# ashawkey/torch-ngp

Measured on AMD Instinct MI355X. Metric: training samples/s (rays x steps), lego-shaped synthetic, fp16 autocast, full step incl. Adam, higher is better.
Workload: dtype f16

## Files before the change

include/ngp_hip.h:

```cpp
#ifndef NGP_HIP_H
#define NGP_HIP_H

#include <stddef.h>
#include <stdint.h>

#ifdef __cplusplus
extern "C" {
#endif

typedef void* ngp_stream_t;

enum {
    NGP_OK = 0,
    NGP_ERR_INVALID = 1,
    NGP_ERR_LAUNCH = 2,
    NGP_ERR_DEVICE = 3
};

enum { NGP_F32 = 0, NGP_F16 = 1, NGP_F64 = 2 };

#define NGP_MAX_LEVELS 32

const char* ngp_last_error(void);
int ngp_abi_version(void);
// ... 177 lines not shown
#define NGP_FF_LAYERED 4u
#define NGP_FF_SINGLE_WAVE 8u
#define NGP_FF_DEFER_REDUCE 16u
#define NGP_FF_RECOMPUTE 32u
#define NGP_FF_SERIAL_FLUSH 64u
int ngp_ffmlp_forward_ex(const void* inputs, const void* weights, uint32_t B, uint32_t input_dim, uint32_t output_dim,
                         uint32_t hidden_dim, uint32_t num_layers, uint32_t activation, uint32_t output_activation,
                         void* forward_buffer, void* outputs, uint32_t flags, ngp_stream_t stream);
int ngp_ffmlp_inference_ex(const void* inputs, const void* weights, uint32_t B, uint32_t input_dim,
                           uint32_t output_dim, uint32_t hidden_dim, uint32_t num_layers, uint32_t activation,
                           uint32_t output_activation, void* inference_buffer, void* outputs, uint32_t flags,
                           ngp_stream_t stream);
int ngp_ffmlp_backward_ex(const void* grad, const void* inputs, const void* weights, const void* forward_buffer,
                          uint32_t B, uint32_t input_dim, uint32_t output_dim, uint32_t hidden_dim, uint32_t num_layers,
                          uint32_t activation, uint32_t output_activation, int calc_grad_inputs, void* backward_buffer,
                          void* grad_inputs, void* grad_weights, uint32_t flags, ngp_stream_t stream);

size_t ngp_ffmlp_backward_workspace_bytes(uint32_t B, uint32_t input_dim, uint32_t hidden_dim, uint32_t num_layers);
int ngp_ffmlp_backward_ws(const void* grad, const void* inputs, const void* weights, const void* forward_buffer, uint32_t B,
                          uint32_t input_dim, uint32_t output_dim, uint32_t hidden_dim, uint32_t num_layers, uint32_t activation,
                          uint32_t output_activation, int calc_grad_inputs, void* backward_buffer, void* grad_inputs, void* grad_weights,
                          uint32_t flags, void* workspace, size_t workspace_bytes, ngp_stream_t stream);

size_t ngp_ffmlp_backward_backward_workspace_bytes(uint32_t B, uint32_t input_dim, uint32_t hidden_dim, uint32_t num_layers,
                                                   uint32_t activation);
int ngp_ffmlp_backward_backward(const void* grad, const void* inputs, const void* weights, const void* forward_buffer, const void* u,
                                uint32_t B, uint32_t input_dim, uint32_t output_dim, uint32_t hidden_dim, uint32_t num_layers,
                                uint32_t activation, void* grad_grad, void* grad_weights2, void* grad_inputs2, void* workspace,
                                size_t workspace_bytes, ngp_stream_t stream);

int ngp_network_forward(const void* enc, const float* dirs, uint32_t M, uint32_t M_valid, const void* w_sigma, const void* w_color,
                        uint32_t num_layers_sigma, uint32_t num_layers_color, float density_scale, int training,
                        void* forward_buffer_sigma, void* h16, float* sigma, void* color_in, void* forward_buffer_color, float* rgb,
                        uint32_t flags, ngp_stream_t stream);

int ngp_network_forward_rows(const void* enc, const float* dirs, uint32_t M, uint32_t M_valid, const void* w_sigma, const void* w_color,
                             uint32_t num_layers_sigma, uint32_t num_layers_color, float density_scale, int training,
                             void* forward_buffer_sigma, void* h16, float* sigma, void* color_in, void* forward_buffer_color, float* rgb,
                             uint32_t flags, const uint32_t* rows_dev, ngp_stream_t stream);

int ngp_network_backward_color(const void* grad_out16, const void* color_in, const void* w_color, const void* forward_buffer_color, uint32_t M,
                               uint32_t num_layers_color, void* backward_buffer, const float* grad_sigma, const void* h16,
                               float density_scale, void* grad_h16, void* grad_w_color, uint32_t flags, ngp_stream_t stream);
uint32_t ngp_ffmlp_backward_slab_count(uint32_t B, uint32_t input_dim, uint32_t hidden_dim, uint32_t num_layers);
int ngp_ffmlp_reduce_slabs_pair(const void* slabs_a, uint32_t n_slabs_a, uint32_t n_params_a, void* grad_weights_a, const void* slabs_b,
                                uint32_t n_slabs_b, uint32_t n_params_b, void* grad_weights_b, float* found_inf, ngp_stream_t stream);

int ngp_pipeline_mid_forward(const void* h16, const float* dirs, float* sigma, void* color_in, uint32_t M, uint32_t M_valid,
                             float density_scale, ngp_stream_t stream);
int ngp_pipeline_rgb_forward(const void* out16, float* rgb, uint32_t M, ngp_stream_t stream);
int ngp_pipeline_rgb_backward(const float* grad_rgb, const float* rgb, void* grad_out16, uint32_t M, ngp_stream_t stream);
int ngp_pipeline_mid_backward(const float* grad_sigma, const void* h16, const void* grad_color_in, void* grad_h16, uint32_t M,
                              float density_scale, ngp_stream_t stream);

int ngp_pipeline_mse_loss(const float* image, const float* target, uint32_t n, const float* loss_scale, float* loss,
                          float* grad_image, ngp_stream_t stream);

#define NGP_LINEAR_STACK_MAX 8
uint32_t ngp_linear_stack_flat_size(uint32_t depth, uint32_t n_in, uint32_t hidden, uint32_t n_out, int identity);
int ngp_linear_stack_pack(const float* const* weights, uint32_t depth, uint32_t n_in, uint32_t hidden, uint32_t n_out, int identity,
                          void* flat_fp16, ngp_stream_t stream);
int ngp_linear_stack_unpack_grad(const void* grad_flat_fp16, uint32_t depth, uint32_t n_in, uint32_t hidden, uint32_t n_out, int identity,
                                 float* const* grads, ngp_stream_t stream);

int ngp_pad_2d_fp16(const void* src, uint32_t src_rows, uint32_t src_cols, uint32_t src_row_stride, void* dst, uint32_t dst_rows,
                    uint32_t dst_cols, ngp_stream_t stream);

int ngp_rays_from_pixels(const float* poses, uint32_t B, float fx, float fy, float cx, float cy, uint32_t W, const int64_t* inds,
                         uint32_t inds_batch_stride, uint32_t N, float* rays_o, float* rays_d, ngp_stream_t stream);

#define NGP_MARCH_RESET_COUNTER 1u
#define NGP_MARCH_ZERO_TAIL 2u
#define NGP_MARCH_SCAN_LAUNCH 8u
#define NGP_MARCH_NOISE_FROM_SEED 4u
int ngp_march_rays_train_ex(const float* rays_o, const float* rays_d, const uint8_t* grid, float bound, float dt_gamma,
                            uint32_t max_steps, uint32_t N, uint32_t C, uint32_t H, uint32_t M, const float* nears,
                            const float* fars, float* xyzs, float* dirs, float* deltas, int32_t* rays, int32_t* counter,
                            const float* noises, void* workspace, uint32_t flags, ngp_stream_t stream);
int ngp_march_rays_train_aabb(const float* rays_o, const float* rays_d, const uint8_t* grid, float bound, float dt_gamma,
                              uint32_t max_steps, uint32_t N, uint32_t C, uint32_t H, uint32_t M, const float* aabb, float min_near,
                              float* nears, float* fars, float* xyzs, float* dirs, float* deltas, int32_t* rays, int32_t* counter,
                              const float* noises, void* workspace, uint32_t flags, ngp_stream_t stream);

int ngp_march_rays_ex(uint32_t n_alive, uint32_t n_step, const int32_t* rays_alive, const float* rays_t, const float* rays_o,
                      const float* rays_d, float bound, float dt_gamma, uint32_t max_steps, uint32_t C, uint32_t H,
                      const uint8_t* grid, const float* nears, const float* fars, float* xyzs, float* dirs, float* deltas,
                      const float* noises, uint32_t zero_rows, ngp_stream_t stream);

int ngp_march_rays_dev(const int32_t* state, uint32_t alive_bound, uint32_t n_total, uint32_t n_step_cap, const int32_t* rays_alive, const float* rays_t,
                       const float* rays_o, const float* rays_d, float bound, float dt_gamma, uint32_t max_steps, uint32_t C, uint32_t H,
                       const uint8_t* grid, const float* nears, const float* fars, float* xyzs, float* dirs, float* deltas,
                       const float* noises, uint32_t rows, ngp_stream_t stream);
int ngp_march_rays_dev_rows(const int32_t* state, uint32_t alive_bound, uint32_t n_total, uint32_t n_step_cap, const int32_t* rays_alive, const float* rays_t,
                            const float* rays_o, const float* rays_d, float bound, float dt_gamma, uint32_t max_steps, uint32_t C, uint32_t H,
                            const uint8_t* grid, const float* nears, const float* fars, float* xyzs, float* dirs, float* deltas,
                            const float* noises, uint32_t rows, uint32_t* rows_used, ngp_stream_t stream);
int ngp_composite_rays_dev(const int32_t* state, uint32_t alive_bound, uint32_t n_total, uint32_t n_step_cap, float T_thresh, int32_t* rays_alive, float* rays_t,
                           const float* sigmas, const float* rgbs, const float* deltas, float* weights_sum, float* depth, float* image,
                           ngp_stream_t stream);
int ngp_compact_rays_dev(const int32_t* state, uint32_t alive_bound, uint32_t n_total, uint32_t n_step_cap, uint32_t max_steps, const int32_t* rays_alive,
                         int32_t* out_alive, int32_t* out_state, void* workspace, ngp_stream_t stream);

int ngp_composite_rays_features(uint32_t n_alive, uint32_t n_step, float T_thresh, const int32_t* rays_alive, const float* sigmas,
                                const void* feats, const float* deltas, const float* weights_sum, uint32_t C, int feat_dtype,
                                float* out, ngp_stream_t stream);
int ngp_composite_rays_features_dev(const int32_t* state, uint32_t alive_bound, uint32_t n_total, uint32_t n_step_cap, float T_thresh,
                                    const int32_t* rays_alive, const float* sigmas, const void* feats, const float* deltas,
                                    const float* weights_sum, uint32_t C, int feat_dtype, float* out, ngp_stream_t stream);

typedef struct ngp_render_loop {
    int32_t* state;
    int32_t* alive[2];
    float* rays_t; const float* rays_o; const float* rays_d; const float* nears; const float* fars; const uint8_t* grid; const float* noises;
    float* xyzs; float* dirs; float* deltas; void* enc; float* sigmas; float* rgbs;
    const void* embeddings; const int32_t* offsets; const float* level_cost_host; const void* w_sigma; const void* w_color;
    float* weights_sum; float* depth; float* image; void* compact_workspace;
    uint32_t* rows_used;
    uint32_t lanes, rows, n_total, n_step_cap, max_steps, cascade, grid_size;
    uint32_t L, H, gridtype, interp, num_layers_sigma, num_layers_color;
    int32_t align_corners;
    float bound, dt_gamma, T_thresh, S, density_scale;
} ngp_render_loop_t;
int ngp_render_iterations_dev(const ngp_render_loop_t* args, uint32_t n_iter, uint32_t first_cur, ngp_stream_t stream);

size_t ngp_coarse_occupancy_bytes(uint32_t C, uint32_t H);
int ngp_coarse_occupancy(const uint8_t* grid, uint32_t C, uint32_t H, uint8_t* coarse, ngp_stream_t stream);
int ngp_cull_rays(const float* rays_o, const float* rays_d, const float* nears, const float* fars, uint32_t N, float bound, uint32_t C,
                  uint32_t H, const uint8_t* coarse, int32_t* rays_alive, ngp_stream_t stream);

int ngp_composite_rays_train_forward_ex(const float* sigmas, const float* rgbs, const float* deltas, const int32_t* rays,
                                        uint32_t M, uint32_t N, float T_thresh, float* weights_sum, float* depth, float* image,
                                        int bg_mode, float bg_scalar, const float* bg, const float* nears, const float* fars,
                                        float* image_out, float* depth_out, ngp_stream_t stream);
int ngp_composite_rays_train_backward_ex(const float* grad_weights_sum, const float* grad_image, const float* sigmas,
                                         const float* rgbs, const float* deltas, const int32_t* rays,
                                         const float* weights_sum, const float* image, uint32_t M, uint32_t N,
                                         float T_thresh, float* grad_sigmas, float* grad_rgbs, int bg_mode, float bg_scalar,
                                         const float* bg, const uint32_t* rows_used, ngp_stream_t stream);

int ngp_composite_rays_train_geo_forward(const float* sigmas, const float* rgbs, const float* deltas, const int32_t* rays, uint32_t M,
                                         uint32_t N, float T_thresh, float* weights_sum, float* depth, float* image,
                                         float* distortion, ngp_stream_t stream);
int ngp_composite_rays_train_geo_backward(const float* grad_weights_sum, const float* grad_depth, const float* grad_image,
                                          const float* grad_distortion, const float* sigmas, const float* rgbs, const float* deltas,
                                          const int32_t* rays, const float* weights_sum, const float* depth, const float* image,
                                          const float* distortion, uint32_t M, uint32_t N, float T_thresh, float* grad_sigmas,
                                          float* grad_rgbs, ngp_stream_t stream);
int ngp_composite_rays_train_geo_forward_f64(const double* sigmas, const double* rgbs, const double* deltas, const int32_t* rays,
                                             uint32_t M, uint32_t N, float T_thresh, double* weights_sum, double* depth, double* image,
                                             double* distortion, ngp_stream_t stream);
int ngp_composite_rays_train_geo_backward_f64(const double* grad_weights_sum, const double* grad_depth, const double* grad_image,
                                              const double* grad_distortion, const double* sigmas, const double* rgbs,
                                              const double* deltas, const int32_t* rays, const double* weights_sum, const double* depth,
                                              const double* image, const double* distortion, uint32_t M, uint32_t N, float T_thresh,
                                              double* grad_sigmas, double* grad_rgbs, ngp_stream_t stream);

int ngp_composite_rays_train_features_forward(const float* sigmas, const void* feats, const float* deltas, const int32_t* rays, uint32_t M,
                                              uint32_t N, uint32_t C, float T_thresh, int feat_dtype, float* out, ngp_stream_t stream);
int ngp_composite_rays_train_features_backward(const float* grad_out, const float* sigmas, const void* feats, const float* deltas,
                                               const int32_t* rays, const float* out, uint32_t M, uint32_t N, uint32_t C, float T_thresh,
                                               int feat_dtype, float* grad_sigmas, void* grad_feats, ngp_stream_t stream);
int ngp_composite_rays_train_features_forward_f64(const double* sigmas, const double* feats, const double* deltas, const int32_t* rays,
                                                  uint32_t M, uint32_t N, uint32_t C, float T_thresh, double* out, ngp_stream_t stream);
int ngp_composite_rays_train_features_backward_f64(const double* grad_out, const double* sigmas, const double* feats, const double* deltas,
                                                   const int32_t* rays, const double* out, uint32_t M, uint32_t N, uint32_t C,
                                                   float T_thresh, double* grad_sigmas, double* grad_feats, ngp_stream_t stream);
// ... 91 lines not shown
```

torch-ngp_amd/_ngp_capi.py:

```python
import ctypes
import os

import torch

_HERE = os.path.dirname(os.path.abspath(__file__))
LIB_PATH = os.environ.get('NGP_HIP_LIBRARY') or os.path.join(_HERE, 'libngp_hip.so')

NGP_F32, NGP_F16, NGP_F64 = 0, 1, 2
NGP_FF_INPUT_PLANAR, NGP_FF_DX_PLANAR, NGP_FF_LAYERED, NGP_FF_SINGLE_WAVE, NGP_FF_DEFER_REDUCE, NGP_FF_RECOMPUTE = 1, 2, 4, 8, 16, 32
NGP_FF_SERIAL_FLUSH = 64
NGP_MARCH_RESET_COUNTER, NGP_MARCH_ZERO_TAIL, NGP_MARCH_NOISE_FROM_SEED, NGP_MARCH_SCAN_LAUNCH = 1, 2, 4, 8
NGP_OPT_PHASE_CHECK, NGP_OPT_PHASE_UPDATE, NGP_OPT_PHASE_COMMIT, NGP_OPT_PHASE_FLIP = 1, 2, 4, 8
ABI_VERSION = 11

if not os.path.exists(LIB_PATH):
    raise ImportError(
        f"{LIB_PATH} is missing: build the HIP extension first (python __graft_entry__.py, or "
        f"make -C {os.path.join(_HERE, 'csrc')}).  There is no CPU fallback for these operators.")

lib = ctypes.CDLL(LIB_PATH)

_vp, _u32, _f32, _i32, _sz = ctypes.c_void_p, ctypes.c_uint32, ctypes.c_float, ctypes.c_int, ctypes.c_size_t

_SIGNATURES = {
    'ngp_grid_encode_forward': [_vp, _vp, _vp, _vp, _u32, _u32, _u32, _u32, _f32, _u32, _vp, _u32, _i32, _u32, _i32, _vp],
    'ngp_grid_encode_backward': [_vp, _vp, _vp, _vp, _vp, _u32, _u32, _u32, _u32, _f32, _u32, _vp, _vp, _u32, _i32, _u32, _i32, _vp],
    'ngp_grad_total_variation': [_vp, _vp, _vp, _vp, _f32, _u32, _u32, _u32, _u32, _f32, _u32, _u32, _i32, _i32, _vp],
    'ngp_grid_corner_indices': [_vp, _vp, _vp, _u32, _u32, _u32, _f32, _u32, _u32, _i32, _vp],
    'ngp_grid_level_table': [_u32, _f32, _u32, _vp, _vp],
    'ngp_grid_encode_backward_backward': [_vp, _vp, _vp, _vp, _vp, _vp, _vp, _vp, _u32, _u32, _u32, _u32, _f32, _u32, _u32, _i32, _u32, _i32, _vp,
                                          _sz, _vp],
    'ngp_grid_encode_backward_ordered': [_vp, _vp, _vp, _vp, _vp, _u32, _u32, _u32, _u32, _f32, _u32, _vp, _vp, _u32, _i32, _u32, _i32, _f32, _vp,
                                         _sz, _vp],
    'ngp_grid_encode_backward_backward_ordered': [_vp, _vp, _vp, _vp, _vp, _vp, _vp, _vp, _u32, _u32, _u32, _u32, _f32, _u32, _u32, _i32, _u32, _i32,
                                                  _vp, _sz, _vp],
    'ngp_grid_backward_is_reproducible': [_vp, _u32, _u32, _u32, _u32, _f32, _u32, _u32, _i32, _i32],
    'ngp_sh_encode_forward': [_vp, _vp, _u32, _u32, _u32, _vp, _i32, _vp],
    'ngp_sh_encode_backward': [_vp, _vp, _u32, _u32, _u32, _vp, _vp, _i32, _vp],
    'ngp_freq_encode_forward': [_vp, _u32, _u32, _u32, _u32, _vp, _vp],
    'ngp_freq_encode_backward': [_vp, _vp, _u32, _u32, _u32, _u32, _vp, _vp],
    'ngp_freq_encode_forward_f64': [_vp, _u32, _u32, _u32, _u32, _vp, _vp],
    'ngp_freq_encode_backward_f64': [_vp, _vp, _u32, _u32, _u32, _u32, _vp, _vp],
    'ngp_freq_encode_backward_backward': [_vp, _vp, _vp, _u32, _u32, _u32, _u32, _vp, _vp, _i32, _vp],
    'ngp_sh_encode_backward_backward': [_vp, _vp, _vp, _vp, _u32, _u32, _u32, _vp, _vp, _i32, _vp],
    'ngp_near_far_from_aabb': [_vp, _vp, _vp, _u32, _f32, _vp, _vp, _vp],
    'ngp_sph_from_ray': [_vp, _vp, _f32, _u32, _vp, _vp],
    'ngp_morton3D': [_vp, _u32, _vp, _vp],
    'ngp_morton3D_invert': [_vp, _u32, _vp, _vp],
    'ngp_packbits': [_vp, _u32, _f32, _vp, _vp],
    'ngp_packbits_ex': [_vp, _u32, _f32, _vp, _vp, _vp],
    'ngp_march_rays_train': [_vp, _vp, _vp, _f32, _f32, _u32, _u32, _u32, _u32, _u32, _vp, _vp, _vp, _vp, _vp, _vp, _vp, _vp, _vp, _vp],
    'ngp_composite_rays_train_forward': [_vp, _vp, _vp, _vp, _u32, _u32, _f32, _vp, _vp, _vp, _vp],
    'ngp_composite_rays_train_backward': [_vp, _vp, _vp, _vp, _vp, _vp, _vp, _vp, _u32, _u32, _f32, _vp, _vp, _vp],
    'ngp_march_rays': [_u32, _u32, _vp, _vp, _vp, _vp, _f32, _f32, _u32, _u32, _u32, _vp, _vp, _vp, _vp, _vp, _vp, _vp, _vp],
    'ngp_march_rays_ex': [_u32, _u32, _vp, _vp, _vp, _vp, _f32, _f32, _u32, _u32, _u32, _vp, _vp, _vp, _vp, _vp, _vp, _vp, _u32, _vp],
    'ngp_composite_rays': [_u32, _u32, _f32, _vp, _vp, _vp, _vp, _vp, _vp, _vp, _vp, _vp],
    'ngp_near_far_from_aabb_f64': [_vp, _vp, _vp, _u32, _f32, _vp, _vp, _vp],
    'ngp_sph_from_ray_f64': [_vp, _vp, _f32, _u32, _vp, _vp],
    'ngp_packbits_f64': [_vp, _u32, _f32, _vp, _vp],
    'ngp_composite_rays_train_forward_f64': [_vp, _vp, _vp, _vp, _u32, _u32, _f32, _vp, _vp, _vp, _vp],
    'ngp_composite_rays_train_backward_f64': [_vp, _vp, _vp, _vp, _vp, _vp, _vp, _vp, _u32, _u32, _f32, _vp, _vp, _vp],
    'ngp_composite_rays_f64': [_u32, _u32, _f32, _vp, _vp, _vp, _vp, _vp, _vp, _vp, _vp, _vp],
    'ngp_compact_rays': [_vp, _u32, _vp, _vp, _vp, _vp],
    'ngp_coarse_occupancy': [_vp, _u32, _u32, _vp, _vp],
    'ngp_cull_rays': [_vp, _vp, _vp, _vp, _u32, _f32, _u32, _u32, _vp, _vp, _vp],
    'ngp_march_rays_dev': [_vp, _u32, _u32, _u32, _vp, _vp, _vp, _vp, _f32, _f32, _u32, _u32, _u32, _vp, _vp, _vp, _vp, _vp, _vp, _vp, _u32, _vp],
    'ngp_composite_rays_dev': [_vp, _u32, _u32, _u32, _f32, _vp, _vp, _vp, _vp, _vp, _vp, _vp, _vp, _vp],
    'ngp_compact_rays_dev': [_vp, _u32, _u32, _u32, _u32, _vp, _vp, _vp, _vp, _vp],
    'ngp_render_iterations_dev': [_vp, _u32, _u32, _vp],
    'ngp_ffmlp_forward': [_vp, _vp, _u32, _u32, _u32, _u32, _u32, _u32, _u32, _vp, _vp, _vp],
    'ngp_ffmlp_inference': [_vp, _vp, _u32, _u32, _u32, _u32, _u32, _u32, _u32, _vp, _vp, _vp],
    'ngp_ffmlp_backward': [_vp, _vp, _vp, _vp, _u32, _u32, _u32, _u32, _u32, _u32, _u32, _i32, _vp, _vp, _vp, _vp],
    'ngp_grid_encode_forward_ex': [_vp, _vp, _vp, _vp, _u32, _u32, _u32, _u32, _f32, _u32, _vp, _u32, _i32, _u32, _i32, _f32, _vp],
    'ngp_grid_encode_forward_sched': [_vp, _vp, _vp, _vp, _u32, _u32, _u32, _u32, _f32, _u32, _vp, _u32, _i32, _u32, _i32, _f32, _vp, _vp],
    'ngp_grid_encode_forward_sel': [_vp, _vp, _vp, _vp, _vp, _vp, _vp, _u32, _u32, _u32, _u32, _f32, _u32, _u32, _i32, _u32, _i32, _f32, _vp, _vp],
    'ngp_grid_encode_backward_ex': [_vp, _vp, _vp, _vp, _vp, _u32, _u32, _u32, _u32, _f32, _u32, _vp, _vp, _u32, _i32, _u32, _i32, _f32, _vp],
    'ngp_grid_encode_backward_ws': [_vp, _vp, _vp, _vp, _vp, _u32, _u32, _u32, _u32, _f32, _u32, _vp, _vp, _u32, _i32, _u32, _i32, _f32, _vp, _vp,
                                    _sz, _vp],
    'ngp_grid_encode_backward_checked': [_vp, _vp, _vp, _vp, _vp, _u32, _u32, _u32, _u32, _f32, _u32, _vp, _vp, _u32, _i32, _u32, _i32, _f32, _vp,
                                         _vp, _sz, _vp, _vp],
    'ngp_grid_encode_backward_checked_slabs': [_vp, _vp, _vp, _vp, _vp, _u32, _u32, _u32, _u32, _f32, _u32, _vp, _vp, _u32, _i32, _u32, _i32, _f32,
                                               _vp, _vp, _sz, _vp, _vp, _vp],
    'ngp_density_grid_update': [_vp, _vp, _u32, _f32, _f32, _vp, _u32, _vp, _f32, _vp, _vp, _vp, _vp],
    'ngp_ffmlp_forward_ex': [_vp, _vp, _u32, _u32, _u32, _u32, _u32, _u32, _u32, _vp, _vp, _u32, _vp],
    'ngp_ffmlp_inference_ex': [_vp, _vp, _u32, _u32, _u32, _u32, _u32, _u32, _u32, _vp, _vp, _u32, _vp],
    'ngp_ffmlp_backward_ex': [_vp, _vp, _vp, _vp, _u32, _u32, _u32, _u32, _u32, _u32, _u32, _i32, _vp, _vp, _vp, _u32, _vp],
    'ngp_ffmlp_backward_ws': [_vp, _vp, _vp, _vp, _u32, _u32, _u32, _u32, _u32, _u32, _u32, _i32, _vp, _vp, _vp, _u32, _vp, _sz, _vp],
    'ngp_ffmlp_backward_backward': [_vp, _vp, _vp, _vp, _vp, _u32, _u32, _u32, _u32, _u32, _u32, _vp, _vp, _vp, _vp, _sz, _vp],
    'ngp_network_forward': [_vp, _vp, _u32, _u32, _vp, _vp, _u32, _u32, _f32, _i32, _vp, _vp, _vp, _vp, _vp, _vp, _u32, _vp],
    'ngp_network_forward_rows': [_vp, _vp, _u32, _u32, _vp, _vp, _u32, _u32, _f32, _i32, _vp, _vp, _vp, _vp, _vp, _vp, _u32, _vp, _vp],
    'ngp_march_rays_dev_rows': [_vp, _u32, _u32, _u32, _vp, _vp, _vp, _vp, _f32, _f32, _u32, _u32, _u32, _vp, _vp, _vp, _vp, _vp, _vp, _vp, _u32, _vp, _vp],
    'ngp_pipeline_mid_forward': [_vp, _vp, _vp, _vp, _u32, _u32, _f32, _vp],
    'ngp_pipeline_rgb_forward': [_vp, _vp, _u32, _vp],
    'ngp_pipeline_rgb_backward': [_vp, _vp, _vp, _u32, _vp],
    'ngp_pipeline_mid_backward': [_vp, _vp, _vp, _vp, _u32, _f32, _vp],
    'ngp_pipeline_mse_loss': [_vp, _vp, _u32, _vp, _vp, _vp, _vp],
    'ngp_rays_from_pixels': [_vp, _u32, _f32, _f32, _f32, _f32, _u32, _vp, _u32, _u32, _vp, _vp, _vp],
    'ngp_march_rays_train_ex': [_vp, _vp, _vp, _f32, _f32, _u32, _u32, _u32, _u32, _u32, _vp, _vp, _vp, _vp, _vp, _vp, _vp, _vp, _vp, _u32, _vp],
    'ngp_march_rays_train_aabb': [_vp, _vp, _vp, _f32, _f32, _u32, _u32, _u32, _u32, _u32, _vp, _f32, _vp, _vp, _vp, _vp, _vp, _vp, _vp, _vp, _vp, _u32,
                                  _vp],
    'ngp_composite_rays_train_forward_ex': [_vp, _vp, _vp, _vp, _u32, _u32, _f32, _vp, _vp, _vp, _i32, _f32, _vp, _vp, _vp, _vp, _vp, _vp],
    'ngp_composite_rays_train_backward_ex': [_vp, _vp, _vp, _vp, _vp, _vp, _vp, _vp, _u32, _u32, _f32, _vp, _vp, _i32, _f32, _vp, _vp, _vp],
    'ngp_composite_rays_train_geo_forward': [_vp, _vp, _vp, _vp, _u32, _u32, _f32, _vp, _vp, _vp, _vp, _vp],
    'ngp_composite_rays_train_geo_backward': [_vp, _vp, _vp, _vp, _vp, _vp, _vp, _vp, _vp, _vp, _vp, _vp, _u32, _u32, _f32, _vp, _vp, _vp],
    'ngp_composite_rays_train_geo_forward_f64': [_vp, _vp, _vp, _vp, _u32, _u32, _f32, _vp, _vp, _vp, _vp, _vp],
    'ngp_composite_rays_train_geo_backward_f64': [_vp, _vp, _vp, _vp, _vp, _vp, _vp, _vp, _vp, _vp, _vp, _vp, _u32, _u32, _f32, _vp, _vp, _vp],
    'ngp_composite_rays_train_features_forward': [_vp, _vp, _vp, _vp, _u32, _u32, _u32, _f32, _i32, _vp, _vp],
    'ngp_composite_rays_train_features_backward': [_vp, _vp, _vp, _vp, _vp, _vp, _u32, _u32, _u32, _f32, _i32, _vp, _vp, _vp],
    'ngp_composite_rays_train_features_forward_f64': [_vp, _vp, _vp, _vp, _u32, _u32, _u32, _f32, _vp, _vp],
    'ngp_composite_rays_train_features_backward_f64': [_vp, _vp, _vp, _vp, _vp, _vp, _u32, _u32, _u32, _f32, _vp, _vp, _vp],
    'ngp_composite_rays_features': [_u32, _u32, _f32, _vp, _vp, _vp, _vp, _vp, _u32, _i32, _vp, _vp],
    'ngp_composite_rays_features_dev': [_vp, _u32, _u32, _u32, _f32, _vp, _vp, _vp, _vp, _vp, _u32, _i32, _vp, _vp],
    'ngp_composite_train_loss_backward': [_vp, _vp, _vp, _vp, _u32, _u32, _f32, _i32, _f32, _vp, _vp, _vp, _vp, _vp, _vp, _vp, _vp, _vp, _vp, _vp,
                                          _vp, _vp, _sz, _vp],
    'ngp_composite_train_geo_loss_backward': [_vp, _vp, _vp, _vp, _u32, _u32, _f32, _i32, _f32, _vp, _vp, _vp, _vp, _f32, _f32, _vp, _vp, _vp, _vp,
                                              _vp, _vp, _vp, _vp, _vp, _vp, _vp, _vp, _vp, _sz, _vp],
    'ngp_network_backward_color': [_vp, _vp, _vp, _vp, _u32, _u32, _vp, _vp, _vp, _f32, _vp, _vp, _u32, _vp],
    'ngp_ffmlp_reduce_slabs_pair': [_vp, _u32, _u32, _vp, _vp, _u32, _u32, _vp, _vp, _vp],
    'ngp_optim_adam_step': [_i32, _vp, _vp, _vp, _vp, _vp, _vp, _vp, _vp, _f32, _f32, _f32, _f32, _f32, _f32, _f32, _vp, _vp],
    'ngp_optim_adam_step_ex': [_i32, _vp, _vp, _vp, _vp, _vp, _vp, _vp, _vp, _f32, _f32, _f32, _f32, _f32, _f32, _f32, _vp, _vp, _f32, _u32, _vp],
    'ngp_optim_adam_small_commit': [_i32, _vp, _vp, _vp, _vp, _vp, _vp, _vp, _vp, _f32, _f32, _f32, _f32, _f32, _f32, _f32, _vp, _i32, _vp, _vp,
                                    ctypes.c_uint64, _vp],
    'ngp_optim_ema_update': [_i32, _vp, _vp, _vp, _f32, _vp],
    'ngp_optim_poison_shards': [_vp, _u32, ctypes.c_uint64, _vp, _vp],
    'ngp_optim_shard_verdict': [_vp, _vp, _vp, _u32, ctypes.c_uint64, _vp],
    'ngp_linear_stack_pack': [_vp, _u32, _u32, _u32, _u32, _i32, _vp, _vp],
    'ngp_linear_stack_unpack_grad': [_vp, _u32, _u32, _u32, _u32, _i32, _vp, _vp],
    'ngp_pad_2d_fp16': [_vp, _u32, _u32, _u32, _vp, _u32, _u32, _vp],
    'ngp_allocate_splitk': [_sz],
    'ngp_free_splitk': [],
    'ngp_cmdlist_create': [_vp],
    'ngp_cmdlist_begin': [_vp],
    'ngp_cmdlist_mark': [_vp, _u32, _i32],
    'ngp_cmdlist_end': [_vp],
    'ngp_cmdlist_count': [_vp, _vp],
    'ngp_cmdlist_entry_name': [_vp, _u32, _vp, _u32],
    'ngp_cmdlist_replay': [_vp, _vp],
    'ngp_cmdlist_wait_mark': [_vp, _u32, _vp],
    'ngp_cmdlist_destroy': [_vp],
    'ngp_ray_sample_ts': [_vp, _vp, _vp, _vp, _u32, _u32, _f32, _vp, _vp],
    'ngp_ray_sample_ts_f64': [_vp, _vp, _vp, _vp, _u32, _u32, _f32, _vp, _vp],
    'ngp_ray_points_forward': [_vp, _vp, _vp, _vp, _u32, _u32, _f32, _vp, _vp, _vp],
    'ngp_ray_points_forward_f64': [_vp, _vp, _vp, _vp, _u32, _u32, _f32, _vp, _vp, _vp],
    'ngp_ray_points_backward': [_vp, _vp, _vp, _vp, _vp, _vp, _vp, _u32, _u32, _f32, _vp, _vp, _vp],
    'ngp_ray_points_backward_f64': [_vp, _vp, _vp, _vp, _vp, _vp, _u32, _u32, _f32, _vp, _vp, _vp],
    'ngp_grid_input_gradient': [_vp, _vp, _vp, _vp, _u32, _u32, _u32, _u32, _f32, _u32, _u32, _i32, _u32, _i32, _f32, _vp, _vp],
    'ngp_rays_from_pixels_backward': [_vp, _vp, _u32, _f32, _f32, _f32, _f32, _u32, _vp, _u32, _u32, _vp, _vp],
    'ngp_error_map_draw': [_vp, _u32, _u32, _u32, _u32, _u32, _u32, _vp, _vp, _vp, _vp, _vp, _vp],
    'ngp_error_map_update': [_vp, _vp, _vp, _vp, _u32, _u32, _f32, _f32, _vp],
}
for _name, _args in _SIGNATURES.items():
    _fn = getattr(lib, _name)
    _fn.argtypes = _args
    _fn.restype = ctypes.c_int
lib.ngp_last_error.restype = ctypes.c_char_p
lib.ngp_target_arch.restype = ctypes.c_char_p
lib.ngp_abi_version.restype = ctypes.c_int
lib.ngp_ffmlp_backward_slab_count.argtypes = [_u32, _u32, _u32, _u32]
lib.ngp_ffmlp_backward_slab_count.restype = _u32
lib.ngp_march_rays_train_workspace_bytes.argtypes = [_u32]
lib.ngp_march_rays_train_workspace_bytes.restype = _sz
lib.ngp_compact_rays_workspace_bytes.argtypes = [_u32]
lib.ngp_ffmlp_backward_workspace_bytes.argtypes = [_u32, _u32, _u32, _u32]
lib.ngp_ffmlp_backward_workspace_bytes.restype = _sz
lib.ngp_ffmlp_backward_backward_workspace_bytes.argtypes = [_u32, _u32, _u32, _u32, _u32]
lib.ngp_ffmlp_backward_backward_workspace_bytes.restype = _sz
lib.ngp_grid_backward_workspace_bytes.argtypes = [_vp, _u32, _u32, _u32, _u32, _f32, _u32, _u32, _i32, _i32]
lib.ngp_grid_backward_workspace_bytes.restype = _sz
lib.ngp_grid_backward_backward_workspace_bytes.argtypes = [_vp, _u32, _u32, _u32, _u32, _i32]
lib.ngp_grid_backward_backward_workspace_bytes.restype = _sz
lib.ngp_compact_rays_workspace_bytes.restype = _sz
lib.ngp_grid_ordered_workspace_bytes.argtypes = [_u32, _u32, _u32, _i32]
lib.ngp_grid_ordered_workspace_bytes.restype = _sz
lib.ngp_grid_table_adam_prefix.argtypes = [_vp, _u32, _u32, _u32, _u32, _f32, _u32, _u32, _i32, _i32]
lib.ngp_grid_table_adam_prefix.restype = _u32
lib.ngp_coarse_occupancy_bytes.argtypes = [_u32, _u32]
lib.ngp_coarse_occupancy_bytes.restype = _sz
lib.ngp_grid_forward_work_lists.argtypes = [_u32, _u32, _vp, _vp, _vp, _vp]
lib.ngp_grid_forward_work_lists.restype = _u32
lib.ngp_density_grid_update_workspace_bytes.argtypes = [_u32]
lib.ngp_linear_stack_flat_size.argtypes = [_u32, _u32, _u32, _u32, _i32]
lib.ngp_linear_stack_flat_size.restype = _u32
lib.ngp_density_grid_update_workspace_bytes.restype = _sz
# ... 138 lines not shown
```

torch-ngp_amd/csrc/common.h:

```cpp
#pragma once
#include <hip/hip_runtime.h>
#include <stdint.h>
#include <cstdio>
#include <cstdarg>

#include "../../include/ngp_hip.h"
#include "cmdlist_core.h"

namespace ngp {

using half_t = _Float16;
typedef _Float16 half2_t __attribute__((ext_vector_type(2)));
typedef _Float16 half4_t __attribute__((ext_vector_type(4)));
typedef _Float16 half8_t __attribute__((ext_vector_type(8)));
typedef float float2_t __attribute__((ext_vector_type(2)));
typedef float float4_t __attribute__((ext_vector_type(4)));
typedef float float16_t __attribute__((ext_vector_type(16)));

constexpr int WAVE = 64;

void set_error(const char* fmt, ...);
void set_error_message(const char* message);

inline int check_launch(const char* what) {
    hipError_t e = hipGetLastError();
    if (e != hipSuccess) {
        set_error("%s: kernel launch failed: %s", what, hipGetErrorString(e));
        return NGP_ERR_LAUNCH;
    }
    return NGP_OK;
}

#define NGP_REQUIRE(cond, code, ...)        \
    do {                                    \
        if (!(cond)) {                      \
            ::ngp::set_error(__VA_ARGS__);  \
            return (code);                  \
        }                                   \
    } while (0)

inline uint32_t cdiv(uint32_t a, uint32_t b) { return (a + b - 1) / b; }
inline uint64_t cdiv64(uint64_t a, uint64_t b) { return (a + b - 1) / b; }

inline hipStream_t as_stream(ngp_stream_t s) { return reinterpret_cast<hipStream_t>(s); }

template <typename T> struct launch_param { using type = T; };
template <typename... KA>
inline hipError_t launch(const char* name, void (*kernel)(KA...), dim3 grid, dim3 block, size_t lds, hipStream_t st, const typename launch_param<KA>::type&... a) {
    void* argv[] = {const_cast<void*>(static_cast<const void*>(&a))..., nullptr};
    const hipError_t e = hipLaunchKernel(reinterpret_cast<const void*>(kernel), grid, block, argv, lds, st);
    if (cmdlist::List* l = cmdlist::recording()) {
        static const size_t sizes[] = {sizeof(KA)..., 0}, aligns[] = {alignof(KA)..., 0};
        l->record_launch(reinterpret_cast<const void*>(kernel), name, cmdlist::Dim{grid.x, grid.y, grid.z}, cmdlist::Dim{block.x, block.y, block.z},
                         (uint32_t)lds, (uint32_t)sizeof...(KA), argv, sizes, aligns);
    }
    return e;
}
#define NGP_LAUNCH_STATUS(kernel, grid, block, lds, st, ...) ::ngp::launch(#kernel, kernel, grid, block, lds, st, __VA_ARGS__)
#define NGP_LAUNCH(...) ((void)NGP_LAUNCH_STATUS(__VA_ARGS__))
inline hipError_t memset_async(void* dst, int value, size_t bytes, hipStream_t st) {
    const hipError_t e = hipMemsetAsync(dst, value, bytes, st);
    if (cmdlist::List* l = cmdlist::recording()) e == hipSuccess ? l->record_memset(dst, value, bytes) : l->poison();
    return e;
}
inline hipError_t memcpy_async(void* dst, const void* src, size_t bytes, hipMemcpyKind kind, hipStream_t st) {
    const hipError_t e = hipMemcpyAsync(dst, src, bytes, kind, st);
    if (cmdlist::List* l = cmdlist::recording()) e == hipSuccess ? l->record_memcpy(dst, src, bytes, (int)kind) : l->poison();
    return e;
}

#ifdef NGP_DEBUG_BOUNDS
#define NGP_BOUNDS(cond) do { if (!(cond)) __builtin_trap(); } while (0)
#else
#define NGP_BOUNDS(cond) do { } while (0)
#endif

__device__ __forceinline__ _Float16 to_half_rne(float v) {
    asm volatile("" : "+v"(v));
    return (_Float16)v;
}

__device__ __forceinline__ float clampf(float x, float lo, float hi) { return fminf(hi, fmaxf(lo, x)); }

__device__ __forceinline__ uint32_t wave_inclusive_scan(uint32_t v) {
    const int lane = threadIdx.x & 63;
#pragma unroll
    for (int o = 1; o < 64; o <<= 1) {
        uint32_t n = __shfl_up(v, o, 64);
        if (lane >= o) v += n;
    }
    return v;
}

__device__ __forceinline__ float wave_sum(float v) {
#pragma unroll
    for (int o = 32; o > 0; o >>= 1) v += __shfl_xor(v, o, 64);
    return v;
}

template <int CTRL, int ROW_MASK>
__device__ __forceinline__ float dpp_or(float identity, float src) {
    return __builtin_bit_cast(float, __builtin_amdgcn_update_dpp(__builtin_bit_cast(int, identity), __builtin_bit_cast(int, src), CTRL, ROW_MASK,
                                                                 0xF, false));
}
__device__ __forceinline__ float wave_incl_sum(float v, int) {
    v += dpp_or<0x111, 0xF>(0.0f, v);
    v += dpp_or<0x112, 0xF>(0.0f, v);
    v += dpp_or<0x114, 0xF>(0.0f, v);
    v += dpp_or<0x118, 0xF>(0.0f, v);
    v += dpp_or<0x142, 0xA>(0.0f, v);
    v += dpp_or<0x143, 0xC>(0.0f, v);
    return v;
}
__device__ __forceinline__ float lane63(float v) { return __builtin_bit_cast(float, __builtin_amdgcn_readlane(__builtin_bit_cast(int, v), 63)); }
__device__ __forceinline__ float wave_total(float v) { return lane63(wave_incl_sum(v, 0)); }

__device__ __forceinline__ void loss_sum_block(const float* err, uint32_t N, float* loss, float* part) {
    const uint32_t t = threadIdx.x;
    float acc = 0.0f;
    if (t < 256u) {
        for (uint32_t i = t; i < N; i += 256u) acc += __hip_atomic_load(&err[i], __ATOMIC_RELAXED, __HIP_MEMORY_SCOPE_AGENT);
        acc = wave_total(acc);
        if ((t & 63u) == 0u) part[t >> 6] = acc;
    }
    __syncthreads();
    if (t == 0u) {
        float v = 0.0f;
#pragma unroll
        for (int w = 0; w < 4; w++) v += part[w];
        loss[0] = v / (float)(3u * N);
    }
}

enum OptState { OPT_SCALE, OPT_GROWTH_TRACKER, OPT_FOUND_INF, OPT_STEP_COUNT, OPT_LR_MULT, OPT_TABLE_PARITY, OPT_TICKET, OPT_SCALE_DEAD, OPT_STATE_WORDS };
static_assert(OPT_STATE_WORDS == 8, "include/ngp_hip.h: state = device float[8]");
struct AdamConsts {
    float inv_scale, bc1, bc2_sqrt, lr_mult;
    bool skip;
};
__device__ __forceinline__ AdamConsts adam_consts(const float* state, float beta1, float beta2, float grad_mult) {
    AdamConsts a;
    const bool scale_dead = !__builtin_isfinite(1.0f / state[OPT_SCALE]);
    a.skip = state[OPT_FOUND_INF] != 0.0f || scale_dead;
    a.inv_scale = scale_dead ? 0.0f : grad_mult / state[OPT_SCALE];
    const float t = state[OPT_STEP_COUNT] + 1.0f;
    a.bc1 = 1.0f - powf(beta1, t);
    a.bc2_sqrt = sqrtf(1.0f - powf(beta2, t));
    a.lr_mult = state[OPT_LR_MULT];
    return a;
}
__device__ __forceinline__ void adam_element(float g, float& pm, float& pv, float& pp, float beta1, float beta2, float eps, float step_size,
                                             float bc2_sqrt) {
    pm = beta1 * pm + (1.0f - beta1) * g;
    pv = beta2 * pv + (1.0f - beta2) * g * g;
    pp -= step_size * pm / (sqrtf(pv) / bc2_sqrt + eps);
}
struct TableAdam {
    float* p[2];
// ... 73 lines not shown
```

torch-ngp_amd/csrc/ffmlp.hip:

```cpp
#include "common.h"
#include "sh_poly.inc"

namespace ngp {

constexpr int FF_WAVES = 4;
constexpr int FF_THREADS = FF_WAVES * 64;
constexpr int FF_TILE = 32;

enum Act : uint32_t { ACT_RELU = 0, ACT_EXP = 1, ACT_SINE = 2, ACT_SIGMOID = 3, ACT_SQUAREPLUS = 4, ACT_SOFTPLUS = 5, ACT_NONE = 6 };
constexpr float K_ACT = 10.0f;

__device__ __forceinline__ float act_forward(uint32_t a, float x) {
    switch (a) {
        case ACT_RELU: return x > 0.0f ? x : 0.0f;
        case ACT_EXP: return __expf(x);
        case ACT_SINE: return __sinf(x);
        case ACT_SIGMOID: return 1.0f / (1.0f + __expf(-x));
        case ACT_SQUAREPLUS: { const float s = x * K_ACT; return 0.5f * (s + sqrtf(s * s + 4.0f)) / K_ACT; }
        case ACT_SOFTPLUS: return __logf(__expf(x * K_ACT) + 1.0f) / K_ACT;
        default: return x;
    }
}
__device__ __forceinline__ float act_backward_factor(uint32_t a, float y) {
    switch (a) {
// ... 251 lines not shown
            const half8_t* wl = img_hid + (size_t)l * NIB * NKB * 64;
#pragma unroll
            for (int ib = 0; ib < NIB; ib++) {
                acc[ib] = zero16();
#pragma unroll
                for (int kb = 0; kb < NKB; kb++) acc[ib] = mfma(wl[(ib * NKB + kb) * 64], hid[kb], acc[ib]);
            }
        }
        float16_t o = zero16();
#pragma unroll
        for (int kb = 0; kb < NKB; kb++) o = mfma(img_out[kb * 64], hid[kb], o);
        half4_t lo, hi;
#pragma unroll
        for (int c = 0; c < 4; c++) {
            lo[c] = (half_t)(PLAIN ? o[c] : act_forward(out_act, o[c]));
            hi[c] = (half_t)(PLAIN ? o[4 + c] : act_forward(out_act, o[4 + c]));
        }
        half_t* orow = outputs + ((size_t)tile * FF_TILE + n) * 16 + 4 * h;
        *reinterpret_cast<half4_t*>(orow) = lo;
        *reinterpret_cast<half4_t*>(orow + 8) = hi;
    }
}

template <int WIDTH, bool TRAIN, bool PLAIN>
__global__ __launch_bounds__(FF_THREADS) __attribute__((amdgpu_waves_per_eu(4, 4))) void k_ffmlp_forward(
    const half_t* __restrict__ inputs, const half_t* __restrict__ weights, half_t* __restrict__ forward_buffer, half_t* __restrict__ outputs,
    uint32_t n_tiles, uint32_t in_dim, uint32_t num_layers, uint32_t act, uint32_t out_act, bool in_planar) {
    ffmlp_forward_body<WIDTH, TRAIN, PLAIN>(inputs, weights, forward_buffer, outputs, n_tiles, in_dim, num_layers, act, out_act, in_planar);
}
template <int WIDTH, bool TRAIN, bool PLAIN>
__global__ __launch_bounds__(FF_THREADS) __attribute__((amdgpu_waves_per_eu(2, 2))) void k_ffmlp_forward_wide(
    const half_t* __restrict__ inputs, const half_t* __restrict__ weights, half_t* __restrict__ forward_buffer, half_t* __restrict__ outputs,
    uint32_t n_tiles, uint32_t in_dim, uint32_t num_layers, uint32_t act, uint32_t out_act, bool in_planar) {
    ffmlp_forward_body<WIDTH, TRAIN, PLAIN>(inputs, weights, forward_buffer, outputs, n_tiles, in_dim, num_layers, act, out_act, in_planar);
}


template <bool TRAIN, int NT>
__device__ __forceinline__ void relu_network_tail(float16_t (&acc)[NT][2], float16_t (&o)[NT], const half8_t* __restrict__ hid_img,
                                                  const half8_t* __restrict__ out_img, uint32_t nl, half_t* __restrict__ fb, size_t layer_stride,
                                                  const uint32_t (&tile)[NT], const bool (&live)[NT], int lane) {
    constexpr int WIDTH = 64, NIB = 2, NKB = 4;
    half8_t hid[NT][NKB];
    for (uint32_t l = 0;; l++) {
#pragma unroll
        for (int t = 0; t < NT; t++) {
            pack_hidden_relu<WIDTH>(acc[t], hid[t]);
            if (TRAIN && fb && live[t]) {
                half8_t* dst = reinterpret_cast<half8_t*>(fb) + l * layer_stride + (size_t)tile[t] * NKB * 64 + lane;
#pragma unroll
                for (int kb = 0; kb < NKB; kb++) stream_store(dst + kb * 64, hid[t][kb]);
            }
        }
        if (l + 1 == nl) break;
        const half8_t* wl = hid_img + (size_t)l * NIB * NKB * 64;
#pragma unroll
        for (int ib = 0; ib < NIB; ib++) {
#pragma unroll
            for (int t = 0; t < NT; t++) acc[t][ib] = zero16();
#pragma unroll
            for (int kb = 0; kb < NKB; kb++) {
                const half8_t a = wl[(ib * NKB + kb) * 64];
#pragma unroll
                for (int t = 0; t < NT; t++) acc[t][ib] = mfma(a, hid[t][kb], acc[t][ib]);
            }
        }
    }
#pragma unroll
    for (int t = 0; t < NT; t++) o[t] = zero16();
#pragma unroll
    for (int kb = 0; kb < NKB; kb++) {
        const half8_t a = out_img[kb * 64];
#pragma unroll
        for (int t = 0; t < NT; t++) o[t] = mfma(a, hid[t][kb], o[t]);
    }
}

template <bool TRAIN, int WAVES , int NT >
__global__ __launch_bounds__(WAVES * 64) __attribute__((amdgpu_waves_per_eu(NT == 1 ? 4 : 2, NT == 1 ? 4 : 3))) void k_network_forward(
    const half_t* __restrict__ enc, bool enc_planar, const float* __restrict__ dirs, uint32_t M_valid, const half_t* __restrict__ w_sigma,
    const half_t* __restrict__ w_color, half_t* __restrict__ fb_s, half_t* __restrict__ h16, float* __restrict__ sigma,
    half_t* __restrict__ color_in, half_t* __restrict__ fb_c, float* __restrict__ rgb, uint32_t n_tiles_cap, uint32_t nl_s, uint32_t nl_c,
    float density_scale, const uint32_t* __restrict__ rows_dev) {
    constexpr int WIDTH = 64, NIB = 2, NKB = 4;
    constexpr uint32_t in_kb = 2;
    const uint32_t n_tiles = rows_dev ? min(n_tiles_cap, (rows_dev[0] + (uint32_t)FF_TILE - 1u) / (uint32_t)FF_TILE) : n_tiles_cap;
    extern __shared__ __attribute__((aligned(16))) unsigned char smem[];
    half8_t* img_s = reinterpret_cast<half8_t*>(smem);
    const uint32_t frags_s = NIB * in_kb + (nl_s - 1) * NIB * NKB + NKB;
    half8_t* img_c = img_s + (size_t)frags_s * 64;
    const size_t rows = (size_t)n_tiles_cap * FF_TILE;
    const int lane = threadIdx.x & 63, wid = threadIdx.x >> 6;
    const int n = lane & 31, h = lane >> 5;
    const uint32_t n_groups = (n_tiles + NT - 1) / NT;
    half8_t x_next[NT][in_kb];
    float dir_next[NT][3];
#pragma unroll
    for (int t = 0; t < NT; t++) dir_next[t][0] = dir_next[t][1] = dir_next[t][2] = 0.0f;
    auto request = [&](uint32_t group) {
        if (group < n_groups) {
#pragma unroll
            for (int t = 0; t < NT; t++) {
                const uint32_t tl = group * NT + t < n_tiles ? group * NT + t : n_tiles - 1;
                const size_t srow = (size_t)tl * FF_TILE + n;
#pragma unroll
                for (uint32_t kb = 0; kb < in_kb; kb++) x_next[t][kb] = load_features8(enc, enc_planar, rows, srow, 32, 16 * kb + 8 * h);
                dir_next[t][0] = dir_next[t][1] = dir_next[t][2] = 0.0f;
                if (srow < M_valid) { dir_next[t][0] = dirs[srow * 3]; dir_next[t][1] = dirs[srow * 3 + 1]; dir_next[t][2] = dirs[srow * 3 + 2]; }
            }
        }
    };
    request(blockIdx.x * WAVES + wid);
    build_forward_image<WIDTH>(img_s, w_sigma, 32, nl_s);
    build_forward_image<WIDTH>(img_c, w_color, 32, nl_c);
    __syncthreads();

    const size_t layer_stride = (size_t)n_tiles_cap * NKB * 64;
    const half8_t* s_l0 = img_s + lane;
    const half8_t* s_hid = s_l0 + (size_t)NIB * in_kb * 64;
    const half8_t* s_out = s_hid + (size_t)(nl_s - 1) * NIB * NKB * 64;
    const half8_t* c_l0 = img_c + lane;
    const half8_t* c_hid = c_l0 + (size_t)NIB * in_kb * 64;
    const half8_t* c_out = c_hid + (size_t)(nl_c - 1) * NIB * NKB * 64;

    for (uint32_t group = blockIdx.x * WAVES + wid; group < n_groups; group += gridDim.x * WAVES) {
        uint32_t tile[NT];
        bool live[NT];
        size_t srow[NT];
        half8_t x_cur[NT][in_kb];
        float dir_x[NT], dir_y[NT], dir_z[NT];
#pragma unroll
        for (int t = 0; t < NT; t++) {
            live[t] = NT == 1 || group * NT + t < n_tiles;
            tile[t] = live[t] ? group * NT + t : n_tiles - 1;
            srow[t] = (size_t)tile[t] * FF_TILE + n;
#pragma unroll
            for (uint32_t kb = 0; kb < in_kb; kb++) x_cur[t][kb] = x_next[t][kb];
            dir_x[t] = dir_next[t][0]; dir_y[t] = dir_next[t][1]; dir_z[t] = dir_next[t][2];
        }
        request(group + gridDim.x * WAVES);
        float16_t acc[NT][NIB], o[NT];
#pragma unroll
        for (int t = 0; t < NT; t++)
#pragma unroll
            for (int ib = 0; ib < NIB; ib++) acc[t][ib] = zero16();
#pragma unroll
        for (uint32_t kb = 0; kb < in_kb; kb++)
#pragma unroll
            for (int ib = 0; ib < NIB; ib++) {
                const half8_t a = s_l0[(ib * in_kb + kb) * 64];
#pragma unroll
                for (int t = 0; t < NT; t++) acc[t][ib] = mfma(a, x_cur[t][kb], acc[t][ib]);
            }
        relu_network_tail<TRAIN, NT>(acc, o, s_hid, s_out, nl_s, fb_s, layer_stride, tile, live, lane);
        half8_t cin[NT][2];
#pragma unroll
        for (int t = 0; t < NT; t++) {
            half4_t lo, hi;
#pragma unroll
            for (int c = 0; c < 4; c++) { lo[c] = (half_t)o[t][c]; hi[c] = (half_t)o[t][4 + c]; }
            if (TRAIN && live[t]) {
                half_t* hrow = h16 + srow[t] * 16 + 4 * h;
                *reinterpret_cast<half4_t*>(hrow) = lo;
                *reinterpret_cast<half4_t*>(hrow + 8) = hi;
            }
            if (h == 0 && live[t]) sigma[srow[t]] = density_scale * expf((float)lo[0]);
// ... 529 lines not shown
                pack_transposed(t, xT);
#pragma unroll
                for (int g = 0; g < 2; g++)
#pragma unroll
                    for (int ib = 0; ib < NIB; ib++) gw_in[ib][jb] = mfma(zT[ib][g], xT[g], gw_in[ib][jb]);
            }
        }
        if (with_dx) store_dx<WIDTH, IN_JB>(img_in, dz, grad_inputs, tile, n, h, in_dim, rows, dx_planar);
        if (pf_depth == 1 && tile + tile_step < n_tiles) {
            asm volatile("s_waitcnt lgkmcnt(0)" ::: "memory");
            prefetch_tile<WIDTH>(pf_base, tile + tile_step, grad, fb, inputs, num_layers, layer_stride, rows, in_dim, in_planar, lane, n, h);
        }
    }

    float* red = reinterpret_cast<float*>(smem);
    const SlabLayout lay{WIDTH, in_dim, num_layers};
    const uint32_t n_params = lay.n_params();
    auto each = [&](const auto& sink) { slab_put_all<WIDTH, IN_JB, NHM>(sink, lay, gw_in, gw_hid, gw_out); };
    if (slab_staged_single<WIDTH, IN_JB, NHM> && !serial_flush) {
        static_assert(!slab_staged_single<WIDTH, IN_JB, NHM> || slab_fits_whole<WIDTH, IN_JB, NHM>, "the single-wave staged sum is one pass");
        slab_sum_pass<FF_THREADS>(red, lds_bytes, SlabPart{0, n_params}, wid, slabs + (size_t)blockIdx.x * n_params, grad_weights_direct, n, h, each);
        return;
    }
    slab_serial_begin<FF_THREADS>(red, n_params);
    const SlabSerial serial{red, n, h};
    for (int turn = 0; turn < FF_WAVES; turn++) {
        if (wid == turn) each(serial);
        __syncthreads();
    }
    slab_serial_store<FF_THREADS>(red, n_params, slabs, grad_weights_direct);
}

constexpr int FP_PAIRS = 4;
constexpr int FP_THREADS = 2 * FP_PAIRS * 64;

struct MidEpilogue {
    const float* grad_sigma;
    const half_t* h16;
    half_t* grad_h16;
    float density_scale;
};

template <int WIDTH, int NHM, typename Sink>
__device__ __forceinline__ void recompute_hidden(const half8_t* __restrict__ fimg_lane, uint32_t in_kb, const unsigned char* xb, bool in_planar,
                                                 int lane, Sink&& sink) {
    constexpr int NIB = Shape<WIDTH>::NIB, NKB = Shape<WIDTH>::NKB;
    float16_t acc[NIB];
#pragma unroll
    for (int ib = 0; ib < NIB; ib++) acc[ib] = zero16();
    for (uint32_t kb = 0; kb < in_kb; kb++) {
        const half8_t x = tile_x(xb, kb, in_planar, lane);
#pragma unroll
        for (int ib = 0; ib < NIB; ib++) acc[ib] = mfma(fimg_lane[(ib * in_kb + kb) * 64], x, acc[ib]);
    }
    const half8_t* fhid = fimg_lane + (size_t)NIB * in_kb * 64;
    half8_t hid[NKB];
#pragma unroll
    for (int l = 0; l <= NHM; l++) {
        pack_hidden_relu<WIDTH>(acc, hid);
        sink(l, hid);
        if (l == NHM) break;
        const half8_t* wl = fhid + (size_t)l * NIB * NKB * 64;
#pragma unroll
        for (int ib = 0; ib < NIB; ib++) {
            acc[ib] = zero16();
#pragma unroll
            for (int kb = 0; kb < NKB; kb++) acc[ib] = mfma(wl[(ib * NKB + kb) * 64], hid[kb], acc[ib]);
        }
    }
}

template <int N>
__device__ __forceinline__ void wait_vmcnt() {
    asm volatile("s_waitcnt vmcnt(%0)" ::"n"(N) : "memory");
}

template <int WIDTH, int IN_JB, int NHM , bool RELU, bool RECOMP = false>
__global__ __launch_bounds__(FP_THREADS) __attribute__((amdgpu_waves_per_eu(2, 2)))
void k_ffmlp_backward_paired(const half_t* __restrict__ grad, const half_t* __restrict__ inputs, const half_t* __restrict__ weights,
                             const half_t* __restrict__ forward_buffer, uint32_t n_tiles, uint32_t in_dim, uint32_t num_layers, uint32_t act,
                             bool with_dx, half_t* __restrict__ grad_inputs, float* __restrict__ slabs,
                             half_t* __restrict__ grad_weights_direct, bool in_planar, bool dx_planar, uint32_t pf_depth, MidEpilogue mid,
                             uint32_t lds_bytes, bool serial_flush) {
    static_assert(NHM == 1 || NHM == 2, "the paired backward covers 2- and 3-layer networks");
    constexpr int NIB = Shape<WIDTH>::NIB, NKB = Shape<WIDTH>::NKB;
    extern __shared__ __attribute__((aligned(16))) unsigned char smem[];
    half8_t* img = reinterpret_cast<half8_t*>(smem);
    const uint32_t nfrag = bwd_frag_count<WIDTH>(in_dim, num_layers, with_dx);
    const uint32_t in_kb = in_dim / 16;
    const uint32_t ffrag = RECOMP ? NIB * in_kb + (num_layers - 1) * NIB * NKB : 0u;
    const int lane = threadIdx.x & 63, wid = threadIdx.x >> 6;
    const int n = lane & 31, h = lane >> 5;
    const int pair = wid & (FP_PAIRS - 1), role = wid / FP_PAIRS;
    const size_t layer_stride = (size_t)n_tiles * NKB * 64;
    const half8_t* fb = reinterpret_cast<const half8_t*>(forward_buffer);
    const size_t rows = (size_t)n_tiles * FF_TILE;
    const uint32_t act_layers = RECOMP ? 0u : num_layers;
    const uint32_t tile_frags = 1 + act_layers * NKB + in_kb;
    unsigned char* pf_base = smem + (size_t)(nfrag + ffrag) * 1024 + (size_t)pair * pf_depth * tile_frags * 1024;
    half8_t* scratch = reinterpret_cast<half8_t*>(smem + (size_t)(nfrag + ffrag) * 1024 + (size_t)FP_PAIRS * pf_depth * tile_frags * 1024 +
                                                  (size_t)pair * NHM * NKB * 1024) + lane;
    const uint32_t base_step = gridDim.x * FP_PAIRS;
    uint32_t cur = 0;
    const uint32_t tile_loads = tile_dma_count<WIDTH>(act_layers, in_dim, in_planar);
    auto prefetch = [&](uint32_t buffer, uint32_t tile) {
        const uint32_t issued = prefetch_tile<WIDTH>(pf_base + (size_t)buffer * tile_frags * 1024, tile, grad, fb, inputs, act_layers, layer_stride,
                                                     rows, in_dim, in_planar, lane, n, h);
        NGP_BOUNDS(issued == tile_loads);
        (void)issued;
    };
    if (role == 0) {
        for (uint32_t d = 0; d + 1 < (pf_depth > 1 ? pf_depth : 2u); d++)
            if (blockIdx.x * FP_PAIRS + d * base_step + pair < n_tiles) prefetch(d, blockIdx.x * FP_PAIRS + d * base_step + pair);
    }
    build_backward_image<WIDTH>(img, weights, in_dim, num_layers, with_dx);
    if (RECOMP) build_forward_image<WIDTH>(img + (size_t)nfrag * 64, weights, in_dim, num_layers, 0, ffrag);
    const Selectors sel = make_selectors(n, h);
    __syncthreads();

    const half8_t* img_out = img + lane;
    const half8_t* img_hid = img_out + (size_t)NIB * 64;
    const half8_t* img_in = img_hid + (size_t)(num_layers - 1) * NIB * NKB * 64;
    const half8_t* fimg = img + (size_t)nfrag * 64 + lane;
    static_assert(tile_dma_count<64>(0, 32, false) == 3u && tile_dma_count<64>(0, 32, true) == 9u && tile_dma_count<64>(2, 32, false) == 11u &&
                  tile_dma_count<64>(2, 32, true) == 17u, "the enumerated vmcnt immediates below are the DMA counts of the three-deep shapes");
    const bool deep = pf_depth == 3 && (tile_loads == 3u || tile_loads == 9u || tile_loads == 11u || tile_loads == 17u);
    auto next_tile_buffer = [&](uint32_t base) -> const unsigned char* {
        if (role == 0) {
            if (deep && base + base_step + pair < n_tiles) {
                switch (tile_loads) {
                    case 3u: wait_vmcnt<3>(); break;
                    case 9u: wait_vmcnt<9>(); break;
                    case 11u: wait_vmcnt<11>(); break;
                    default: wait_vmcnt<17>(); break;
                }
            } else {
                wait_vmcnt<0>();
            }
        }
        __syncthreads();
        const unsigned char* tb = pf_base + (size_t)cur * tile_frags * 1024;
        if (pf_depth > 1) {
            const uint32_t ahead = pf_depth - 1;
            const uint32_t fill = cur == 0 ? pf_depth - 1 : cur - 1;
            cur = cur + 1 == pf_depth ? 0u : cur + 1;
            if (role == 0 && base + ahead * base_step + pair < n_tiles) prefetch(fill, base + ahead * base_step + pair);
        }
        return tb;
    };
    auto end_of_round = [&](uint32_t base) {
        if (pf_depth == 1) {
            __syncthreads();
            if (role == 0 && base + base_step + pair < n_tiles) prefetch(0, base + base_step + pair);
        }
    };
    float* red = reinterpret_cast<float*>(smem);
    const SlabLayout lay{WIDTH, in_dim, num_layers};
    const uint32_t n_params = lay.n_params();
    const uint32_t base_out = lay.out();
    const uint32_t base_top = lay.hidden(num_layers - 1);
    const uint32_t base_low = lay.hidden(1);
    const SlabSerial serial{red, n, h};
    constexpr bool whole = slab_fits_whole<WIDTH, IN_JB, NHM>;
    const SlabPart part_a = whole ? SlabPart{0u, n_params} : SlabPart{base_low, n_params - base_low}, part_b = SlabPart{0u, base_low};
    auto pass = [&](SlabPart p, auto&& stage_fn) {
        slab_sum_pass<FP_THREADS>(red, lds_bytes, p, pair, slabs + (size_t)blockIdx.x * n_params, grad_weights_direct, n, h, stage_fn);
// ... 982 lines not shown
```

torch-ngp_amd/csrc/gridencoder.hip:

```cpp
#include "common.h"
#include "grid_index.h"
#include "fp64.h"
#include <math.h>
#include <string.h>
#include <algorithm>
#include <vector>

namespace ngp {

template <typename T, int C>
struct Vec;
template <int C>
struct Vec<float, C> {
    float v[C];
    __device__ __forceinline__ void load(const float* p) {
#pragma unroll
        for (int c = 0; c < C; c++) v[c] = p[c];
    }
};
template <>
struct Vec<float, 2> {
    float v[2];
    __device__ __forceinline__ void load(const float* p) {
        float2_t t = *reinterpret_cast<const float2_t*>(p);
// ... 878 lines not shown
#pragma unroll
    for (int s = 0; s < NS; s++) {
        slot[s] = 0u;
        if (binned && bin_issues(live_mask, bin_run_mask(bl.addr[s], pairs))) slot[s] = lds_add_rtn_u32(bin_counter_addr<FAST>(bl.addr[s], it, prow_base));
    }
    const half2_t gh = __builtin_bit_cast(half2_t, gbits);
    const float g0 = (float)gh.x, g1 = (float)gh.y;
#pragma unroll
    for (int s = 0; s < NS; s++) {
        const uint32_t addr = bl.addr[s];
        float w = bl.wp[0][s & 1];
#pragma unroll
        for (int d = 1; d < D; d++) w *= bl.wp[d][(s >> d) & 1];
        float v0 = w * g0, v1 = w * g1;
        const LaneMask m = bin_run_mask(addr, pairs);
        uint32_t key = FAST ? (addr & (uint32_t)(BIN_SLICE - 1)) : (it.interleaved ? (addr >> BIN_DENSE_BITS) : (addr & (uint32_t)(BIN_SLICE - 1)));
        if (m.any()) {
            seg_scan_rows(v0, v1, m);
            if (__builtin_amdgcn_ballot_w64(fmaxf(__builtin_fabsf(v0), __builtin_fabsf(v1)) >= 32768.0f) != 0ull) {
                if (__builtin_fabsf(v0) >= 32768.0f) { v0 *= 0.015625f; key |= BIN_KEY_SCALED0; }
                if (__builtin_fabsf(v1) >= 32768.0f) { v1 *= 0.015625f; key |= BIN_KEY_SCALED1; }
            }
        }
        const uint32_t packed = pack_half2(v0, v1);
        if (bin_issues(live_mask, m)) {
            NGP_BOUNDS(!binned || slot[s] < (uint32_t)(BIN_PPB * NS) + (uint32_t)BIN_MAX_BINS);
            if (binned)
                *(__attribute__((address_space(3))) unsigned long long*)(uintptr_t)(staging_base + slot[s] * 8u) = ((unsigned long long)packed << 32) | key;
            else atomic_add_packed(it.gtable + (size_t)addr * 2, packed);
        }
    }
}

template <int BPL, int WAVES>
__device__ __forceinline__ uint32_t bin_offsets(const uint32_t* __restrict__ hist, uint32_t* __restrict__ prow, int lane, int wid, const BinItem& it,
                                                uint32_t n_chunks, uint32_t* __restrict__ descriptors, uint32_t staging_base) {
    constexpr int CAP = 64 * BPL;
    uint32_t tot[BPL], mine[BPL];
#pragma unroll
    for (int k = 0; k < BPL; k++) tot[k] = mine[k] = 0u;
#pragma unroll BPL <= 2 ? WAVES : 1
    for (int w = 0; w < WAVES; w++) {
#pragma unroll
        for (int k = 0; k < BPL; k++) tot[k] += hist[w * CAP + lane * BPL + k];
    }
#pragma unroll 1
    for (int w = 0; w < wid; w++) {
#pragma unroll
        for (int k = 0; k < BPL; k++) mine[k] += hist[w * CAP + lane * BPL + k];
    }
    uint32_t begin = 0u;
    {
        uint32_t even[BPL], erun = 0u;
#pragma unroll
        for (int k = 0; k < BPL; k++) { even[k] = (tot[k] + 1u) & ~1u; erun += even[k]; }
        const uint32_t incl = wave_incl_sum_u32(erun);
        begin = incl - erun;
        const uint32_t total_units = wave_last_lane(incl) >> 1;
#pragma unroll
        for (int k = 0; k < BPL; k++) {
            prow[lane * BPL + k] = begin + mine[k];
            const uint32_t bin = (uint32_t)(lane * BPL + k);
            NGP_BOUNDS(begin + even[k] <= (uint32_t)(BIN_PPB * 8) + (uint32_t)CAP && it.chunk_x < n_chunks);
            if (wid == 0 && bin < it.n_bins) {
                descriptors[it.desc_base + (size_t)bin * n_chunks + it.chunk_x] = (begin >> 1) | (tot[k] << 16);
                if (tot[k] & 1u)
                    *(volatile __attribute__((address_space(3))) unsigned long long*)(uintptr_t)(staging_base + (begin + tot[k]) * 8u) = 0ull;
            }
            begin += even[k];
        }
        return total_units;
    }
}

#ifndef NGP_BIN_WAVES_PER_EU
#define NGP_BIN_WAVES_PER_EU 6
#endif
template <int D, int AMERGE ,
          int BPL >
__global__ __launch_bounds__(BIN_THREADS) __attribute__((amdgpu_waves_per_eu(BPL == 2 ? NGP_BIN_WAVES_PER_EU : 4, BPL == 2 ? NGP_BIN_WAVES_PER_EU : 4)))
void k_grid_backward_bin(const half_t* __restrict__ grad, const float* __restrict__ inputs, const int32_t* __restrict__ offsets,
                         half_t* __restrict__ grad_grid, uint32_t B, GridLevels lv, uint32_t gridtype, bool align_corners, uint32_t interp,
                         InputMap im, BinPlan plan, uint32_t* __restrict__ descriptors, uint2* __restrict__ records, AtomicPart ap) {
    uint32_t bin_block = blockIdx.x, n_bin_blocks = gridDim.x;
    if (ap.n_blocks) {
        const uint64_t total = gridDim.x;
        const uint32_t a0 = (uint32_t)(((uint64_t)blockIdx.x * ap.n_blocks) / total);
        const uint32_t a1 = (uint32_t)((((uint64_t)blockIdx.x + 1u) * ap.n_blocks) / total);
        if (a1 > a0) {
            backward_atomic_block<half_t, D, 2, AMERGE, BIN_THREADS>(grad, inputs, offsets, grad_grid, B, ap.levels.level[a0 / ap.blocks_per_level], lv,
                                                                gridtype, align_corners, interp, ap.points_per_block, im,
                                                                a0 % ap.blocks_per_level);
            return;
        }
        bin_block = blockIdx.x - a0;
        n_bin_blocks = gridDim.x - ap.n_blocks;
    }
    constexpr int C = 2;
    constexpr int NS = 1 << D;
    constexpr int MAX_REC = BIN_PPB * NS;
    constexpr int WAVES = BIN_THREADS / 64;
    extern __shared__ __attribute__((aligned(16))) unsigned char bin_smem[];
    unsigned char* staging = bin_smem;
    const uint32_t staging_base = (uint32_t)(uintptr_t)(__attribute__((address_space(3))) void*)staging;
    uint32_t* hist = reinterpret_cast<uint32_t*>(bin_smem + sizeof(uint2) * (MAX_REC + 64 * BPL));
    constexpr uint32_t cap = 64 * BPL;
    static_assert((MAX_REC / 2 + 32 * BPL) * BIN_UNIT_BYTES <= MAX_REC * sizeof(uint2), "pair units (plus half a unit of padding per bin) fit the chunk");
    uint32_t* pos = hist + WAVES * cap;
    const int tid = threadIdx.x, lane = tid & 63, wid = (int)__builtin_amdgcn_readfirstlane(tid >> 6);
    uint32_t* __restrict__ hrow = hist + wid * cap;
    uint32_t* __restrict__ prow = pos + wid * cap;
    const uint32_t hrow_base = (uint32_t)(uintptr_t)(__attribute__((address_space(3))) void*)hrow;
    const uint32_t prow_base = (uint32_t)(uintptr_t)(__attribute__((address_space(3))) void*)prow;
    const uint32_t n_levels = plan.n_levels;
    const uint32_t n_items = plan.n_chunks * n_levels;
    uint32_t item = (uint32_t)(((uint64_t)bin_block * n_items) / n_bin_blocks);
    const uint32_t item_end = (uint32_t)((((uint64_t)bin_block + 1u) * n_items) / n_bin_blocks);
    BinItem it;
    it.chunk_x = item / n_levels;
    it.li = item - it.chunk_x * n_levels;

    for (uint32_t i = lane; i < cap; i += 64) hrow[i] = 0u;
    unsigned long long levels_differ;
    {
        bool differ = false;
        if ((uint32_t)lane < n_levels) {
            const uint32_t level = plan.level(lane);
            differ = (uint32_t)offsets[level + 1] - (uint32_t)offsets[level] != plan.size(lane);
        }
        levels_differ = __builtin_amdgcn_ballot_w64(differ);
    }
    float x[D];
#pragma unroll
    for (int d = 0; d < D; d++) x[d] = 0.0f;
    uint32_t g_cur = 0u, chunk_loaded = 0xffffffffu;
    auto fetch_g = [&](uint32_t chunk_x, uint32_t li) -> uint32_t {
        const uint32_t b = chunk_x * BIN_PPB + (uint32_t)tid;
        return b < B ? *reinterpret_cast<const uint32_t*>(grad + ((size_t)plan.level(li) * B + b) * C) : 0u;
    };
    if (item < item_end) g_cur = fetch_g(it.chunk_x, it.li);
    __syncthreads();
    for (; item < item_end; item++) {
        const uint32_t b = it.chunk_x * BIN_PPB + (uint32_t)tid;
        const bool in_range = b < B;
        if (it.chunk_x != chunk_loaded) {
            chunk_loaded = it.chunk_x;
            if (in_range) {
#pragma unroll
                for (int d = 0; d < D; d++) x[d] = inputs[(size_t)b * D + d];
            }
        }
        uint32_t li_next = it.li + 1u, chunk_next = it.chunk_x;
        if (li_next == n_levels) { li_next = 0u; chunk_next++; }
        const uint32_t g_next = item + 1u < item_end ? fetch_g(chunk_next, li_next) : 0u;
        const uint32_t* __restrict__ lc = plan.lc[it.li];
        const uint32_t level = lc[LC_LEVEL], flags = lc[LC_FLAGS];
        it.n_bins = lc[LC_N_BINS];
        it.scale = __builtin_bit_cast(float, lc[LC_SCALE]);
        it.desc_base = lc[LC_DESC_BASE];
        it.interleaved = (flags & LC_INTERLEAVED) != 0u;
        LevelIndexer<D> indexer;
        indexer.size = lc[LC_SIZE];
        indexer.mask = lc[LC_MASK];
        indexer.hashed = (flags & LC_HASHED) != 0u;
        indexer.need_mod = (flags & LC_NEED_MOD) != 0u;
#pragma unroll
// ... 1007 lines not shown
```

torch-ngp_amd/csrc/raymarching.hip:

```cpp
#include "common.h"
#include <math.h>
#include <float.h>

namespace ngp {

constexpr int RM_THREADS = 256;

__device__ __forceinline__ void near_far_from_aabb(float ox, float oy, float oz, float dx, float dy, float dz, const float* __restrict__ aabb,
                                                   float min_near, float& near_out, float& far_out) {
    const float rdx = 1.0f / dx, rdy = 1.0f / dy, rdz = 1.0f / dz;
    float near = (aabb[0] - ox) * rdx, far = (aabb[3] - ox) * rdx, t;
    near_out = far_out = FLT_MAX;
    if (near > far) { t = near; near = far; far = t; }
    float ny = (aabb[1] - oy) * rdy, fy = (aabb[4] - oy) * rdy;
    if (ny > fy) { t = ny; ny = fy; fy = t; }
    if (near > fy || ny > far) return;
    if (ny > near) near = ny;
    if (fy < far) far = fy;
    float nz = (aabb[2] - oz) * rdz, fz = (aabb[5] - oz) * rdz;
    if (nz > fz) { t = nz; nz = fz; fz = t; }
    if (near > fz || nz > far) return;
    if (nz > near) near = nz;
    if (fz < far) far = fz;
    if (near < min_near) near = min_near;
// ... 254 lines not shown
    const float stop = fminf(tt, far);
    constexpr int U = 8;
    for (;;) {
        float s[U];
        float c = t;
#pragma unroll
        for (int i = 0; i < U; i++) {
            c += CONST_DT ? dt_const : step_dt(p, c);
            s[i] = c;
        }
        float pick = s[U - 1];
#pragma unroll
        for (int i = U - 2; i >= 0; i--) pick = (s[i] < stop) ? pick : s[i];
        if (!(pick > t)) return stop;
        t = pick;
        if (!(t < stop)) return t;
    }
}

__device__ __forceinline__ uint32_t block_sum(uint32_t v, uint32_t* lds4) {
    const int lane = threadIdx.x & 63, wid = threadIdx.x >> 6;
    uint32_t s = v;
#pragma unroll
    for (int o = 32; o > 0; o >>= 1) s += __shfl_xor(s, o, 64);
    __syncthreads();
    if (lane == 0) lds4[wid] = s;
    __syncthreads();
    uint32_t tot = 0;
#pragma unroll
    for (int w = 0; w < RM_THREADS / 64; w++) tot += lds4[w];
    return tot;
}

constexpr int MW_WAVES = 4;
constexpr uint32_t CT_GROUPS = 32, CT_GROUP_STRIDE = 32;
constexpr uint32_t MARCH_MASK_WINDOWS = 20;

__host__ __device__ inline size_t march_ws_ticket_word(uint32_t N) {
    const size_t words = (size_t)(2 + ((N + 1u) & ~1u)) + 2 * (size_t)N * MARCH_MASK_WINDOWS;
    return (words + CT_GROUP_STRIDE - 1) / CT_GROUP_STRIDE * CT_GROUP_STRIDE;
}

__device__ __forceinline__ float readlane_f(float v, uint32_t l) {
    return __builtin_bit_cast(float, __builtin_amdgcn_readlane(__builtin_bit_cast(int, v), (int)l));
}

template <bool CONST_DT>
__device__ __forceinline__ void window_terms(const MarchParams& p, float t_base, float dt_const, uint32_t lane, float& mine,
                                             float& t_next_base, float& inc_out, bool& closed_out) {
    if (CONST_DT) {
        const float t1 = t_base + dt_const;
        const float inc = t1 - t_base;
        const float err = dt_const - inc;
        const float t_end = __builtin_fmaf(64.0f, inc, t_base);
        const uint32_t e0 = __builtin_bit_cast(uint32_t, t_base) >> 23, e1 = __builtin_bit_cast(uint32_t, t_end) >> 23;
        const float half_ulp = __builtin_bit_cast(float, (e0 > 24u ? e0 - 24u : 0u) << 23);
        const bool closed = inc > 0.0f && e0 == e1 && e0 > 24u && e0 < 255u && fabsf(err) != half_ulp;
        if (__builtin_amdgcn_readfirstlane((int)closed)) {
            mine = __builtin_fmaf((float)lane, inc, t_base);
            t_next_base = t_end;
            inc_out = inc;
            closed_out = true;
            return;
        }
    }
    inc_out = 0.0f;
    closed_out = false;
    float t = t_base;
    mine = t_base;
#pragma unroll
    for (uint32_t j = 1; j < 64; j++) {
        t += CONST_DT ? dt_const : step_dt(p, t);
        mine = (lane == j) ? t : mine;
    }
    t_next_base = t + (CONST_DT ? dt_const : step_dt(p, t));
}

__device__ __forceinline__ float seeded_noise(uint32_t n, uint32_t seed) {
    uint32_t x = (n * 0x9E3779B9u) ^ (seed * 0x85EBCA6Bu + 0x27D4EB2Fu);
    x ^= x >> 16; x *= 0x7FEB352Du; x ^= x >> 15; x *= 0x846CA68Bu; x ^= x >> 16;
    return (float)(x >> 8) * 0x1p-24f;
}

template <bool WRITE, bool CONST_DT>
__global__ __launch_bounds__(MW_WAVES * 64) void k_march_train_wave(const float* __restrict__ rays_o, const float* __restrict__ rays_d,
                                                                    const uint8_t* __restrict__ grid, float bound, float dt_gamma,
                                                                    uint32_t max_steps, uint32_t N, uint32_t C, uint32_t H, uint32_t M,
                                                                    float* __restrict__ nears, float* __restrict__ fars,
                                                                    float* __restrict__ xyzs, float* __restrict__ dirs,
                                                                    float* __restrict__ deltas, int32_t* __restrict__ rays,
                                                                    const float* __restrict__ noises, uint32_t* __restrict__ n_windows,
                                                                    uint64_t* __restrict__ masks, bool noise_from_seed,
                                                                    const float* __restrict__ aabb, float min_near,
                                                                    uint32_t* __restrict__ fit_end, uint32_t ray_blocks,
                                                                    int32_t* __restrict__ self_scan_counter, bool zero_tail) {
    const uint32_t lane = threadIdx.x & 63;
    __shared__ uint32_t part[MW_WAVES], part2[MW_WAVES];
    if (WRITE && blockIdx.x >= ray_blocks) {
        uint32_t first_row;
        if (self_scan_counter) {
            constexpr uint32_t T = MW_WAVES * 64;
            const uint32_t per = (N + T - 1) / T, lo = min(N, threadIdx.x * per), hi = min(N, lo + per);
            uint32_t seg = 0;
            for (uint32_t i = lo; i < hi; i++) seg += (uint32_t)rays[i * 3 + 2];
            const uint32_t incl = wave_inclusive_scan(seg);
            if (lane == 63) part[threadIdx.x >> 6] = incl;
            __syncthreads();
            uint32_t before = 0, total = 0;
#pragma unroll
            for (int w = 0; w < MW_WAVES; w++) { before += (uint32_t)w < (threadIdx.x >> 6) ? part[w] : 0u; total += part[w]; }
            uint32_t off = before + incl - seg, unfit = 0xFFFFFFFFu;
            for (uint32_t i = lo; i < hi; i++) {
                const uint32_t c = (uint32_t)rays[i * 3 + 2];
                if (c != 0u && off + c > M && unfit == 0xFFFFFFFFu) unfit = off;
                off += c;
            }
#pragma unroll
            for (int o = 32; o > 0; o >>= 1) unfit = min(unfit, (uint32_t)__shfl_xor((int)unfit, o, 64));
            if (lane == 0) part2[threadIdx.x >> 6] = unfit;
            __syncthreads();
#pragma unroll
            for (int w = 0; w < MW_WAVES; w++) unfit = min(unfit, part2[w]);
            const uint32_t end = unfit != 0xFFFFFFFFu ? unfit : total;
            first_row = end < M ? end : M;
            if (blockIdx.x == ray_blocks && threadIdx.x == 0) {
                self_scan_counter[0] = (int32_t)total;
                self_scan_counter[1] = (int32_t)N;
                fit_end[0] = first_row;
                fit_end[1] = 0u;
            }
            if (blockIdx.x == ray_blocks && threadIdx.x < CT_GROUPS) fit_end[march_ws_ticket_word(N) + threadIdx.x * CT_GROUP_STRIDE] = 0u;
        } else {
            first_row = fit_end[0];
        }
        if (zero_tail) {
            const uint32_t stride = (gridDim.x - ray_blocks) * MW_WAVES * 64;
            for (uint32_t row = first_row + (blockIdx.x - ray_blocks) * MW_WAVES * 64 + threadIdx.x; row < M; row += stride) {
                xyzs[(size_t)row * 3] = 0.0f; xyzs[(size_t)row * 3 + 1] = 0.0f; xyzs[(size_t)row * 3 + 2] = 0.0f;
                dirs[(size_t)row * 3] = 0.0f; dirs[(size_t)row * 3 + 1] = 0.0f; dirs[(size_t)row * 3 + 2] = 0.0f;
                *reinterpret_cast<float2_t*>(deltas + (size_t)row * 2) = float2_t{0.0f, 0.0f};
            }
        }
        return;
    }
    const uint32_t wid = (uint32_t)__builtin_amdgcn_readfirstlane((int)(threadIdx.x >> 6));
    const uint32_t n = blockIdx.x * MW_WAVES + wid;
    uint32_t scanned_offset = 0;
    if (WRITE && self_scan_counter) {
        uint32_t sum = 0;
        const uint32_t first = blockIdx.x * MW_WAVES;
        for (uint32_t i = threadIdx.x; i < first; i += MW_WAVES * 64) sum += (uint32_t)rays[i * 3 + 2];
#pragma unroll
        for (int o = 32; o > 0; o >>= 1) sum += (uint32_t)__shfl_xor((int)sum, o, 64);
        if (lane == 0) part[wid] = sum;
        __syncthreads();
#pragma unroll
        for (int w = 0; w < MW_WAVES; w++) scanned_offset += part[w];
        for (uint32_t w = 0; w < wid; w++) scanned_offset += first + w < N ? (uint32_t)rays[(first + w) * 3 + 2] : 0u;
        if (n < N && lane == 0) rays[n * 3 + 1] = (int32_t)scanned_offset;
    }
    if (n >= N) return;
    const MarchParams p = make_params(bound, dt_gamma, max_steps, C, H, grid);
    const Ray r = load_ray(rays_o, rays_d, n);
    float far, near;
    if (!WRITE && aabb) {
        near_far_from_aabb(r.ox, r.oy, r.oz, r.dx, r.dy, r.dz, aabb, min_near, near, far);
        if (lane == 0) { nears[n] = near; fars[n] = far; }
    } else {
        far = fars[n];
        near = nears[n];
    }
    const float dt_const = step_dt(p, 0.0f);

    uint32_t limit = max_steps, offset = 0;
    if (WRITE) {
        offset = self_scan_counter ? scanned_offset : (uint32_t)rays[n * 3 + 1];
        limit = (uint32_t)rays[n * 3 + 2];
        if (limit == 0 || offset + limit > M) return;
    }
    uint32_t num_steps = 0;
    const float noise = noise_from_seed ? seeded_noise(n, reinterpret_cast<const uint32_t*>(noises)[0]) : noises[n];
    float t_base = __builtin_fmaf(step_dt(p, near), noise, near);
    float last_t = t_base;
    uint32_t window = 0;

    if (WRITE) {
        const uint32_t nw = n_windows[n];
        if (nw <= MARCH_MASK_WINDOWS) {
            const uint64_t* my_masks = masks + (size_t)n * MARCH_MASK_WINDOWS;
            for (; window < nw; window++) {
                float mine, t_next, inc_unused;
                bool closed_unused;
                window_terms<CONST_DT>(p, t_base, dt_const, lane, mine, t_next, inc_unused, closed_unused);
                t_base = t_next;
                const uint64_t emit = my_masks[window];
                if (emit == 0ull) continue;
                const float x = clampf(__builtin_fmaf(mine, r.dx, r.ox), -p.bound, p.bound);
                const float y = clampf(__builtin_fmaf(mine, r.dy, r.oy), -p.bound, p.bound);
                const float z = clampf(__builtin_fmaf(mine, r.dz, r.oz), -p.bound, p.bound);
                const float dt = step_dt(p, mine);
                const bool e = (emit >> lane) & 1ull;
                const uint64_t below = emit & ((1ull << lane) - 1ull);
                const uint32_t rank = (uint32_t)__builtin_popcountll(below);
                const float t_after = mine + dt;
                const int src = below ? 63 - __builtin_clzll(below) : 0;
                const float prev_after = __shfl(t_after, src, 64);
                const float lt = below ? prev_after : last_t;
                if (e) {
                    const size_t o = (size_t)offset + rank;
                    float* xo = xyzs + o * 3;
                    float* dd = dirs + o * 3;
                    xo[0] = x; xo[1] = y; xo[2] = z;
                    dd[0] = r.dx; dd[1] = r.dy; dd[2] = r.dz;
                    *reinterpret_cast<float2_t*>(deltas + o * 2) = float2_t{dt, t_after - lt};
                }
                last_t = readlane_f(t_after, 63u - (uint32_t)__builtin_clzll(emit));
                offset += (uint32_t)__builtin_popcountll(emit);
            }
            return;
        }
    }
    float carry = -INFINITY;
    bool done = !(t_base < far);

    float mine_n = 0.0f, t_after_n = t_base, base_n = t_base, inc_n = 0.0f;
    bool closed_n = false;
    ProbeGeom g_n = {};
    uint32_t byte_n = 0u;
    bool valid_n = false;
    auto issue_window = [&](float base) {
        base_n = base;
        window_terms<CONST_DT>(p, base, dt_const, lane, mine_n, t_after_n, inc_n, closed_n);
        valid_n = mine_n < far;
        g_n = probe_geom(p, r, valid_n ? mine_n : near);
        byte_n = p.grid[g_n.index >> 3];
    };
    if (!done) issue_window(t_base);

    while (!done) {
        const float mine = mine_n;
        const float t_next_base = t_after_n;
        const float win_base = base_n, win_inc = inc_n;
        const bool win_closed = closed_n;
        const bool valid = valid_n;
        const ProbeGeom g = g_n;
        const uint32_t byte = byte_n;
        if (__builtin_amdgcn_readfirstlane((int)(t_next_base < far))) issue_window(t_next_base);
        else valid_n = false;
        bool occ = false;
        float tt = -INFINITY;
        const float x = g.x, y = g.y, z = g.z, dt = g.dt;
        if (valid) occ = probe_resolve(p, r, mine, g, byte, tt);
        const uint64_t validmask = __ballot(valid);
        const uint64_t occmask = __ballot(valid && occ);
        const uint64_t entrymask = __ballot(!(mine < carry));
        uint32_t cur = entrymask ? (uint32_t)__builtin_ctzll(entrymask) : 64u;
        bool ray_done = false;
        uint64_t emit = 0;

        if (cur < 64u) {
            const float target = (valid && !occ) ? tt : -INFINITY;
            uint32_t land = lane + 1u;
            if (CONST_DT && win_closed) {
                const float est = fminf(fmaxf(ceilf((target - win_base) / win_inc) - 1.0f, 0.0f), 64.0f);
                const uint32_t q0 = (uint32_t)est;
                land = q0 > land ? q0 : land;
#pragma unroll
                for (int k = 0; k < 2; k++) {
                    const float tq = __builtin_fmaf((float)land, win_inc, win_base);
                    land = (land < 64u && tq < target) ? land + 1u : land;
                }
                land = land < 64u ? land : 64u;
            } else {
#pragma unroll
                for (uint32_t s = 32; s >= 1; s >>= 1) {
                    const uint32_t q = land + s - 1u;
                    const float tq = __shfl(mine, (int)(q & 63u), 64);
                    const bool adv = (q < 64u) && (tq < target);
                    land = adv ? land + s : land;
                }
            }
            carry = -INFINITY;
            while (cur < 64u) {
                if (!((validmask >> cur) & 1ull) || num_steps >= limit) { ray_done = true; break; }
                if ((occmask >> cur) & 1ull) {
                    const uint64_t rest = ~(occmask >> cur);
                    uint32_t run = rest ? (uint32_t)__builtin_ctzll(rest) : 64u;
                    const uint32_t room = limit - num_steps;
                    run = run < room ? run : room;
                    emit |= (run >= 64u ? ~0ull : ((1ull << run) - 1ull)) << cur;
                    num_steps += run;
                    cur += run;
                } else {
                    const uint32_t nx = (uint32_t)__builtin_amdgcn_readlane((int)land, (int)cur);
                    if (nx >= 64u) carry = readlane_f(target, cur);
                    cur = nx;
                }
            }
        }

        if (WRITE && emit != 0ull) {
            const bool e = (emit >> lane) & 1ull;
            const uint64_t below = emit & ((1ull << lane) - 1ull);
            const uint32_t rank = (uint32_t)__builtin_popcountll(below);
            const float t_after = mine + dt;
            const int src = below ? 63 - __builtin_clzll(below) : 0;
            const float prev_after = __shfl(t_after, src, 64);
            const float lt = below ? prev_after : last_t;
            if (e) {
                const size_t o = (size_t)offset + rank;
                NGP_BOUNDS(o < (size_t)M);
                float* xo = xyzs + o * 3;
                float* dd = dirs + o * 3;
                xo[0] = x; xo[1] = y; xo[2] = z;
                dd[0] = r.dx; dd[1] = r.dy; dd[2] = r.dz;
                *reinterpret_cast<float2_t*>(deltas + o * 2) = float2_t{dt, t_after - lt};
            }
            last_t = readlane_f(t_after, 63u - (uint32_t)__builtin_clzll(emit));
            offset += (uint32_t)__builtin_popcountll(emit);
        }
        if (!WRITE && lane == 0 && window < MARCH_MASK_WINDOWS) masks[(size_t)n * MARCH_MASK_WINDOWS + window] = emit;
        window++;
        done = ray_done || (validmask != ~0ull);
        t_base = t_next_base;
    }
    if (!WRITE && lane == 0) {
        rays[n * 3] = (int32_t)n;
        rays[n * 3 + 2] = (int32_t)num_steps;
        n_windows[n] = window;
    }
}

constexpr int SCAN_THREADS = 1024;
__global__ __launch_bounds__(SCAN_THREADS) void k_march_train_scan(int32_t* __restrict__ rays, int32_t* __restrict__ counter, uint32_t N,
                                                                   uint32_t M, int reset, uint32_t* __restrict__ ws) {
    __shared__ uint32_t wsum[SCAN_THREADS / 64];
    __shared__ uint32_t first_unfit;
    const int lane = threadIdx.x & 63, wid = threadIdx.x >> 6;
    uint32_t running = reset ? 0u : (uint32_t)counter[0];
    const int32_t rays_before = reset ? 0 : counter[1];
    if (threadIdx.x == 0) first_unfit = 0xFFFFFFFFu;
    __syncthreads();
    for (uint32_t tile = 0; tile < N; tile += SCAN_THREADS) {
        const uint32_t n = tile + threadIdx.x;
        const uint32_t c = n < N ? (uint32_t)rays[n * 3 + 2] : 0u;
        const uint32_t incl = wave_inclusive_scan(c);
        if (lane == 63) wsum[wid] = incl;
        __syncthreads();
        uint32_t wbase = 0, total = 0;
#pragma unroll
        for (int w = 0; w < SCAN_THREADS / 64; w++) {
            const uint32_t v = wsum[w];
            wbase += w < wid ? v : 0u;
            total += v;
        }
        const uint32_t offset = running + wbase + incl - c;
        if (n < N) {
            rays[n * 3 + 1] = (int32_t)offset;
            if (c != 0u && offset + c > M) atomicMin(&first_unfit, offset);
        }
        running += total;
        __syncthreads();
    }
    if (threadIdx.x == 0) {
        counter[0] = (int32_t)running;
        counter[1] = rays_before + (int32_t)N;
        const uint32_t fit_end = first_unfit != 0xFFFFFFFFu ? first_unfit : running;
        ws[0] = fit_end < M ? fit_end : M;
        ws[1] = 0u;
    }
    if (threadIdx.x < CT_GROUPS) ws[march_ws_ticket_word(N) + threadIdx.x * CT_GROUP_STRIDE] = 0u;
}

__device__ __host__ __forceinline__ uint32_t loop_n_step(uint32_t n_total, uint32_t n_alive, uint32_t cap) {
    if (cap == 0u) cap = 8u;
    if (n_alive == 0) return 1u;
    const uint32_t q = n_total / n_alive;
    return q > cap ? cap : (q < 1u ? 1u : q);
}

__global__ __launch_bounds__(RM_THREADS) void k_march_rays(uint32_t n_alive, uint32_t n_step, const int32_t* __restrict__ rays_alive,
                                                           const float* __restrict__ rays_t, const float* __restrict__ rays_o,
                                                           const float* __restrict__ rays_d, float bound, float dt_gamma,
                                                           uint32_t max_steps, uint32_t C, uint32_t H, const uint8_t* __restrict__ grid,
                                                           const float* __restrict__ fars, float* __restrict__ xyzs,
                                                           float* __restrict__ dirs, float* __restrict__ deltas,
                                                           const float* __restrict__ noises, uint32_t zero_rows,
                                                           const int32_t* __restrict__ dev_state, uint32_t n_total, uint32_t n_step_cap,
                                                           uint32_t* __restrict__ rows_used) {
    const uint32_t n = blockIdx.x * RM_THREADS + threadIdx.x;
    if (dev_state) {
        n_alive = (uint32_t)dev_state[0];
        n_step = loop_n_step(n_total, n_alive, n_step_cap);
    }
    if (rows_used) {
        const uint32_t used = n_alive * n_step;
        const uint32_t padded = min(zero_rows, used + 128u - used % 128u);
        if (n == 0u) rows_used[0] = padded;
        zero_rows = padded;
    }
    if (zero_rows > 0) {
        for (uint32_t row = n_alive * n_step + n; row < zero_rows; row += gridDim.x * RM_THREADS) {
            xyzs[(size_t)row * 3] = 0.0f; xyzs[(size_t)row * 3 + 1] = 0.0f; xyzs[(size_t)row * 3 + 2] = 0.0f;
            dirs[(size_t)row * 3] = 0.0f; dirs[(size_t)row * 3 + 1] = 0.0f; dirs[(size_t)row * 3 + 2] = 0.0f;
            deltas[(size_t)row * 2] = 0.0f; deltas[(size_t)row * 2 + 1] = 0.0f;
        }
    }
    if (n >= n_alive) return;
    const uint32_t index = (uint32_t)rays_alive[n];
    const MarchParams p = make_params(bound, dt_gamma, max_steps, C, H, grid);
    const Ray r = load_ray(rays_o, rays_d, index);
    const float far = fars[index];
    float t = rays_t[index];
// ... 268 lines not shown
    const float gi0 = grad_image[index * 3], gi1 = grad_image[index * 3 + 1], gi2 = grad_image[index * 3 + 2];
    float gw = grad_ws ? grad_ws[index] : 0.0f;
    if (fin.mode != 0) {
        const float b0 = fin.mode == 2 ? fin.bg[index * 3] : fin.bg_scalar, b1 = fin.mode == 2 ? fin.bg[index * 3 + 1] : fin.bg_scalar,
                    b2 = fin.mode == 2 ? fin.bg[index * 3 + 2] : fin.bg_scalar;
        gw -= gi0 * b0 + gi1 * b1 + gi2 * b2;
    }
    const RayTotals f{image[index * 3], image[index * 3 + 1], image[index * 3 + 2], weights_sum[index], 0.0f, 0.0f};
    composite_backward_sweep<false>(sigmas, rgbs, deltas, offset, num, T_thresh, lane, f, RayGrads{gi0, gi1, gi2, gw, 0.0f, 0.0f}, sink);
}

__global__ __launch_bounds__(CT_WAVES * 64) void k_composite_train_geo_fwd(const float* __restrict__ sigmas, const float* __restrict__ rgbs,
                                                                           const float* __restrict__ deltas, const int32_t* __restrict__ rays,
                                                                           uint32_t M, uint32_t N, float T_thresh,
                                                                           float* __restrict__ weights_sum, float* __restrict__ depth,
                                                                           float* __restrict__ image, float* __restrict__ distortion) {
    const int lane = threadIdx.x & 63;
    const uint32_t n = blockIdx.x * CT_WAVES + (threadIdx.x >> 6);
    if (n >= N) return;
    const uint32_t index = (uint32_t)rays[n * 3], offset = (uint32_t)rays[n * 3 + 1], num = (uint32_t)rays[n * 3 + 2];
    RayTotals f{};
    if (num != 0 && offset + num <= M) f = composite_forward_sweep<true>(sigmas, rgbs, deltas, offset, num, T_thresh, lane);
    if (lane == 0) {
        weights_sum[index] = f.ws;
        depth[index] = f.d;
        image[index * 3] = f.r; image[index * 3 + 1] = f.g; image[index * 3 + 2] = f.b;
        distortion[index] = f.dist;
    }
}

__global__ __launch_bounds__(CT_WAVES * 64) void k_composite_train_geo_bwd(const float* __restrict__ grad_ws, const float* __restrict__ grad_depth,
                                                                           const float* __restrict__ grad_image, const float* __restrict__ grad_dist,
                                                                           const float* __restrict__ sigmas, const float* __restrict__ rgbs,
                                                                           const float* __restrict__ deltas, const int32_t* __restrict__ rays,
                                                                           const float* __restrict__ weights_sum, const float* __restrict__ depth,
                                                                           const float* __restrict__ image, const float* __restrict__ distortion,
                                                                           uint32_t M, uint32_t N, float T_thresh, float* __restrict__ grad_sigmas,
                                                                           float* __restrict__ grad_rgbs) {
    const int lane = threadIdx.x & 63;
    const uint32_t n = blockIdx.x * CT_WAVES + (threadIdx.x >> 6);
    if (n >= N) return;
    const uint32_t index = (uint32_t)rays[n * 3], offset = (uint32_t)rays[n * 3 + 1], num = (uint32_t)rays[n * 3 + 2];
    if (num == 0 || offset + num > M) return;
    const float gi0 = grad_image ? grad_image[index * 3] : 0.0f, gi1 = grad_image ? grad_image[index * 3 + 1] : 0.0f,
                gi2 = grad_image ? grad_image[index * 3 + 2] : 0.0f;
    const float gw = grad_ws ? grad_ws[index] : 0.0f, gd = grad_depth ? grad_depth[index] : 0.0f, gl = grad_dist ? grad_dist[index] : 0.0f;
    const RayTotals f{image[index * 3], image[index * 3 + 1], image[index * 3 + 2], weights_sum[index], depth[index], distortion[index]};
    composite_backward_sweep<true>(sigmas, rgbs, deltas, offset, num, T_thresh, lane, f, RayGrads{gi0, gi1, gi2, gw, gd, gl},
                                   RgbSink{grad_sigmas, grad_rgbs, false});
}

__device__ __forceinline__ void composite_loss_tail(const float* __restrict__ ray_err, uint32_t N, uint32_t* __restrict__ ticket,
                                                    float* __restrict__ loss, uint32_t ray_blocks, uint32_t* __restrict__ group_tickets) {
    if (loss == nullptr) return;
    __shared__ float part[CT_WAVES];
    __shared__ bool last;
    asm volatile("s_waitcnt vmcnt(0)" ::: "memory");
    __builtin_amdgcn_fence(__ATOMIC_RELEASE, "workgroup");
    __syncthreads();
    if (threadIdx.x == 0) {
        const uint32_t groups = ray_blocks < CT_GROUPS ? ray_blocks : CT_GROUPS;
        const uint32_t group = blockIdx.x % groups, members = (ray_blocks - group + groups - 1u) / groups;
        uint32_t* gt = group_tickets + group * CT_GROUP_STRIDE;
        bool l = false;
        if (__hip_atomic_fetch_add(gt, 1u, __ATOMIC_RELAXED, __HIP_MEMORY_SCOPE_AGENT) == members - 1u) {
            __hip_atomic_store(gt, 0u, __ATOMIC_RELAXED, __HIP_MEMORY_SCOPE_AGENT);
            l = __hip_atomic_fetch_add(ticket, 1u, __ATOMIC_RELAXED, __HIP_MEMORY_SCOPE_AGENT) == groups - 1u;
        }
        last = l;
    }
    __syncthreads();
    if (!last) return;
    static_assert(CT_WAVES == 4, "loss_sum_block adds four wave sums");
    loss_sum_block(ray_err, N, loss, part);
    if (threadIdx.x == 0) __hip_atomic_store(ticket, 0u, __ATOMIC_RELAXED, __HIP_MEMORY_SCOPE_AGENT);
}

__global__ __launch_bounds__(CT_WAVES * 64) void k_composite_train_loss_bwd(
    const float* __restrict__ sigmas, const float* __restrict__ rgbs, const float* __restrict__ deltas, const int32_t* __restrict__ rays,
    uint32_t M, uint32_t N, float T_thresh, float* __restrict__ weights_sum, Finish fin, const float* __restrict__ target,
    const float* __restrict__ loss_scale, float* __restrict__ ray_err, uint32_t* __restrict__ ticket, float* __restrict__ loss,
    float* __restrict__ grad_sigmas, half_t* __restrict__ grad_out16, const uint32_t* __restrict__ rows_used, uint32_t ray_blocks,
    uint32_t* __restrict__ group_tickets) {
    const int lane = threadIdx.x & 63;
    const SigmoidHalfSink sink{grad_sigmas, grad_out16};
    if (blockIdx.x >= ray_blocks) return zero_unowned_rows(sink, rows_used, M, ray_blocks);
    const uint32_t n = blockIdx.x * CT_WAVES + (threadIdx.x >> 6);
    if (n < N) {
        const uint32_t index = (uint32_t)rays[n * 3], offset = (uint32_t)rays[n * 3 + 1], num = (uint32_t)rays[n * 3 + 2];
        const bool has_rows = num != 0 && offset + num <= M;
        RayTotals f{};
        if (has_rows) f = composite_forward_sweep<false>(sigmas, rgbs, deltas, offset, num, T_thresh, lane);
        const float b0 = fin.mode == 2 ? fin.bg[index * 3] : fin.bg_scalar, b1 = fin.mode == 2 ? fin.bg[index * 3 + 1] : fin.bg_scalar,
                    b2 = fin.mode == 2 ? fin.bg[index * 3 + 2] : fin.bg_scalar;
        const float t1 = 1.0f - f.ws;
        const float i0 = f.r + t1 * b0, i1 = f.g + t1 * b1, i2 = f.b + t1 * b2;
        const float scale = loss_scale ? loss_scale[0] : 1.0f;
        const float norm = 2.0f / (float)(3u * N);
        const float e0 = i0 - target[index * 3], e1 = i1 - target[index * 3 + 1], e2 = i2 - target[index * 3 + 2];
        const float gi0 = (norm * e0) * scale, gi1 = (norm * e1) * scale, gi2 = (norm * e2) * scale;
        if (lane == 0) {
            weights_sum[index] = f.ws;
            fin.image_out[index * 3] = i0; fin.image_out[index * 3 + 1] = i1; fin.image_out[index * 3 + 2] = i2;
            const float nr = fin.nears[index], fr = fin.fars[index];
            fin.depth_out[index] = fmaxf(f.d - nr, 0.0f) / (fr - nr);
            __hip_atomic_store(&ray_err[n], __builtin_fmaf(e2, e2, __builtin_fmaf(e1, e1, e0 * e0)), __ATOMIC_RELAXED, __HIP_MEMORY_SCOPE_AGENT);
        }
        if (has_rows) {
            const float gw = 0.0f - (gi0 * b0 + gi1 * b1 + gi2 * b2);
            composite_backward_sweep<false>(sigmas, rgbs, deltas, offset, num, T_thresh, lane, f, RayGrads{gi0, gi1, gi2, gw, 0.0f, 0.0f}, sink);
        }
    }
    composite_loss_tail(ray_err, N, ticket, loss, ray_blocks, group_tickets);
}

__global__ __launch_bounds__(CT_WAVES * 64) void k_composite_train_geo_loss_bwd(
    const float* __restrict__ sigmas, const float* __restrict__ rgbs, const float* __restrict__ deltas, const int32_t* __restrict__ rays,
    uint32_t M, uint32_t N, float T_thresh, float* __restrict__ weights_sum, Finish fin, const float* __restrict__ target,
    float lambda_distortion, float lambda_depth, const float* __restrict__ target_depth, const float* __restrict__ depth_weight,
    const float* __restrict__ loss_scale, float* __restrict__ depth_raw, float* __restrict__ distortion, float* __restrict__ ray_err,
    uint32_t* __restrict__ ticket, float* __restrict__ loss, float* __restrict__ grad_sigmas, half_t* __restrict__ grad_out16,
    const uint32_t* __restrict__ rows_used, uint32_t ray_blocks, uint32_t* __restrict__ group_tickets) {
    const int lane = threadIdx.x & 63;
    const SigmoidHalfSink sink{grad_sigmas, grad_out16};
    if (blockIdx.x >= ray_blocks) return zero_unowned_rows(sink, rows_used, M, ray_blocks);
    const uint32_t n = blockIdx.x * CT_WAVES + (threadIdx.x >> 6);
    if (n < N) {
        const uint32_t index = (uint32_t)rays[n * 3], offset = (uint32_t)rays[n * 3 + 1], num = (uint32_t)rays[n * 3 + 2];
        const bool has_rows = num != 0 && offset + num <= M;
        RayTotals f{};
        if (has_rows) f = composite_forward_sweep<true>(sigmas, rgbs, deltas, offset, num, T_thresh, lane);
        const float b0 = fin.mode == 2 ? fin.bg[index * 3] : fin.bg_scalar, b1 = fin.mode == 2 ? fin.bg[index * 3 + 1] : fin.bg_scalar,
                    b2 = fin.mode == 2 ? fin.bg[index * 3 + 2] : fin.bg_scalar;
        const float t1 = 1.0f - f.ws;
        const float i0 = f.r + t1 * b0, i1 = f.g + t1 * b1, i2 = f.b + t1 * b2;
        const float scale = loss_scale ? loss_scale[0] : 1.0f;
        const float norm = 2.0f / (float)(3u * N);
        const float e0 = i0 - target[index * 3], e1 = i1 - target[index * 3 + 1], e2 = i2 - target[index * 3 + 2];
        const float gi0 = (norm * e0) * scale, gi1 = (norm * e1) * scale, gi2 = (norm * e2) * scale;
        const float nr = fin.nears[index], fr = fin.fars[index];
        const float span = fmaxf(fr - nr, FLT_MIN);
        const float dn = f.dist / span;
        const float gl = ((lambda_distortion / (float)N) / span) * scale;
        const float m = depth_weight ? depth_weight[index] : 1.0f;
        const float dz = f.d - (target_depth ? target_depth[index] : 0.0f);
        const float gd = (((2.0f * lambda_depth) / (float)N) * m * dz) * scale;
        if (lane == 0) {
            weights_sum[index] = f.ws;
            fin.image_out[index * 3] = i0; fin.image_out[index * 3 + 1] = i1; fin.image_out[index * 3 + 2] = i2;
            fin.depth_out[index] = fmaxf(f.d - nr, 0.0f) / (fr - nr);
            depth_raw[index] = f.d;
            distortion[index] = dn;
            __hip_atomic_store(&ray_err[n], __builtin_fmaf(e2, e2, __builtin_fmaf(e1, e1, e0 * e0)) +
                                                3.0f * (lambda_distortion * dn + lambda_depth * (m * (dz * dz))),
                               __ATOMIC_RELAXED, __HIP_MEMORY_SCOPE_AGENT);
        }
        if (has_rows) {
            const float gw = 0.0f - (gi0 * b0 + gi1 * b1 + gi2 * b2);
            composite_backward_sweep<true>(sigmas, rgbs, deltas, offset, num, T_thresh, lane, f, RayGrads{gi0, gi1, gi2, gw, gd, gl}, sink);
        }
    }
    composite_loss_tail(ray_err, N, ticket, loss, ray_blocks, group_tickets);
}

__global__ __launch_bounds__(RM_THREADS) void k_composite_rays(uint32_t n_alive, uint32_t n_step, float T_thresh, int32_t* __restrict__ rays_alive,
                                                               float* __restrict__ rays_t, const float* __restrict__ sigmas,
// ... 424 lines not shown
#define RM_LAUNCH_1D(kernel, count, st, ...) NGP_LAUNCH(kernel, dim3(cdiv((count), RM_THREADS)), dim3(RM_THREADS), 0, st, __VA_ARGS__)

extern "C" int ngp_near_far_from_aabb(const float* rays_o, const float* rays_d, const float* aabb, uint32_t N, float min_near,
                                      float* nears, float* fars, ngp_stream_t stream) {
    if (N == 0) return NGP_OK;
    NGP_REQUIRE(rays_o && rays_d && aabb && nears && fars, NGP_ERR_INVALID, "near_far_from_aabb: NULL tensor");
    RM_LAUNCH_1D(k_near_far_from_aabb, N, as_stream(stream), rays_o, rays_d, aabb, N, min_near, nears, fars);
    return check_launch("near_far_from_aabb");
}

extern "C" int ngp_sph_from_ray(const float* rays_o, const float* rays_d, float radius, uint32_t N, float* coords,
                                ngp_stream_t stream) {
    if (N == 0) return NGP_OK;
    NGP_REQUIRE(rays_o && rays_d && coords, NGP_ERR_INVALID, "sph_from_ray: NULL tensor");
    RM_LAUNCH_1D(k_sph_from_ray, N, as_stream(stream), rays_o, rays_d, radius, N, coords);
    return check_launch("sph_from_ray");
}

extern "C" int ngp_morton3D(const int32_t* coords, uint32_t N, int32_t* indices, ngp_stream_t stream) {
    if (N == 0) return NGP_OK;
    NGP_REQUIRE(coords && indices, NGP_ERR_INVALID, "morton3D: NULL tensor");
    RM_LAUNCH_1D(k_morton3D, N, as_stream(stream), coords, N, indices);
    return check_launch("morton3D");
}

extern "C" int ngp_morton3D_invert(const int32_t* indices, uint32_t N, int32_t* coords, ngp_stream_t stream) {
    if (N == 0) return NGP_OK;
    NGP_REQUIRE(coords && indices, NGP_ERR_INVALID, "morton3D_invert: NULL tensor");
    RM_LAUNCH_1D(k_morton3D_invert, N, as_stream(stream), indices, N, coords);
    return check_launch("morton3D_invert");
}

extern "C" int ngp_packbits_ex(const float* grid, uint32_t N, float density_thresh, const float* thresh_cap, uint8_t* bitfield,
                               ngp_stream_t stream) {
    if (N == 0) return NGP_OK;
    NGP_REQUIRE(grid && bitfield, NGP_ERR_INVALID, "packbits: NULL tensor");
    NGP_REQUIRE((reinterpret_cast<uintptr_t>(grid) & 15) == 0, NGP_ERR_INVALID, "packbits: grid must be 16-byte aligned");
    RM_LAUNCH_1D(k_packbits, N, as_stream(stream), grid, N, density_thresh, thresh_cap, bitfield);
    return check_launch("packbits");
}

extern "C" int ngp_packbits(const float* grid, uint32_t N, float density_thresh, uint8_t* bitfield, ngp_stream_t stream) {
    return ngp_packbits_ex(grid, N, density_thresh, nullptr, bitfield, stream);
}

extern "C" size_t ngp_density_grid_update_workspace_bytes(uint32_t n_cells) {
    return sizeof(double) * (size_t)cdiv(n_cells, DM_THREADS * DM_PER_THREAD) + 64;
}

extern "C" int ngp_density_grid_update(const float* sigmas, const int64_t* cells, uint32_t n, float density_scale, float decay, float* density_grid,
                                       uint32_t n_cells, float* scratch, float density_thresh, float* mean_out, uint8_t* bitfield, void* workspace,
                                       ngp_stream_t stream) {
    NGP_REQUIRE(density_grid && scratch && mean_out && bitfield && workspace, NGP_ERR_INVALID, "density_grid_update: NULL tensor");
    NGP_REQUIRE(n_cells >= 8 && n_cells % 8 == 0, NGP_ERR_INVALID, "density_grid_update: the grid must hold a multiple of 8 cells (got %u)", n_cells);
    NGP_REQUIRE(((reinterpret_cast<uintptr_t>(density_grid) | reinterpret_cast<uintptr_t>(scratch)) & 15) == 0, NGP_ERR_INVALID,
                "density_grid_update: grid and scratch must be 16-byte aligned");
    hipStream_t st = as_stream(stream);
    if (n) {
        NGP_REQUIRE(sigmas && cells, NGP_ERR_INVALID, "density_grid_update: NULL tensor");
        RM_LAUNCH_1D(k_density_scatter, n, st, sigmas, cells, n, density_scale, scratch, n_cells);
    }
    const uint32_t blocks = cdiv(n_cells, DM_THREADS * DM_PER_THREAD);
    double* partials = reinterpret_cast<double*>(workspace);
    uint32_t* ticket = reinterpret_cast<uint32_t*>(partials + blocks);
    NGP_LAUNCH(k_density_apply_mean, dim3(blocks), dim3(DM_THREADS), 0, st, density_grid, scratch, n_cells, decay, partials, ticket, mean_out);
    RM_LAUNCH_1D(k_packbits, n_cells / 8, st, (const float*)density_grid, n_cells / 8, density_thresh, (const float*)mean_out, bitfield);
    return check_launch("density_grid_update");
}

extern "C" size_t ngp_march_rays_train_workspace_bytes(uint32_t N) {
    return sizeof(uint32_t) * (march_ws_ticket_word(N) + (size_t)CT_GROUPS * CT_GROUP_STRIDE);
}

static int check_march_args(const char* fn, uint32_t C, uint32_t H, uint32_t max_steps) {
    NGP_REQUIRE(C >= 1 && C <= 8, NGP_ERR_INVALID, "%s: cascade count C must be in [1, 8] (got %u)", fn, C);
    NGP_REQUIRE(H >= 2 && H <= 1024, NGP_ERR_INVALID, "%s: grid size H must be in [2, 1024] (got %u)", fn, H);
    NGP_REQUIRE(max_steps >= 1, NGP_ERR_INVALID, "%s: max_steps must be positive", fn);
    return NGP_OK;
}

static int march_rays_train_impl(const float* rays_o, const float* rays_d, const uint8_t* grid_in, float bound, float dt_gamma,
                                 uint32_t max_steps, uint32_t N, uint32_t C, uint32_t H, uint32_t M, const float* aabb, float min_near,
                                 float* nears, float* fars, float* xyzs, float* dirs, float* deltas, int32_t* rays, int32_t* counter,
                                 const float* noises, void* workspace, uint32_t flags, ngp_stream_t stream) {
    int rc = check_march_args("march_rays_train", C, H, max_steps);
    if (rc) return rc;
    if (N == 0) return NGP_OK;
    NGP_REQUIRE(rays_o && rays_d && grid_in && nears && fars && xyzs && dirs && deltas && rays && counter && noises && workspace,
                NGP_ERR_INVALID, "march_rays_train: NULL tensor");
    hipStream_t st = as_stream(stream);
    uint32_t* ws = reinterpret_cast<uint32_t*>(workspace);
    const uint32_t ray_blocks = cdiv(N, MW_WAVES);
    const bool zero_tail = (flags & NGP_MARCH_ZERO_TAIL) && M > 0;
    const bool self_scan = (flags & NGP_MARCH_RESET_COUNTER) && !(flags & NGP_MARCH_SCAN_LAUNCH) && N <= 8192u;
    const uint32_t extra = zero_tail ? 16u : (self_scan ? 1u : 0u);
    const dim3 block(MW_WAVES * 64);
    const bool const_dt = dt_gamma == 0.0f;
#define MARCH_WAVE(WRITE, CDT)                                                                                                              \
    NGP_LAUNCH((k_march_train_wave<WRITE, CDT>), dim3(ray_blocks + ((WRITE) ? extra : 0u)), block, 0, st, rays_o, rays_d, grid_bits,   \
                       bound, dt_gamma, max_steps, N, C, H, M, nears, fars, xyzs, dirs, deltas, rays, noises, ws_windows, ws_masks,              \
                       (flags & NGP_MARCH_NOISE_FROM_SEED) != 0, aabb, min_near, ws, ray_blocks, self_scan ? counter : (int32_t*)nullptr,       \
                       zero_tail)
    const uint8_t* grid_bits = grid_in;
    uint32_t* ws_windows = ws + 2;
    uint64_t* ws_masks = reinterpret_cast<uint64_t*>(ws + 2 + ((N + 1u) & ~1u));
    if (const_dt) MARCH_WAVE(false, true); else MARCH_WAVE(false, false);
    rc = check_launch("march_rays_train(count)");
    if (rc) return rc;
    if (!self_scan) {
        NGP_LAUNCH(k_march_train_scan, dim3(1), dim3(SCAN_THREADS), 0, st, rays, counter, N, M, (int)((flags & NGP_MARCH_RESET_COUNTER) != 0), ws);
        rc = check_launch("march_rays_train(scan)");
        if (rc) return rc;
    }
    if (const_dt) MARCH_WAVE(true, true); else MARCH_WAVE(true, false);
#undef MARCH_WAVE
    return check_launch("march_rays_train(write)");
}

extern "C" int ngp_march_rays_train_ex(const float* rays_o, const float* rays_d, const uint8_t* grid_in, float bound, float dt_gamma,
                                       uint32_t max_steps, uint32_t N, uint32_t C, uint32_t H, uint32_t M, const float* nears,
                                       const float* fars, float* xyzs, float* dirs, float* deltas, int32_t* rays, int32_t* counter,
                                       const float* noises, void* workspace, uint32_t flags, ngp_stream_t stream) {
    return march_rays_train_impl(rays_o, rays_d, grid_in, bound, dt_gamma, max_steps, N, C, H, M, nullptr, 0.0f, const_cast<float*>(nears),
                                 const_cast<float*>(fars), xyzs, dirs, deltas, rays, counter, noises, workspace, flags, stream);
}

extern "C" int ngp_march_rays_train_aabb(const float* rays_o, const float* rays_d, const uint8_t* grid_in, float bound, float dt_gamma,
                                         uint32_t max_steps, uint32_t N, uint32_t C, uint32_t H, uint32_t M, const float* aabb, float min_near,
                                         float* nears, float* fars, float* xyzs, float* dirs, float* deltas, int32_t* rays, int32_t* counter,
                                         const float* noises, void* workspace, uint32_t flags, ngp_stream_t stream) {
    NGP_REQUIRE(aabb || N == 0, NGP_ERR_INVALID, "march_rays_train_aabb: NULL box");
    return march_rays_train_impl(rays_o, rays_d, grid_in, bound, dt_gamma, max_steps, N, C, H, M, aabb, min_near, nears, fars, xyzs, dirs, deltas,
                                 rays, counter, noises, workspace, flags, stream);
}

extern "C" int ngp_march_rays_train(const float* rays_o, const float* rays_d, const uint8_t* grid_in, float bound, float dt_gamma,
                                    uint32_t max_steps, uint32_t N, uint32_t C, uint32_t H, uint32_t M, const float* nears,
                                    const float* fars, float* xyzs, float* dirs, float* deltas, int32_t* rays, int32_t* counter,
                                    const float* noises, void* workspace, ngp_stream_t stream) {
    return ngp_march_rays_train_ex(rays_o, rays_d, grid_in, bound, dt_gamma, max_steps, N, C, H, M, nears, fars, xyzs, dirs, deltas, rays,
                                   counter, noises, workspace, 0u, stream);
}

static int make_finish(const char* fn, int bg_mode, float bg_scalar, const float* bg, const float* nears, const float* fars, float* image_out,
                       float* depth_out, bool forward, Finish* fin) {
    NGP_REQUIRE(bg_mode >= 0 && bg_mode <= 2, NGP_ERR_INVALID, "%s: bg_mode must be 0, 1 or 2", fn);
    NGP_REQUIRE(bg_mode != 2 || bg, NGP_ERR_INVALID, "%s: bg_mode 2 needs a per-ray background tensor", fn);
    NGP_REQUIRE(bg_mode == 0 || !forward || (nears && fars && image_out && depth_out), NGP_ERR_INVALID, "%s: NULL finishing tensor", fn);
    *fin = Finish{bg_mode, bg_scalar, bg, nears, fars, image_out, depth_out};
    return NGP_OK;
}

extern "C" int ngp_composite_rays_train_forward_ex(const float* sigmas, const float* rgbs, const float* deltas, const int32_t* rays,
                                                   uint32_t M, uint32_t N, float T_thresh, float* weights_sum, float* depth, float* image,
                                                   int bg_mode, float bg_scalar, const float* bg, const float* nears, const float* fars,
                                                   float* image_out, float* depth_out, ngp_stream_t stream) {
    if (N == 0) return NGP_OK;
    NGP_REQUIRE(sigmas && rgbs && deltas && rays && weights_sum && depth && image, NGP_ERR_INVALID,
                "composite_rays_train_forward: NULL tensor");
    Finish fin;
    int rc = make_finish("composite_rays_train_forward", bg_mode, bg_scalar, bg, nears, fars, image_out, depth_out, true, &fin);
    if (rc) return rc;
    NGP_LAUNCH(k_composite_train_fwd, dim3(cdiv(N, CT_WAVES)), dim3(CT_WAVES * 64), 0, as_stream(stream), sigmas, rgbs, deltas,
                       rays, M, N, T_thresh, weights_sum, depth, image, fin);
    return check_launch("composite_rays_train_forward");
}

extern "C" int ngp_composite_rays_train_forward(const float* sigmas, const float* rgbs, const float* deltas, const int32_t* rays,
                                                uint32_t M, uint32_t N, float T_thresh, float* weights_sum, float* depth,
                                                float* image, ngp_stream_t stream) {
    return ngp_composite_rays_train_forward_ex(sigmas, rgbs, deltas, rays, M, N, T_thresh, weights_sum, depth, image, 0, 0.0f, nullptr,
                                               nullptr, nullptr, nullptr, nullptr, stream);
}

extern "C" int ngp_composite_rays_train_backward_ex(const float* grad_weights_sum, const float* grad_image, const float* sigmas,
                                                    const float* rgbs, const float* deltas, const int32_t* rays,
                                                    const float* weights_sum, const float* image, uint32_t M, uint32_t N,
                                                    float T_thresh, float* grad_sigmas, float* grad_rgbs, int bg_mode, float bg_scalar,
                                                    const float* bg, const uint32_t* rows_used, ngp_stream_t stream) {
    if (N == 0) return NGP_OK;
    NGP_REQUIRE(grad_image && sigmas && rgbs && deltas && rays && weights_sum && image && grad_sigmas && grad_rgbs, NGP_ERR_INVALID,
                "composite_rays_train_backward: NULL tensor");
    NGP_REQUIRE(grad_weights_sum || bg_mode != 0, NGP_ERR_INVALID, "composite_rays_train_backward: NULL tensor");
    Finish fin;
    int rc = make_finish("composite_rays_train_backward", bg_mode, bg_scalar, bg, nullptr, nullptr, nullptr, nullptr, false, &fin);
    if (rc) return rc;
    const uint32_t ray_blocks = cdiv(N, CT_WAVES);
    const uint32_t tail_blocks = rows_used ? 32u : 0u;
    NGP_LAUNCH(k_composite_train_bwd, dim3(ray_blocks + tail_blocks), dim3(CT_WAVES * 64), 0, as_stream(stream), grad_weights_sum,
                       grad_image, sigmas, rgbs, deltas, rays, weights_sum, image, M, N, T_thresh, grad_sigmas, grad_rgbs, fin, rows_used,
                       ray_blocks);
    return check_launch("composite_rays_train_backward");
}

extern "C" int ngp_composite_rays_train_geo_forward(const float* sigmas, const float* rgbs, const float* deltas, const int32_t* rays, uint32_t M,
                                                    uint32_t N, float T_thresh, float* weights_sum, float* depth, float* image,
                                                    float* distortion, ngp_stream_t stream) {
    if (N == 0) return NGP_OK;
    NGP_REQUIRE(sigmas && rgbs && deltas && rays && weights_sum && depth && image && distortion, NGP_ERR_INVALID,
                "composite_rays_train_geo_forward: NULL tensor");
    NGP_LAUNCH(k_composite_train_geo_fwd, dim3(cdiv(N, CT_WAVES)), dim3(CT_WAVES * 64), 0, as_stream(stream), sigmas, rgbs, deltas,
                       rays, M, N, T_thresh, weights_sum, depth, image, distortion);
    return check_launch("composite_rays_train_geo_forward");
}

extern "C" int ngp_composite_rays_train_geo_backward(const float* grad_weights_sum, const float* grad_depth, const float* grad_image,
                                                     const float* grad_distortion, const float* sigmas, const float* rgbs,
                                                     const float* deltas, const int32_t* rays, const float* weights_sum, const float* depth,
                                                     const float* image, const float* distortion, uint32_t M, uint32_t N, float T_thresh,
                                                     float* grad_sigmas, float* grad_rgbs, ngp_stream_t stream) {
    if (N == 0) return NGP_OK;
    NGP_REQUIRE(sigmas && rgbs && deltas && rays && weights_sum && depth && image && distortion && grad_sigmas && grad_rgbs, NGP_ERR_INVALID,
                "composite_rays_train_geo_backward: NULL tensor");
    NGP_LAUNCH(k_composite_train_geo_bwd, dim3(cdiv(N, CT_WAVES)), dim3(CT_WAVES * 64), 0, as_stream(stream), grad_weights_sum,
                       grad_depth, grad_image, grad_distortion, sigmas, rgbs, deltas, rays, weights_sum, depth, image, distortion, M, N,
                       T_thresh, grad_sigmas, grad_rgbs);
// ... 287 lines not shown
```

torch-ngp_amd/fused.py:

```python
import ctypes
import os
from collections import namedtuple

import numpy as np
import torch
from torch.autograd import Function

import _ngp_capi as capi
from optim import announce_overwrite, clean_deposits, resync_stale_shadows

_PLANAR_IN = capi.NGP_FF_INPUT_PLANAR
_PLANAR_DX = capi.NGP_FF_DX_PLANAR

NetCfg = namedtuple('NetCfg', 'bound L S H gridtype align interp nl_sigma nl_color training')
RenderCfg = namedtuple('RenderCfg', 'cascade grid_size min_near capacity perturb dt_gamma max_steps T_thresh density_scale bg_scalar')
Marched = namedtuple('Marched', 'xyzs dirs deltas rays nears fars ws')
Saved = namedtuple('Saved', 'xyzs offsets enc ws16 wc16 fb_s fb_c h16 color_in rgb sigma deltas rays weights_sum image_raw bg march_ws')
Bufs = namedtuple('Bufs', 'emb16 ws16 wc16 g_emb g_ws g_wc')


class GeoLoss(namedtuple('GeoLoss', 'lambda_distortion lambda_depth target_depth depth_weight', defaults=(0.0, 0.0, None, None))):
    __slots__ = ()

    def __new__(cls, lambda_distortion=0.0, lambda_depth=0.0, target_depth=None, depth_weight=None):
# ... 82 lines not shown
        scratch_s = scratch_c[:nl_sigma]
        capi.check(capi.lib.ngp_ffmlp_backward_ex(g_h16.data_ptr(), enc.data_ptr(), ws16.data_ptr(), fb_s.data_ptr(), M, 32, 16, 64, nl_sigma,
                                                   0, 6, 1, scratch_s.data_ptr(), g_enc.data_ptr(), g_ws.data_ptr(), _PLANAR_IN | _PLANAR_DX, st))
        _grid_backward(g_enc, x, offsets, g_emb, M, cfg.L, cfg.S, cfg.H, cfg.gridtype, cfg.align, cfg.interp, cfg.bound, st)
        if deposited:
            return None, None, None, None, None, None, None, None, None
        return None, None, g_emb, g_ws, g_wc, None, None, None, None


USE_FUSED_NETWORK = True


def _network_forward(enc, dirs, d_valid, ws16, wc16, nl_sigma, nl_color, density_scale, training, fb_s, h16, sigma, color_in, fb_c, out16, rgb, M, st):
    if USE_FUSED_NETWORK:
        capi.check(capi.lib.ngp_network_forward(enc.data_ptr(), dirs.data_ptr(), M, d_valid, ws16.data_ptr(), wc16.data_ptr(), nl_sigma, nl_color,
                                                 float(density_scale), 1 if training else 0, capi.ptr(fb_s), capi.ptr(h16) if training else None,
                                                 sigma.data_ptr(), capi.ptr(color_in) if training else None, capi.ptr(fb_c), rgb.data_ptr(), _PLANAR_IN, st))
        return
    if training:
        capi.check(capi.lib.ngp_ffmlp_forward_ex(enc.data_ptr(), ws16.data_ptr(), M, 32, 16, 64, nl_sigma, 0, 6, fb_s.data_ptr(), h16.data_ptr(),
                                                  _PLANAR_IN, st))
    else:
        capi.check(capi.lib.ngp_ffmlp_inference_ex(enc.data_ptr(), ws16.data_ptr(), M, 32, 16, 64, nl_sigma, 0, 6, None, h16.data_ptr(), _PLANAR_IN, st))
    capi.check(capi.lib.ngp_pipeline_mid_forward(h16.data_ptr(), dirs.data_ptr(), sigma.data_ptr(), color_in.data_ptr(), M, d_valid, float(density_scale), st))
    if training:
        capi.check(capi.lib.ngp_ffmlp_forward_ex(color_in.data_ptr(), wc16.data_ptr(), M, 32, 16, 64, nl_color, 0, 6, fb_c.data_ptr(), out16.data_ptr(), 0, st))
    else:
        capi.check(capi.lib.ngp_ffmlp_inference_ex(color_in.data_ptr(), wc16.data_ptr(), M, 32, 16, 64, nl_color, 0, 6, None, out16.data_ptr(), 0, st))
    capi.check(capi.lib.ngp_pipeline_rgb_forward(out16.data_ptr(), rgb.data_ptr(), M, st))


def _grid_backward(g_enc, x, offsets, g_emb, M, L, S, H, gridtype, align, interp, bound, st, found_inf=None, slabs=None, overwrite=False,
                   table_adam=None):
    arr, ws, nbytes = capi.grid_backward_workspace(offsets, M, 3, 2, L, S, H, gridtype, align, capi.NGP_F16)
    if overwrite:
        slabs = slabs if slabs is not None else capi.SlabSets()
        slabs.overwrite_table = 1
    if table_adam is not None:
        if not overwrite:
            raise RuntimeError('fused: table_adam needs overwrite_table')
        slabs.table_adam = ctypes.cast(ctypes.pointer(table_adam), ctypes.c_void_p)
    if found_inf is not None and arr is None:
        raise RuntimeError('fused: the in-kernel non-finite sweep needs the host copy of the encoder offsets (call iteration_checks_gradients '
                           'outside stream capture first)')
    capi.check(capi.lib.ngp_grid_encode_backward_checked_slabs(g_enc.data_ptr(), x.data_ptr(), None, offsets.data_ptr(), capi.ptr(g_emb), M, 3, 2, L, S,
                                                                 H, None, None, gridtype, align, interp, capi.NGP_F16, float(bound),
                                                                 None if arr is None else ctypes.cast(arr, ctypes.c_void_p), capi.ptr(ws), nbytes,
                                                                 capi.ptr(found_inf), None if slabs is None else ctypes.cast(ctypes.pointer(slabs), ctypes.c_void_p),
                                                                 st))


def _half_weights(params, cast=True):
    sh = [getattr(p, '_ngp_fp16_pin', None) for p in params]
    if any(t is None for t in sh):
        resync_stale_shadows(params)
        sh = [t if t is not None else getattr(p, '_ngp_fp16', None) for t, p in zip(sh, params)]
    if cast:
        sh = [t if t is not None else p.detach().to(torch.half) for t, p in zip(sh, params)]
    return sh


def _operands(params, deposit, overwrite_table=False):
    sh = [getattr(p, '_ngp_fp16', None) for p in params]
    gr = [getattr(p, '_ngp_grad16', None) for p in params]
    if not deposit or any(t is None for t in sh + gr):
        return Bufs(*_half_weights(params), None, None, None)
    resync_stale_shadows(params)
    clean_deposits(params[1:] if overwrite_table else params)
    return Bufs(*sh, *gr)


def _grad_targets(bufs, n_emb, dev):
    if bufs.g_emb is not None:
        return bufs.g_emb, bufs.g_ws.view(-1), bufs.g_wc.view(-1), True
    return torch.zeros(n_emb, 2, device=dev, dtype=torch.half), torch.empty_like(bufs.ws16), torch.empty_like(bufs.wc16), False


def fused_ngp(x, d, encoder, sigma_net, color_net, bound, training, density_scale=1.0):
    cfg = network_cfg(encoder, sigma_net, color_net, bound, training)
    params = (encoder.embeddings, sigma_net.weights, color_net.weights)
    return _fused_ngp.apply(x, d, *params, encoder.offsets, cfg, _operands(params, deposit=training), density_scale)


def _render_train_march(rays_o, rays_d, bitfield, aabb, counter, cfg, rcfg, noise_seed=None, into=None):
    N = rays_o.shape[0]
    M = rcfg.capacity
    dev = rays_o.device
    st = capi.stream()
    f32 = dict(device=dev, dtype=torch.float32)
    if into is not None:
        (xyzs, dirs, deltas, rays, nears, fars, ws) = into
    else:
        nears = torch.empty(N, **f32)
        fars = torch.empty(N, **f32)
        xyzs = torch.empty(M, 3, **f32)
        dirs = torch.empty(M, 3, **f32)
        deltas = torch.empty(M, 2, **f32)
        rays = torch.empty(N, 3, device=dev, dtype=torch.int32)
        ws = torch.empty(capi.lib.ngp_march_rays_train_workspace_bytes(N), dtype=torch.uint8, device=dev)
    march_flags = capi.NGP_MARCH_RESET_COUNTER | capi.NGP_MARCH_ZERO_TAIL | (0 if USE_FUSED_SCAN else capi.NGP_MARCH_SCAN_LAUNCH)
    if rcfg.perturb and noise_seed is not None:
        noises, march_flags = noise_seed, march_flags | capi.NGP_MARCH_NOISE_FROM_SEED
    else:
        noises = torch.rand(N, **f32) if rcfg.perturb else torch.zeros(N, **f32)
    capi.check(capi.lib.ngp_march_rays_train_aabb(rays_o.data_ptr(), rays_d.data_ptr(), bitfield.data_ptr(), float(cfg.bound), float(rcfg.dt_gamma),
                                                   rcfg.max_steps, N, rcfg.cascade, rcfg.grid_size, M, aabb.data_ptr(), float(rcfg.min_near),
                                                   nears.data_ptr(), fars.data_ptr(), xyzs.data_ptr(), dirs.data_ptr(), deltas.data_ptr(),
                                                   rays.data_ptr(), counter.data_ptr(), noises.data_ptr(), ws.data_ptr(), march_flags, st))
    return Marched(xyzs, dirs, deltas, rays, nears, fars, ws)


def _render_train_network(marched, bufs, bg, offsets, cfg, rcfg, composite=True):
    xyzs, rays = marched.xyzs, marched.rays
    nl_sigma, nl_color = cfg.nl_sigma, cfg.nl_color
    N, M = rays.shape[0], rcfg.capacity
    dev = xyzs.device
    st = capi.stream()
    f32 = dict(device=dev, dtype=torch.float32)
    half = dict(device=dev, dtype=torch.half)
    enc = torch.empty(cfg.L, M, 2, **half)
    costs = capi.ray_level_costs(cfg.L, cfg.S, cfg.H, 3.0 ** 0.5 / (rcfg.max_steps * max(float(cfg.bound), 1e-6))) if USE_BALANCED_FORWARD else None
    _grid_forward(xyzs, bufs.emb16, offsets, enc, M, cfg.L, cfg.S, cfg.H, cfg.gridtype, cfg.align, cfg.interp, cfg.bound, costs, st)
    h16 = torch.empty(M, 16, **half)
    color_in = torch.empty(M, 32, **half)
    out16 = torch.empty(M, 16, **half)
    sigma = torch.empty(M, **f32)
    rgb = torch.empty(M, 3, **f32)
    if _recompute(nl_sigma, nl_color):
        fb_s = fb_c = None
    else:
        fb_s = torch.empty(nl_sigma, M, 64, **half)
        fb_c = torch.empty(nl_color, M, 64, **half)
    _network_forward(enc, marched.dirs, M, bufs.ws16, bufs.wc16, nl_sigma, nl_color, float(rcfg.density_scale), True, fb_s, h16, sigma, color_in, fb_c,
                     out16, rgb, M, st)
    saved = Saved(xyzs, offsets, enc, bufs.ws16, bufs.wc16, fb_s, fb_c, h16, color_in, rgb, sigma, marched.deltas, rays, weights_sum=None,
                  image_raw=None, bg=bg, march_ws=marched.ws)
    if not composite:
        return saved
    weights_sum = torch.empty(N, **f32)
    depth_raw = torch.empty(N, **f32)
    image_raw = torch.empty(N, 3, **f32)
    image = torch.empty(N, 3, **f32)
    depth = torch.empty(N, **f32)
    bg_mode = 2 if bg is not None else 1
    capi.check(capi.lib.ngp_composite_rays_train_forward_ex(sigma.data_ptr(), rgb.data_ptr(), marched.deltas.data_ptr(), rays.data_ptr(), M, N,
                                                             float(rcfg.T_thresh), weights_sum.data_ptr(), depth_raw.data_ptr(), image_raw.data_ptr(),
                                                             bg_mode, float(rcfg.bg_scalar), capi.ptr(bg), marched.nears.data_ptr(),
                                                             marched.fars.data_ptr(), image.data_ptr(), depth.data_ptr(), st))
    return image, depth, weights_sum, saved._replace(weights_sum=weights_sum, image_raw=image_raw)


def _render_train_backward(saved, cfg, rcfg, grad_image, grad_ws, g_emb, g_ws, g_wc, found_inf=None, overwrite=False, input_grads=False):
    s = saved
    M, N = s.xyzs.shape[0], s.rays.shape[0]
    dev = s.xyzs.device
    st = capi.stream()
    g_sigma = torch.empty(M, device=dev)
    g_rgb = torch.empty(M, 3, device=dev)
    bg_mode = 2 if s.bg is not None else 1
    capi.check(capi.lib.ngp_composite_rays_train_backward_ex(capi.ptr(grad_ws), grad_image.data_ptr(), s.sigma.data_ptr(), s.rgb.data_ptr(),
                                                              s.deltas.data_ptr(), s.rays.data_ptr(), s.weights_sum.data_ptr(),
                                                              s.image_raw.data_ptr(), M, N, float(rcfg.T_thresh), g_sigma.data_ptr(),
                                                              g_rgb.data_ptr(), bg_mode, float(rcfg.bg_scalar), capi.ptr(s.bg),
                                                              s.march_ws.data_ptr(), st))
    g_out16 = torch.empty(M, 16, device=dev, dtype=torch.half)
    capi.check(capi.lib.ngp_pipeline_rgb_backward(g_rgb.data_ptr(), s.rgb.data_ptr(), g_out16.data_ptr(), M, st))
    return _network_backward(saved, cfg, rcfg, g_sigma, g_out16, g_emb, g_ws, g_wc, found_inf, None, overwrite, input_grads=input_grads)


def _network_backward(saved, cfg, rcfg, g_sigma, g_out16, g_emb, g_ws, g_wc, found_inf=None, loss_job=None, overwrite=False, table_adam=None,
                      input_grads=False):
    if input_grads and saved.fb_c is None:
        raise RuntimeError('fused: gradients with respect to the rays need the stored activations of the MLPs; this render was run with '
                           'NGP_FUSED_RECOMPUTE=1 (NGP_FF_RECOMPUTE: no forward buffers) -- switch it off to refine poses')
    s = saved
    nl_sigma, nl_color, density_scale = cfg.nl_sigma, cfg.nl_color, rcfg.density_scale
    grid = (cfg.L, cfg.S, cfg.H, cfg.gridtype, cfg.align, cfg.interp, cfg.bound)
    M = s.xyzs.shape[0]
    st = capi.stream()
    half = dict(device=s.xyzs.device, dtype=torch.half)
    g_enc = torch.empty(cfg.L, M, 2, **half)
    g_color_in = None
    if USE_FUSED_MID and nl_color in (2, 3) and nl_sigma in (2, 3) and not input_grads:
# ... 158 lines not shown
    return bool(USE_RECOMPUTE and USE_FUSED_NETWORK and USE_FUSED_MID and nl_color in (2, 3) and nl_sigma in (2, 3))


def iteration_checks_gradients(model):
    nl = (int(model.sigma_net.num_layers), int(model.color_net.num_layers))
    return bool(USE_FUSED_CHECK and USE_FUSED_MID and all(n in (2, 3) for n in nl) and capi.host_offsets(model.encoder.offsets) is not None)


def _train_iteration_rest(marched, bufs, bg_t, offsets, target, loss_scale, cfg, rcfg, found_inf=None, overwrite=False, table_adam=None,
                          geo_loss=None):
    if table_adam is not None and not (USE_FUSED_COMPOSITE and found_inf is not None and overwrite):
        raise RuntimeError('fused: table_adam needs the fused compositor, the in-kernel non-finite sweep (found_inf) and overwrite_table')
    if geo_loss is not None and not USE_FUSED_COMPOSITE:
        raise RuntimeError('fused: geo_loss needs the fused compositor (USE_FUSED_COMPOSITE)')
    g_emb, g_ws, g_wc = bufs.g_emb, bufs.g_ws.view(-1), bufs.g_wc.view(-1)
    if not USE_FUSED_COMPOSITE:
        image, depth, weights_sum, saved = _render_train_network(marched, bufs, bg_t, offsets, cfg, rcfg)
        loss = torch.empty(1, device=image.device, dtype=torch.float32)
        grad_image = torch.empty_like(image)
        capi.check(capi.lib.ngp_pipeline_mse_loss(image.data_ptr(), target.data_ptr(), image.numel(), capi.ptr(loss_scale), loss.data_ptr(),
                                                   grad_image.data_ptr(), capi.stream()))
        _render_train_backward(saved, cfg, rcfg, grad_image, None, g_emb, g_ws, g_wc, found_inf, overwrite)
        return loss, image, depth, weights_sum
    s = _render_train_network(marched, bufs, bg_t, offsets, cfg, rcfg, composite=False)
    N, M, dev = s.rays.shape[0], s.xyzs.shape[0], s.xyzs.device
    f32 = dict(device=dev, dtype=torch.float32)
    weights_sum, image, depth = torch.empty(N, **f32), torch.empty(N, 3, **f32), torch.empty(N, **f32)
    loss, ray_err = torch.empty(1, **f32), torch.empty(N, **f32)
    g_sigma = torch.empty(M, **f32)
    g_out16 = torch.empty(M, 16, device=dev, dtype=torch.half)
    defer = _carries_reductions(cfg.nl_sigma, cfg.nl_color)
    if geo_loss is not None:
        for name in ('target_depth', 'depth_weight'):
            t = getattr(geo_loss, name)
            if t is not None and (t.shape[0] != N or t.device != dev):
                raise RuntimeError(f'fused: geo_loss.{name} must be [{N}] float32 on {dev}')
        depth_raw, distortion = torch.empty(N, **f32), torch.empty(N, **f32)
        capi.check(capi.lib.ngp_composite_train_geo_loss_backward(s.sigma.data_ptr(), s.rgb.data_ptr(), s.deltas.data_ptr(), s.rays.data_ptr(), M, N,
                                                                   float(rcfg.T_thresh), 2 if s.bg is not None else 1, float(rcfg.bg_scalar),
                                                                   capi.ptr(s.bg), marched.nears.data_ptr(), marched.fars.data_ptr(),
                                                                   target.data_ptr(), geo_loss.lambda_distortion, geo_loss.lambda_depth,
                                                                   capi.ptr(geo_loss.target_depth), capi.ptr(geo_loss.depth_weight),
                                                                   capi.ptr(loss_scale), weights_sum.data_ptr(), image.data_ptr(), depth.data_ptr(),
                                                                   depth_raw.data_ptr(), distortion.data_ptr(),
                                                                   None if defer else loss.data_ptr(), ray_err.data_ptr(), g_sigma.data_ptr(),
                                                                   g_out16.data_ptr(), s.march_ws.data_ptr(),
                                                                   s.march_ws.numel() * s.march_ws.element_size(), capi.stream()))
        _network_backward(s, cfg, rcfg, g_sigma, g_out16, g_emb, g_ws, g_wc, found_inf, loss_job=(ray_err, loss) if defer else None,
                          overwrite=overwrite, table_adam=table_adam)
        return loss, image, depth, weights_sum, depth_raw, distortion
    capi.check(capi.lib.ngp_composite_train_loss_backward(s.sigma.data_ptr(), s.rgb.data_ptr(), s.deltas.data_ptr(), s.rays.data_ptr(), M, N,
                                                           float(rcfg.T_thresh), 2 if s.bg is not None else 1, float(rcfg.bg_scalar), capi.ptr(s.bg),
                                                           marched.nears.data_ptr(), marched.fars.data_ptr(), target.data_ptr(),
                                                           capi.ptr(loss_scale), weights_sum.data_ptr(), image.data_ptr(), depth.data_ptr(),
                                                           None if defer else loss.data_ptr(), ray_err.data_ptr(), g_sigma.data_ptr(),
                                                           g_out16.data_ptr(), s.march_ws.data_ptr(),
                                                           s.march_ws.numel() * s.march_ws.element_size(), capi.stream()))
    _network_backward(s, cfg, rcfg, g_sigma, g_out16, g_emb, g_ws, g_wc, found_inf, loss_job=(ray_err, loss) if defer else None,
                      overwrite=overwrite, table_adam=table_adam)
    return loss, image, depth, weights_sum


@torch.no_grad()
def fused_train_iteration_split(model, rays_o, rays_d, target, box, counter, capacity, loss_scale, bg_color=1, perturb=False, dt_gamma=0,
                                max_steps=1024, T_thresh=1e-4, noise_seed=None, found_inf=None, overwrite_table=False, table_adam=None,
                                geo_loss=None):
    cfg = network_cfg(model.encoder, model.sigma_net, model.color_net, model.bound, True)
    bg_t, rcfg = _render_cfg(model, capacity, bg_color, perturb, dt_gamma, max_steps, T_thresh)
    bufs = _operands((model.encoder.embeddings, model.sigma_net.weights, model.color_net.weights), True, overwrite_table)
    if bufs.g_emb is None:
        raise RuntimeError('fused_train_iteration: the parameters are not managed by optim.NGPAdam(deposit=True)')
    rays_o = rays_o.contiguous().view(-1, 3)
    rays_d = rays_d.contiguous().view(-1, 3)
    target = target.contiguous().view(-1, 3)
    if target.shape[0] != rays_o.shape[0] or target.dtype != torch.float32:
        raise RuntimeError('fused_train_iteration: target must be [N,3] float32')
    if geo_loss is not None and not isinstance(geo_loss, GeoLoss):
        raise TypeError('fused_train_iteration: geo_loss must be a fused.GeoLoss')
    box_ = {}

    def march():
        box_['m'] = _render_train_march(rays_o, rays_d, model.density_bitfield, box, counter, cfg, rcfg, noise_seed, into=box_.get('m'))

    def rest():
        ta = _table_adam_of(table_adam, model)
        out = _train_iteration_rest(box_['m'], bufs, bg_t, model.encoder.offsets, target, loss_scale, cfg, rcfg, found_inf, overwrite_table, ta,
                                    geo_loss)
        if overwrite_table:
            announce_overwrite(model.encoder.embeddings, None if ta is None else _table_adam_prefix(model, cfg, capacity))
        return out
    return march, rest


density_point_spacing = None


@torch.no_grad()
def fused_density(x, encoder, sigma_net, bound):
    M = x.shape[0]
    dev = x.device
    st = capi.stream()
    emb16, w16 = _half_weights((encoder.embeddings, sigma_net.weights))
    L = int(encoder.num_levels)
    enc = torch.empty(L, M, 2, device=dev, dtype=torch.half)
    S, H = float(np.log2(encoder.per_level_scale)), int(encoder.base_resolution)
    costs = None if density_point_spacing is None else capi.ray_level_costs(L, S, H, float(density_point_spacing))
    _grid_forward(x.contiguous(), emb16, encoder.offsets, enc, M, L, S, H, int(encoder.gridtype_id), int(bool(encoder.align_corners)),
                  int(encoder.interp_id), bound, costs, st)
    h16 = torch.empty(M, 16, device=dev, dtype=torch.half)
    capi.check(capi.lib.ngp_ffmlp_inference_ex(enc.data_ptr(), w16.data_ptr(), M, 32, 16, 64, int(sigma_net.num_layers), 0, 6, None, h16.data_ptr(),
                                                _PLANAR_IN, st))
    return torch.exp(h16[:, 0].float()), h16[:, 1:]


def inference_weights(model, x):
    enc, sn, cn = getattr(model, 'encoder', None), getattr(model, 'sigma_net', None), getattr(model, 'color_net', None)
    if enc is None or sn is None or cn is None or torch.is_grad_enabled():
        return None
    probe = torch.empty(128, 3, device=x.device, dtype=torch.float32)
    if not getattr(model, '_fused_ok', lambda *_: False)(probe, probe):
        return None
    emb16, ws16, wc16 = _half_weights((enc.embeddings, sn.weights, cn.weights), cast=False)
    if emb16 is None or ws16 is None or wc16 is None or getattr(emb16, '_ngp_sel', None) is not None:
        return None
    return emb16, ws16, wc16, network_cfg(enc, sn, cn, model.bound, False)


class pinned_half_weights:

    def __init__(self, model):
        enc, sn, cn = getattr(model, 'encoder', None), getattr(model, 'sigma_net', None), getattr(model, 'color_net', None)
        self.params = [getattr(enc, 'embeddings', None), getattr(sn, 'weights', None), getattr(cn, 'weights', None)]

    def __enter__(self):
        if all(p is not None and p.is_cuda for p in self.params) and not torch.is_grad_enabled():
            for p in self.params:
                fn = getattr(p, '_ngp_materialize', None)
                if fn is not None:
                    fn()
                buf = getattr(p, '_ngp_fp16_pinbuf', None)
                if buf is None or buf.shape != p.shape or buf.device != p.device:
                    buf = torch.empty_like(p, dtype=torch.half)
                    p._ngp_fp16_pinbuf = buf
                buf.copy_(p.detach())
                p._ngp_fp16_pin = buf
        return self

    def __exit__(self, *exc):
        for p in self.params:
            if p is not None and hasattr(p, '_ngp_fp16_pin'):
                del p._ngp_fp16_pin
        return False
```

torch-ngp_amd/graph.py:

```python
import contextlib
import os

import torch


def _capture_into(g, **kw):
    import torch.distributed as dist
    if dist.is_available() and dist.is_initialized():
        kw.setdefault('capture_error_mode', 'thread_local')
    return torch.cuda.graph(g, **kw)


MARCH_MARKS = {'boundary': None, 'net': ('k_network_forward', 1), 'composite': ('k_composite_train', 1), 'sigma': ('k_grid_backward_bin', 0),
               'sort': ('k_grid_backward_accumulate', 0)}
MARCH_MARK_ID = 1


_PARKED = []


def _drain_parked():
    if _PARKED and torch.cuda.is_available() and not torch.cuda.is_current_stream_capturing():
        torch.cuda.synchronize()
        del _PARKED[:]


def mse_loss(out, target):
    return torch.nn.functional.mse_loss(out['image'][0], target)


class GraphedTrainStep:
    def __init__(self, model, optimizer, scaler, n_rays, render_kwargs, loss_fn=mse_loss, averager=None, capacity_quantum=8192,
                 update_interval=16, after_update=None, autocast_dtype=torch.float16, direct=True, capacity_slack=2, lookahead=False,
                 fused_table_adam=False, capacity_ladder=(0.8, 1.25, 1.5625, 1.953125, 2.44140625), geo_loss=None):
        self.model, self.optimizer, self.scaler = model, optimizer, scaler
        self.loss_fn, self.averager = loss_fn, averager
        if averager is not None and averager is not optimizer and getattr(optimizer, 'flat_grad16', None) is not None:
            raise RuntimeError('GraphedTrainStep: with optim.NGPAdam(deposit=True) pass the optimizer itself as `averager`')
        self.render_kwargs = dict(render_kwargs)
        self.quantum = int(capacity_quantum)
        self.slack = int(capacity_slack)
        self.update_interval = int(update_interval)
        self.after_update = after_update
        self.autocast_dtype = autocast_dtype
        dev = next(model.parameters()).device
        self.dev = dev
        self.rays_o = torch.zeros(1, n_rays, 3, device=dev)
        self.rays_d = torch.zeros(1, n_rays, 3, device=dev)
        self.target = torch.zeros(n_rays, 3, device=dev)
        self.counter = torch.zeros(16, 2, dtype=torch.int32, device=dev)
        self.global_step = 0
        self.captured_capacity = None
        self._captured = {}
        self.capacity_ladder = tuple(float(f) for f in (capacity_ladder or ()))
        self.n_switches = 0
        self.graphs = None
        self.lists = None
        self.use_lists = os.environ.get('NGP_STEP_CMDLIST', '1') != '0'
        self.march_at = os.environ.get('NGP_STEP_MARCH_AT', 'boundary')
        if self.march_at not in MARCH_MARKS:
            raise ValueError(f'NGP_STEP_MARCH_AT={self.march_at!r}: one of {sorted(MARCH_MARKS)}')
        self.n_list_replays = 0
        self.loss = None
        self.image = None
        self.n_captures = 0
        self.capture_error = None
        self._checked_ok = False
        self.producers_check = False
        self.used_direct = False
        self.graph_updates = True
        self.update_graphs = {}
        self.n_update_captures = 0
        self.update_capture_error = None
        self.capacity = None
        self.direct = bool(direct) and loss_fn is mse_loss and scaler is None and getattr(optimizer, 'flat_grad16', None) is not None
        self.geo_loss = geo_loss
        if geo_loss is not None:
            from fused import GeoLoss
            if not isinstance(geo_loss, GeoLoss):
                raise TypeError('GraphedTrainStep: geo_loss must be a fused.GeoLoss')
            if geo_loss.lambda_depth > 0:
                raise ValueError('GraphedTrainStep: lambda_depth > 0 is not supported under the graphs (depth targets are per-batch tensors); '
                                 'use fused.fused_train_iteration(geo_loss=) eagerly')
            if not self.direct or self.render_kwargs.get('geo', False) or self.render_kwargs.get('staged', False):
                raise ValueError('GraphedTrainStep: geo_loss needs the autograd-free iteration (direct=True, the default loss_fn, scaler=None, '
                                 "optim.NGPAdam) and render_kwargs without 'geo' / 'staged'")
        self.lookahead = bool(lookahead) and self.direct and (averager is None or (averager is optimizer and getattr(optimizer, 'shard', False)))
        self.la = None
        self.la_image = None
        self.la_cur = 0
        self.la_ready = [None, None]
        self.la_hits = 0
        self.occupancy_epoch = 0
        self.la_presampled = None
        self.la_presample_hits = 0
        self.graph_collectives = os.environ.get('NGP_GRAPH_COLLECTIVES', '0') == '1'
        self.la_apply = None
        self.fused_table_adam = bool(fused_table_adam) and self.direct and averager is None and hasattr(optimizer, 'enable_table_fusion')
        self.table_fused = False
        if self.lookahead:
            self.la_rays_o = [torch.zeros(n_rays, 3, device=dev) for _ in range(2)]
            self.la_rays_d = [torch.zeros(n_rays, 3, device=dev) for _ in range(2)]
            self.la_target = [torch.zeros(n_rays, 3, device=dev) for _ in range(2)]
            self.la_seed = torch.zeros(2, dtype=torch.int32, device=dev)
            self.la_side = torch.cuda.Stream(device=dev)
            self.la_event = [torch.cuda.Event(), torch.cuda.Event()]
            self.la_sample_event = torch.cuda.Event()
            self.la_slot_event = None

    def close(self):
        side = getattr(self, 'la_side', None)
        try:
            if torch.cuda.is_available() and torch.cuda.is_current_stream_capturing():
                _PARKED.append((self.graphs, self.la, self.update_graphs, side, getattr(self, 'optimizer', None), getattr(self, '_captured', None),
                                getattr(self, 'la_apply', None), getattr(self, '_sample_pool', None), getattr(self, '_rest_pool', None)))
                return
            if side is not None:
                side.synchronize()
            comm = getattr(getattr(self, 'optimizer', None), '_comm_stream', None)
            if comm is not None:
                comm.synchronize()
            if torch.cuda.is_available() and (self.graphs is not None or self.update_graphs):
                torch.cuda.current_stream().synchronize()
            for snap in [self.__dict__] + list(getattr(self, '_captured', {}).values()):
                for cl in snap.get('lists') or ():
                    cl.destroy()
                snap['lists'] = None
            _drain_parked()
        except Exception:
            pass

    def __del__(self):
        self.close()

    def _capacity(self):
        mc = int(self.model.mean_count)
        if mc <= 0:
            return None
        return ((mc + 128 + self.quantum - 1) // self.quantum) * self.quantum

    _SNAP = ('graphs', 'lists', 'la', 'loss', 'image', 'la_image', 'la_apply', '_rest_pool', 'sharded', 'used_direct', 'table_fused', 'producers_check', '_checked_ok')

    def _snapshot(self):
        return {k: getattr(self, k, None) for k in self._SNAP}
# ... 24 lines not shown
        if cap is not None and self.capture_error is None and not self._fits(cap):
            self._geo_loss_needs_direct()
            self.captured_capacity = cap
            try:
                self._capture()
            except Exception as e:
                self.capture_error = repr(e)
                self.graphs = None
                self._captures_discarded()
                torch.cuda.synchronize()
        if cap is not None and self.graphs is not None and self.capture_error is None and self.capacity_ladder:
            base = self.captured_capacity
            for f in self.capacity_ladder:
                rung = ((int(base * f) + self.quantum - 1) // self.quantum) * self.quantum
                if rung in self._captured or rung < 16384:
                    continue
                kept = {k: getattr(self.optimizer, k) for k in ('_poison_captured', '_poisoned') if hasattr(self.optimizer, k)}
                try:
                    self.captured_capacity = rung
                    self._capture()
                except Exception as e:
                    self.ladder_error = repr(e)
                    for k, v in kept.items():
                        setattr(self.optimizer, k, v)
                    torch.cuda.synchronize()
                    break
            self._activate(base)
        m = self.model
        if self.graphs is not None and self.graph_updates and getattr(m, 'refresh_occupancy', None) is not None and getattr(m, 'cuda_ray', False):
            if update_modes is None:
                update_modes = (True, False) if m.iter_density < 16 else (False,)
            for full in update_modes:
                self._capture_update(bool(full))
        return self.captures - before

    def sync_params(self):
        fn = getattr(self.optimizer, 'materialize', None)
        if fn is not None:
            fn()

    def _overwrites_table(self):
        import fused
        sharded = self.averager is self.optimizer and getattr(self.optimizer, 'shard', False)
        return bool(fused.USE_OVERWRITE_TABLE and (self.averager is None or sharded))

    def _mark_deposits(self):
        emb = getattr(getattr(self.model, 'encoder', None), 'embeddings', None)
        if emb is not None and self.used_direct and self._overwrites_table():
            from optim import replayed_kept_deposits
            replayed_kept_deposits([emb] if self.averager is None else [emb] + list(getattr(self.optimizer, 'flat_params', [])))

    def _after_replay(self):
        self._mark_deposits()
        if self.table_fused:
            from optim import replayed_fused_table_step
            replayed_fused_table_step(self.optimizer)

    def _captures_discarded(self):
        self.lists = None
        fn = getattr(self.optimizer, 'captures_discarded', None)
        if fn is not None:
            fn()

    def _table_fusion_fits(self, emb):
        import ctypes
        import _ngp_capi as capi
        from fused import network_cfg
        from optim import table_fusion_fits
        m = self.model
        arr = capi.host_offsets(m.encoder.offsets)
        if arr is None:
            return False
        cfg = network_cfg(m.encoder, m.sigma_net, m.color_net, m.bound, True)
        prefix = int(capi.lib.ngp_grid_table_adam_prefix(ctypes.cast(arr, ctypes.c_void_p), int(self.captured_capacity), 3, int(emb.shape[1]), cfg.L,
                                                         cfg.S, cfg.H, cfg.gridtype, cfg.align, capi.NGP_F16))
        rest = sum(p.numel() for p in getattr(self.optimizer, 'flat_params', []) if p is not emb)
        return prefix != 0xffffffff and table_fusion_fits(prefix, emb.shape[1], rest)

    def _cmdlist_ok(self, with_march):
        kw = self.render_kwargs
        if torch.is_tensor(kw.get('bg_color', None)) or (with_march and not kw.get('perturb', False)):
            return False
        return bool(self.use_lists and self.direct and self.scaler is None and self.averager is None and self._checked_ok and self._direct_ok())

    def _recording(self, lists, with_march=False):
        if not self._cmdlist_ok(with_march):
            return contextlib.nullcontext()
        from cmdlist import CommandList
        lists.append(CommandList())
        return lists[-1]

    def _replay_rest(self, g, cl):
        if cl is None:
            g.replay()
        else:
            cl.replay(torch.cuda.current_stream().cuda_stream)
            self.n_list_replays += 1

    def _clean_deposits(self):
        clean = getattr(self.optimizer, 'clean_deposits', None)
        if clean is not None and not (self.used_direct and self._overwrites_table()):
            clean(getattr(self.optimizer, 'flat_params', []))

    def _direct_ok(self):
        m, kw = self.model, self.render_kwargs
        if not (self.direct and m.training and getattr(m, 'bg_radius', 0) <= 0 and hasattr(m, '_fused_render_ok')):
            return False
        if kw.get('staged', False) or kw.get('geo', False) or kw.get('aux', None) is not None:
            return False
        bg = kw.get('bg_color', None)
        with torch.autocast('cuda', dtype=self.autocast_dtype):
            return m._fused_render_ok(self.rays_o.view(-1, 3), self.rays_d.view(-1, 3), 1 if bg is None else bg,
                                      kw.get('force_all_rays', False))

    def _iteration_args(self, checked, p=None):
        from optim import FOUND_INF, SCALE, STEP_COUNT
        m, kw, opt = self.model, self.render_kwargs, self.optimizer
        bg = kw.get('bg_color', None)
        if p is None:
            batch, counter, seed = (self.rays_o, self.rays_d, self.target), self.counter[0], opt.scalars.narrow(0, STEP_COUNT, 1)
        else:
            batch, counter, seed = (self.la_rays_o[p], self.la_rays_d[p], self.la_target[p]), self.counter[p], self.la_seed[p:p + 1]
        args = (m, *batch, m.aabb_train, counter, self.captured_capacity, opt.scalars.narrow(0, SCALE, 1), 1 if bg is None else bg, kw.get('perturb', False),
                kw.get('dt_gamma', 0), kw.get('max_steps', 1024), kw.get('T_thresh', 1e-4))
        return args, dict(noise_seed=seed, found_inf=opt.scalars.narrow(0, FOUND_INF, 1) if checked else None, overwrite_table=self._overwrites_table(),
                          table_adam=opt if checked and self.table_fused else None, geo_loss=getattr(self, 'geo_loss', None))

    def _iteration_front(self):
        m = self.model
        if self._direct_ok():
            from fused import fused_train_iteration
            self.optimizer.zero_grad(set_to_none=True)
            self.producers_check = self._checked_ok and (self.averager is None)
            args, kwargs = self._iteration_args(self.producers_check)
            loss, image = fused_train_iteration(*args, **kwargs)[:2]
            self.image = image
            self.used_direct = True
            return loss[0]
        self._geo_loss_needs_direct()
        self.used_direct = False
        self.producers_check = False
        saved_counter, saved_mc, saved_ls = m._buffers['step_counter'], m.mean_count, m.local_step
        m._buffers['step_counter'] = self.counter
        m.mean_count = self.captured_capacity - 128
        m.local_step = 0
        try:
            self.optimizer.zero_grad(set_to_none=True)
            with torch.autocast('cuda', dtype=self.autocast_dtype):
                out = m.render(self.rays_o, self.rays_d, **self.render_kwargs)
                loss = self.loss_fn(out, self.target)
            self.image = self._image_of(out)
            self._scaled(loss).backward()
        finally:
            m._buffers['step_counter'], m.mean_count, m.local_step = saved_counter, saved_mc, saved_ls
        return loss

    @staticmethod
    def _image_of(out):
        return out['image'].detach().reshape(-1, 3).float()

    def _geo_loss_needs_direct(self):
        if getattr(self, 'geo_loss', None) is not None and not self._direct_ok():
            raise RuntimeError('GraphedTrainStep: geo_loss needs the autograd-free iteration and this model / render configuration is not '
                               'eligible for it (GraphedTrainStep._direct_ok)')

    def _scaled(self, loss):
# ... 184 lines not shown
                mean_count = int(m.step_counter[:used, 0].sum().item() / used)
        if use_graph:
            entry = self.update_graphs[full]
            g, mean = entry[0], entry[1]
            if len(entry) == 4:
                if self.la_presampled == full:
                    torch.cuda.current_stream().wait_event(self.la_sample_event)
                    self.la_presample_hits += 1
                else:
                    entry[2].replay()
                self.la_presampled = None
            g.replay()
        else:
            with torch.autocast('cuda', dtype=self.autocast_dtype):
                mean = refresh(full=full)
        if mean_count is not None:
            m.finish_update(mean, mean_count=mean_count)
        else:
            m.finish_update(mean)

    def _eager(self, rays_o, rays_d, target):
        self.optimizer.zero_grad(set_to_none=True)
        geo = getattr(self, 'geo_loss', None)
        with torch.autocast('cuda', dtype=self.autocast_dtype):
            if geo is None:
                out = self.model.render(rays_o, rays_d, **self.render_kwargs)
                loss = self.loss_fn(out, target)
            else:
                out = self.model.render(rays_o, rays_d, **dict(self.render_kwargs, geo=True))
                loss = self.loss_fn(out, target) + geo.lambda_distortion * out['distortion'].float().mean()
        self.image = self._image_of(out)
        self._scaled(loss).backward()
        if self.averager is not None and not getattr(self.optimizer, 'shard', False):
            self.averager.all_reduce()
        self._iteration_back()
        return loss.detach()

    @staticmethod
    def _announced(ready, rays_o, rays_d, epoch):
        return (ready is not None and ready[0] is rays_o and ready[1] is rays_d and ready[2] == (rays_o._version, rays_d._version)
                and ready[3] == epoch)

    def _step_lookahead(self, rays_o, rays_d, target, next_rays):
        m = self.model
        p = self.la_cur
        gm, gr, loss = self.la[p][:3]
        images = getattr(self, 'la_image', None)
        if images is not None:
            self.image = images[p]
        main = torch.cuda.current_stream()
        ready = self.la_ready[p]
        hit = self._announced(ready, rays_o, rays_d, self.occupancy_epoch)
        slot = m.step_counter[m.local_step % 16]
        if ready is not None:
            main.wait_event(self.la_event[p])
        if hit:
            if not (ready[4] is target and ready[5] == target._version):
                self.la_target[p].copy_(target, non_blocking=True)
            self.la_hits += 1
        else:
            torch._foreach_copy_([self.la_rays_o[p], self.la_rays_d[p], self.la_target[p]],
                                 [rays_o.view_as(self.la_rays_o[p]), rays_d.view_as(self.la_rays_d[p]), target], non_blocking=True)
            self.la_seed[p:p + 1].fill_(self.global_step)
            gm.replay()
            slot.copy_(self.counter[p], non_blocking=True)
            if self.la_slot_event is None:
                self.la_slot_event = torch.cuda.Event()
            self.la_slot_event.record(main)
        self.la_ready[p] = None
        q = 1 - p
        ahead = next_rays is not None and (self.global_step + 1) % self.update_interval != 0
        cl = self.lists[p] if self.lists else None
        early = ahead and cl is not None and MARCH_MARKS[self.march_at] is not None
        if early:
            self._replay_rest(gr, cl)
        if ahead:
            side = self.la_side
            if early:
                cl.wait_mark(MARCH_MARK_ID, side.cuda_stream)
            else:
                side.wait_stream(main)
            with torch.cuda.stream(side):
                no, nd = next_rays[0], next_rays[1]
                dst, src = [self.la_rays_o[q], self.la_rays_d[q]], [no.view_as(self.la_rays_o[q]), nd.view_as(self.la_rays_d[q])]
                nt, ntv = None, None
                if len(next_rays) > 2:
                    dst.append(self.la_target[q])
                    src.append(next_rays[2])
                    nt, ntv = next_rays[2], next_rays[2]._version
                torch._foreach_copy_(dst, src, non_blocking=True)
                self.la_seed[q:q + 1].fill_(self.global_step + 1)
                self.la[q][0].replay()
                m.step_counter[(m.local_step + 1) % 16].copy_(self.counter[q], non_blocking=True)
                self.la_event[q].record(side)
            self.la_ready[q] = (no, nd, (no._version, nd._version), self.occupancy_epoch, nt, ntv)
        elif (self.global_step + 1) % self.update_interval == 0 and self.graph_updates and self.update_capture_error is None:
            full = m.iter_density < 16
            entry = self.update_graphs.get(full)
            if entry is not None and len(entry) == 4:
                side = self.la_side
                side.wait_stream(main)
                with torch.cuda.stream(side):
                    entry[2].replay()
                    self.la_sample_event.record(side)
                self.la_presampled = full
        if self.la_apply is not None:
            opt = self.optimizer
            opt.wait_shadows()
            gr.replay()
            opt.reduce_gradients()
            self.la_apply.replay()
            opt.gather_shadows()
        elif not early:
            self._replay_rest(gr, cl)
        self.la_cur = q
        return loss

    def step(self, rays_o, rays_d, target, next_rays=None):
        m = self.model
        if self.global_step % self.update_interval == 0:
            if getattr(self.optimizer, 'shard', False):
                self.optimizer.wait_shadows()
            if self.la is not None:
                torch.cuda.current_stream().wait_stream(self.la_side)
            self._update_extra_state()
            self.occupancy_epoch += 1
            if self.after_update is not None:
                self.after_update(m)
        cap = self._capacity()
        self.capacity = cap
        if cap is None:
            loss = self._eager(rays_o, rays_d, target)
            self.global_step += 1
            return loss
        if self.capture_error is not None:
            loss = self._eager(rays_o, rays_d, target)
            self.global_step += 1
            return loss
        pick = None if self._fits(cap) else self._pick_captured(cap)
        if pick is not None:
            if pick != self.captured_capacity:
                self._activate(pick)
        elif not self._fits(cap):
            self._geo_loss_needs_direct()
            self.captured_capacity = cap
            try:
                self._capture()
            except Exception as e:
                self.capture_error = repr(e)
                self.graphs = None
                self._captures_discarded()
                torch.cuda.synchronize()
                loss = self._eager(rays_o, rays_d, target)
                self.global_step += 1
                return loss
        self.capacity = self.captured_capacity
        self._clean_deposits()
        if self.la is not None:
            loss = self._step_lookahead(rays_o, rays_d, target, next_rays)
            self._after_replay()
            m.local_step += 1
            self.global_step += 1
            return loss
        if getattr(self, 'sharded', False):
            opt = self.optimizer
            pc = getattr(self, '_precopied', None)
            self._precopied = None
            if not (pc is not None and pc[0] is rays_o and pc[1] is rays_d and pc[2] is target
                    and pc[3] == (rays_o._version, rays_d._version, target._version)):
                torch._foreach_copy_([self.rays_o, self.rays_d, self.target], [rays_o.view_as(self.rays_o), rays_d.view_as(self.rays_d), target],
                                     non_blocking=True)
            self.graphs[0].replay()
            opt.wait_shadows()
            self.graphs[1].replay()
            opt.reduce_gradients()
            m.step_counter[m.local_step % 16].copy_(self.counter[0], non_blocking=True)
# ... 22 lines not shown
```

Before: 649.7 million.

## Fuse lookahead ray copies, seed fill and counter copy into native march kernel

```diff
diff --git a/include/ngp_hip.h b/include/ngp_hip.h
--- a/include/ngp_hip.h
+++ b/include/ngp_hip.h
@@ -283,6 +283,16 @@
                               float* nears, float* fars, float* xyzs, float* dirs, float* deltas, int32_t* rays, int32_t* counter,
                               const float* noises, void* workspace, uint32_t flags, ngp_stream_t stream);
 
+#define NGP_MARCH_WIDE 0u
+#define NGP_MARCH_THIN 1u
+#define NGP_MARCH_THIN_MAX_WAVES 8u
+int ngp_march_rays_train_lookahead(const float* rays_o, const float* rays_d, const float* target, const uint8_t* grid, float bound,
+                                   float dt_gamma, uint32_t max_steps, uint32_t N, uint32_t C, uint32_t H, uint32_t M, const float* aabb,
+                                   float min_near, float* keep_o, float* keep_d, float* keep_target, uint32_t seed, uint32_t* seed_word,
+                                   int32_t* ring_slot, float* nears, float* fars, float* xyzs, float* dirs, float* deltas, int32_t* rays,
+                                   int32_t* counter, const float* noises, void* workspace, uint32_t flags, uint32_t geometry,
+                                   uint32_t waves_per_cu, ngp_stream_t stream);
+
 int ngp_march_rays_ex(uint32_t n_alive, uint32_t n_step, const int32_t* rays_alive, const float* rays_t, const float* rays_o,
                       const float* rays_d, float bound, float dt_gamma, uint32_t max_steps, uint32_t C, uint32_t H,
                       const uint8_t* grid, const float* nears, const float* fars, float* xyzs, float* dirs, float* deltas,
diff --git a/torch-ngp_amd/_ngp_capi.py b/torch-ngp_amd/_ngp_capi.py
--- a/torch-ngp_amd/_ngp_capi.py
+++ b/torch-ngp_amd/_ngp_capi.py
@@ -10,6 +10,7 @@
 NGP_FF_INPUT_PLANAR, NGP_FF_DX_PLANAR, NGP_FF_LAYERED, NGP_FF_SINGLE_WAVE, NGP_FF_DEFER_REDUCE, NGP_FF_RECOMPUTE = 1, 2, 4, 8, 16, 32
 NGP_FF_SERIAL_FLUSH = 64
 NGP_MARCH_RESET_COUNTER, NGP_MARCH_ZERO_TAIL, NGP_MARCH_NOISE_FROM_SEED, NGP_MARCH_SCAN_LAUNCH = 1, 2, 4, 8
+NGP_MARCH_WIDE, NGP_MARCH_THIN, NGP_MARCH_THIN_MAX_WAVES = 0, 1, 8
 NGP_OPT_PHASE_CHECK, NGP_OPT_PHASE_UPDATE, NGP_OPT_PHASE_COMMIT, NGP_OPT_PHASE_FLIP = 1, 2, 4, 8
 ABI_VERSION = 11
 
@@ -99,6 +100,8 @@
     'ngp_march_rays_train_ex': [_vp, _vp, _vp, _f32, _f32, _u32, _u32, _u32, _u32, _u32, _vp, _vp, _vp, _vp, _vp, _vp, _vp, _vp, _vp, _u32, _vp],
     'ngp_march_rays_train_aabb': [_vp, _vp, _vp, _f32, _f32, _u32, _u32, _u32, _u32, _u32, _vp, _f32, _vp, _vp, _vp, _vp, _vp, _vp, _vp, _vp, _vp, _u32,
                                   _vp],
+    'ngp_march_rays_train_lookahead': [_vp, _vp, _vp, _vp, _f32, _f32, _u32, _u32, _u32, _u32, _u32, _vp, _f32, _vp, _vp, _vp, _u32, _vp, _vp,
+                                       _vp, _vp, _vp, _vp, _vp, _vp, _vp, _vp, _vp, _u32, _u32, _u32, _vp],
     'ngp_composite_rays_train_forward_ex': [_vp, _vp, _vp, _vp, _u32, _u32, _f32, _vp, _vp, _vp, _i32, _f32, _vp, _vp, _vp, _vp, _vp, _vp],
     'ngp_composite_rays_train_backward_ex': [_vp, _vp, _vp, _vp, _vp, _vp, _vp, _vp, _u32, _u32, _f32, _vp, _vp, _i32, _f32, _vp, _vp, _vp],
     'ngp_composite_rays_train_geo_forward': [_vp, _vp, _vp, _vp, _u32, _u32, _f32, _vp, _vp, _vp, _vp, _vp],
diff --git a/torch-ngp_amd/csrc/common.h b/torch-ngp_amd/csrc/common.h
--- a/torch-ngp_amd/csrc/common.h
+++ b/torch-ngp_amd/csrc/common.h
@@ -74,6 +74,15 @@
 #else
 #define NGP_BOUNDS(cond) do { } while (0)
 #endif
+
+#ifndef NGP_CHAIN_PRIORITY
+#define NGP_CHAIN_PRIORITY 0
+#endif
+__device__ __forceinline__ void raise_chain_priority() {
+#if NGP_CHAIN_PRIORITY
+    asm volatile("s_setprio %0" ::"n"(NGP_CHAIN_PRIORITY));
+#endif
+}
 
 __device__ __forceinline__ _Float16 to_half_rne(float v) {
     asm volatile("" : "+v"(v));
diff --git a/torch-ngp_amd/csrc/ffmlp.hip b/torch-ngp_amd/csrc/ffmlp.hip
--- a/torch-ngp_amd/csrc/ffmlp.hip
+++ b/torch-ngp_amd/csrc/ffmlp.hip
@@ -357,6 +357,7 @@
     const half_t* __restrict__ w_color, half_t* __restrict__ fb_s, half_t* __restrict__ h16, float* __restrict__ sigma,
     half_t* __restrict__ color_in, half_t* __restrict__ fb_c, float* __restrict__ rgb, uint32_t n_tiles_cap, uint32_t nl_s, uint32_t nl_c,
     float density_scale, const uint32_t* __restrict__ rows_dev) {
+    raise_chain_priority();
     constexpr int WIDTH = 64, NIB = 2, NKB = 4;
     constexpr uint32_t in_kb = 2;
     const uint32_t n_tiles = rows_dev ? min(n_tiles_cap, (rows_dev[0] + (uint32_t)FF_TILE - 1u) / (uint32_t)FF_TILE) : n_tiles_cap;
@@ -1052,6 +1053,7 @@
                              bool with_dx, half_t* __restrict__ grad_inputs, float* __restrict__ slabs,
                              half_t* __restrict__ grad_weights_direct, bool in_planar, bool dx_planar, uint32_t pf_depth, MidEpilogue mid,
                              uint32_t lds_bytes, bool serial_flush) {
+    raise_chain_priority();
     static_assert(NHM == 1 || NHM == 2, "the paired backward covers 2- and 3-layer networks");
     constexpr int NIB = Shape<WIDTH>::NIB, NKB = Shape<WIDTH>::NKB;
     extern __shared__ __attribute__((aligned(16))) unsigned char smem[];
diff --git a/torch-ngp_amd/csrc/gridencoder.hip b/torch-ngp_amd/csrc/gridencoder.hip
--- a/torch-ngp_amd/csrc/gridencoder.hip
+++ b/torch-ngp_amd/csrc/gridencoder.hip
@@ -984,6 +984,7 @@
 void k_grid_backward_bin(const half_t* __restrict__ grad, const float* __restrict__ inputs, const int32_t* __restrict__ offsets,
                          half_t* __restrict__ grad_grid, uint32_t B, GridLevels lv, uint32_t gridtype, bool align_corners, uint32_t interp,
                          InputMap im, BinPlan plan, uint32_t* __restrict__ descriptors, uint2* __restrict__ records, AtomicPart ap) {
+    raise_chain_priority();
     uint32_t bin_block = blockIdx.x, n_bin_blocks = gridDim.x;
     if (ap.n_blocks) {
         const uint64_t total = gridDim.x;
diff --git a/torch-ngp_amd/csrc/raymarching.hip b/torch-ngp_amd/csrc/raymarching.hip
--- a/torch-ngp_amd/csrc/raymarching.hip
+++ b/torch-ngp_amd/csrc/raymarching.hip
@@ -360,7 +360,16 @@
     return (float)(x >> 8) * 0x1p-24f;
 }
 
-template <bool WRITE, bool CONST_DT>
+struct MarchAhead {
+    const float* target;
+    float *keep_o, *keep_d, *keep_target;
+    uint32_t* seed_word;
+    int32_t* ring_slot;
+    const int32_t* counter;
+    uint32_t seed, thin;
+};
+
+template <bool WRITE, bool CONST_DT, bool AHEAD>
 __global__ __launch_bounds__(MW_WAVES * 64) void k_march_train_wave(const float* __restrict__ rays_o, const float* __restrict__ rays_d,
                                                                     const uint8_t* __restrict__ grid, float bound, float dt_gamma,
                                                                     uint32_t max_steps, uint32_t N, uint32_t C, uint32_t H, uint32_t M,
@@ -371,8 +380,10 @@
                                                                     uint64_t* __restrict__ masks, bool noise_from_seed,
                                                                     const float* __restrict__ aabb, float min_near,
                                                                     uint32_t* __restrict__ fit_end, uint32_t ray_blocks,
-                                                                    int32_t* __restrict__ self_scan_counter, bool zero_tail) {
+                                                                    int32_t* __restrict__ self_scan_counter, bool zero_tail,
+                                                                    MarchAhead ahead) {
     const uint32_t lane = threadIdx.x & 63;
+    const bool thin = AHEAD && ahead.thin != 0u;
     __shared__ uint32_t part[MW_WAVES], part2[MW_WAVES];
     if (WRITE && blockIdx.x >= ray_blocks) {
         uint32_t first_row;
@@ -406,10 +417,15 @@
                 self_scan_counter[1] = (int32_t)N;
                 fit_end[0] = first_row;
                 fit_end[1] = 0u;
+                if (AHEAD) { ahead.ring_slot[0] = (int32_t)total; ahead.ring_slot[1] = (int32_t)N; }
             }
             if (blockIdx.x == ray_blocks && threadIdx.x < CT_GROUPS) fit_end[march_ws_ticket_word(N) + threadIdx.x * CT_GROUP_STRIDE] = 0u;
         } else {
             first_row = fit_end[0];
+            if (AHEAD && blockIdx.x == ray_blocks && threadIdx.x == 0) {
+                ahead.ring_slot[0] = ahead.counter[0];
+                ahead.ring_slot[1] = ahead.counter[1];
+            }
         }
         if (zero_tail) {
             const uint32_t stride = (gridDim.x - ray_blocks) * MW_WAVES * 64;
@@ -422,9 +438,11 @@
         return;
     }
     const uint32_t wid = (uint32_t)__builtin_amdgcn_readfirstlane((int)(threadIdx.x >> 6));
-    const uint32_t n = blockIdx.x * MW_WAVES + wid;
+    uint32_t n = blockIdx.x * MW_WAVES + wid;
     uint32_t scanned_offset = 0;
-    if (WRITE && self_scan_counter) {
+    if (AHEAD && !WRITE && blockIdx.x == 0 && threadIdx.x == 0) ahead.seed_word[0] = ahead.seed;
+    uint32_t summed_to = 0;
+    if (WRITE && self_scan_counter && !thin) {
         uint32_t sum = 0;
         const uint32_t first = blockIdx.x * MW_WAVES;
         for (uint32_t i = threadIdx.x; i < first; i += MW_WAVES * 64) sum += (uint32_t)rays[i * 3 + 2];
@@ -439,7 +457,22 @@
     }
     if (n >= N) return;
     const MarchParams p = make_params(bound, dt_gamma, max_steps, C, H, grid);
+    do {
+    if (AHEAD && WRITE && self_scan_counter && thin) {
+        uint32_t sum = 0;
+        for (uint32_t i = summed_to + lane; i < n; i += 64u) sum += (uint32_t)rays[i * 3 + 2];
+#pragma unroll
+        for (int o = 32; o > 0; o >>= 1) sum += (uint32_t)__shfl_xor((int)sum, o, 64);
+        scanned_offset += sum;
+        summed_to = n;
+        if (lane == 0) rays[n * 3 + 1] = (int32_t)scanned_offset;
+    }
     const Ray r = load_ray(rays_o, rays_d, n);
+    if (AHEAD && !WRITE && lane < 3u) {
+        ahead.keep_o[n * 3 + lane] = rays_o[n * 3 + lane];
+        ahead.keep_d[n * 3 + lane] = rays_d[n * 3 + lane];
+        ahead.keep_target[n * 3 + lane] = ahead.target[n * 3 + lane];
+    }
     float far, near;
     if (!WRITE && aabb) {
         near_far_from_aabb(r.ox, r.oy, r.oz, r.dx, r.dy, r.dz, aabb, min_near, near, far);
@@ -454,10 +487,10 @@
     if (WRITE) {
         offset = self_scan_counter ? scanned_offset : (uint32_t)rays[n * 3 + 1];
         limit = (uint32_t)rays[n * 3 + 2];
-        if (limit == 0 || offset + limit > M) return;
+        if (limit == 0 || offset + limit > M) continue;
     }
     uint32_t num_steps = 0;
-    const float noise = noise_from_seed ? seeded_noise(n, reinterpret_cast<const uint32_t*>(noises)[0]) : noises[n];
+    const float noise = noise_from_seed ? seeded_noise(n, AHEAD ? ahead.seed : reinterpret_cast<const uint32_t*>(noises)[0]) : noises[n];
     float t_base = __builtin_fmaf(step_dt(p, near), noise, near);
     float last_t = t_base;
     uint32_t window = 0;
@@ -495,7 +528,7 @@
                 last_t = readlane_f(t_after, 63u - (uint32_t)__builtin_clzll(emit));
                 offset += (uint32_t)__builtin_popcountll(emit);
             }
-            return;
+            continue;
         }
     }
     float carry = -INFINITY;
@@ -607,6 +640,7 @@
         rays[n * 3 + 2] = (int32_t)num_steps;
         n_windows[n] = window;
     }
+    } while (thin && (n += ray_blocks * MW_WAVES) < N);
 }
 
 constexpr int SCAN_THREADS = 1024;
@@ -1041,6 +1075,7 @@
     const float* __restrict__ loss_scale, float* __restrict__ ray_err, uint32_t* __restrict__ ticket, float* __restrict__ loss,
     float* __restrict__ grad_sigmas, half_t* __restrict__ grad_out16, const uint32_t* __restrict__ rows_used, uint32_t ray_blocks,
     uint32_t* __restrict__ group_tickets) {
+    raise_chain_priority();
     const int lane = threadIdx.x & 63;
     const SigmoidHalfSink sink{grad_sigmas, grad_out16};
     if (blockIdx.x >= ray_blocks) return zero_unowned_rows(sink, rows_used, M, ray_blocks);
@@ -1631,7 +1666,8 @@
 static int march_rays_train_impl(const float* rays_o, const float* rays_d, const uint8_t* grid_in, float bound, float dt_gamma,
                                  uint32_t max_steps, uint32_t N, uint32_t C, uint32_t H, uint32_t M, const float* aabb, float min_near,
                                  float* nears, float* fars, float* xyzs, float* dirs, float* deltas, int32_t* rays, int32_t* counter,
-                                 const float* noises, void* workspace, uint32_t flags, ngp_stream_t stream) {
+                                 const float* noises, void* workspace, uint32_t flags, ngp_stream_t stream,
+                                 const MarchAhead* ahead = nullptr, uint32_t thin_blocks = 0u) {
     int rc = check_march_args("march_rays_train", C, H, max_steps);
     if (rc) return rc;
     if (N == 0) return NGP_OK;
@@ -1639,21 +1675,29 @@
                 NGP_ERR_INVALID, "march_rays_train: NULL tensor");
     hipStream_t st = as_stream(stream);
     uint32_t* ws = reinterpret_cast<uint32_t*>(workspace);
-    const uint32_t ray_blocks = cdiv(N, MW_WAVES);
+    const uint32_t ray_blocks = thin_blocks ? (thin_blocks < cdiv(N, MW_WAVES) ? thin_blocks : cdiv(N, MW_WAVES)) : cdiv(N, MW_WAVES);
     const bool zero_tail = (flags & NGP_MARCH_ZERO_TAIL) && M > 0;
     const bool self_scan = (flags & NGP_MARCH_RESET_COUNTER) && !(flags & NGP_MARCH_SCAN_LAUNCH) && N <= 8192u;
-    const uint32_t extra = zero_tail ? 16u : (self_scan ? 1u : 0u);
+    const uint32_t extra = zero_tail ? 16u : ((self_scan || ahead) ? 1u : 0u);
     const dim3 block(MW_WAVES * 64);
     const bool const_dt = dt_gamma == 0.0f;
-#define MARCH_WAVE(WRITE, CDT)                                                                                                              \
-    NGP_LAUNCH((k_march_train_wave<WRITE, CDT>), dim3(ray_blocks + ((WRITE) ? extra : 0u)), block, 0, st, rays_o, rays_d, grid_bits,   \
+    MarchAhead la = ahead ? *ahead : MarchAhead{};
+    la.counter = counter;
+    la.thin = thin_blocks ? 1u : 0u;
+#define MARCH_WAVE(WRITE, CDT, AHEAD)                                                                                                       \
+    NGP_LAUNCH((k_march_train_wave<WRITE, CDT, AHEAD>), dim3(ray_blocks + ((WRITE) ? extra : 0u)), block, 0, st, rays_o, rays_d, grid_bits, \
                        bound, dt_gamma, max_steps, N, C, H, M, nears, fars, xyzs, dirs, deltas, rays, noises, ws_windows, ws_masks,              \
                        (flags & NGP_MARCH_NOISE_FROM_SEED) != 0, aabb, min_near, ws, ray_blocks, self_scan ? counter : (int32_t*)nullptr,       \
-                       zero_tail)
+                       zero_tail, la)
+#define MARCH_PASS(WRITE)                                                                                                                   \
+    do {                                                                                                                                    \
+        if (ahead) { if (const_dt) MARCH_WAVE(WRITE, true, true); else MARCH_WAVE(WRITE, false, true); }                                    \
+        else { if (const_dt) MARCH_WAVE(WRITE, true, false); else MARCH_WAVE(WRITE, false, false); }                                        \
+    } while (0)
     const uint8_t* grid_bits = grid_in;
     uint32_t* ws_windows = ws + 2;
     uint64_t* ws_masks = reinterpret_cast<uint64_t*>(ws + 2 + ((N + 1u) & ~1u));
-    if (const_dt) MARCH_WAVE(false, true); else MARCH_WAVE(false, false);
+    MARCH_PASS(false);
     rc = check_launch("march_rays_train(count)");
     if (rc) return rc;
     if (!self_scan) {
@@ -1661,7 +1705,8 @@
         rc = check_launch("march_rays_train(scan)");
         if (rc) return rc;
     }
-    if (const_dt) MARCH_WAVE(true, true); else MARCH_WAVE(true, false);
+    MARCH_PASS(true);
+#undef MARCH_PASS
 #undef MARCH_WAVE
     return check_launch("march_rays_train(write)");
 }
@@ -1681,6 +1726,57 @@
     NGP_REQUIRE(aabb || N == 0, NGP_ERR_INVALID, "march_rays_train_aabb: NULL box");
     return march_rays_train_impl(rays_o, rays_d, grid_in, bound, dt_gamma, max_steps, N, C, H, M, aabb, min_near, nears, fars, xyzs, dirs, deltas,
                                  rays, counter, noises, workspace, flags, stream);
+}
+
+static int device_cus(uint32_t* cus) {
+    static uint32_t cached = 0;
+    if (!cached) {
+        int dev = 0, n = 0;
+        hipError_t e = hipGetDevice(&dev);
+        if (e == hipSuccess) e = hipDeviceGetAttribute(&n, hipDeviceAttributeMultiprocessorCount, dev);
+        NGP_REQUIRE(e == hipSuccess && n > 0, NGP_ERR_LAUNCH, "march_rays_train_lookahead: cannot read the device's compute unit count: %s",
+                    hipGetErrorString(e));
+        cached = (uint32_t)n;
+    }
+    *cus = cached;
+    return NGP_OK;
+}
+
+extern "C" int ngp_march_rays_train_lookahead(const float* rays_o, const float* rays_d, const float* target, const uint8_t* grid_in, float bound,
+                                              float dt_gamma, uint32_t max_steps, uint32_t N, uint32_t C, uint32_t H, uint32_t M, const float* aabb,
+                                              float min_near, float* keep_o, float* keep_d, float* keep_target, uint32_t seed, uint32_t* seed_word,
+                                              int32_t* ring_slot, float* nears, float* fars, float* xyzs, float* dirs, float* deltas, int32_t* rays,
+                                              int32_t* counter, const float* noises, void* workspace, uint32_t flags, uint32_t geometry,
+                                              uint32_t waves_per_cu, ngp_stream_t stream) {
+    int rc = check_march_args("march_rays_train_lookahead", C, H, max_steps);
+    if (rc) return rc;
+    NGP_REQUIRE(N > 0, NGP_ERR_INVALID, "march_rays_train_lookahead: no rays (N must be positive)");
+    NGP_REQUIRE(rays_o && rays_d && target && grid_in && aabb && keep_o && keep_d && keep_target && seed_word && ring_slot && nears && fars && xyzs &&
+                    dirs && deltas && rays && counter && workspace,
+                NGP_ERR_INVALID, "march_rays_train_lookahead: NULL tensor");
+    NGP_REQUIRE(noises || (flags & NGP_MARCH_NOISE_FROM_SEED), NGP_ERR_INVALID,
+                "march_rays_train_lookahead: NULL noises without NGP_MARCH_NOISE_FROM_SEED");
+    NGP_REQUIRE(keep_o != rays_o && keep_d != rays_d && keep_target != target, NGP_ERR_INVALID,
+                "march_rays_train_lookahead: the kept copies must not be the caller's tensors");
+    NGP_REQUIRE(geometry == NGP_MARCH_WIDE || geometry == NGP_MARCH_THIN, NGP_ERR_INVALID,
+                "march_rays_train_lookahead: geometry must be NGP_MARCH_WIDE or NGP_MARCH_THIN (got %u)", geometry);
+    NGP_REQUIRE(waves_per_cu >= 1 && waves_per_cu <= NGP_MARCH_THIN_MAX_WAVES, NGP_ERR_INVALID,
+                "march_rays_train_lookahead: resident waves per CU must be in [1, %u] (got %u)", NGP_MARCH_THIN_MAX_WAVES, waves_per_cu);
+    uint32_t thin_blocks = 0;
+    if (geometry == NGP_MARCH_THIN) {
+        uint32_t cus = 0;
+        rc = device_cus(&cus);
+        if (rc) return rc;
+        thin_blocks = cdiv(cus * waves_per_cu, MW_WAVES);
+    }
+    MarchAhead la{};
+    la.target = target;
+    la.keep_o = keep_o; la.keep_d = keep_d; la.keep_target = keep_target;
+    la.seed_word = seed_word;
+    la.ring_slot = ring_slot;
+    la.seed = seed;
+    return march_rays_train_impl(rays_o, rays_d, grid_in, bound, dt_gamma, max_steps, N, C, H, M, aabb, min_near, nears, fars, xyzs, dirs, deltas,
+                                 rays, counter, noises ? noises : reinterpret_cast<const float*>(seed_word), workspace, flags, stream, &la, thin_blocks);
 }
 
 extern "C" int ngp_march_rays_train(const float* rays_o, const float* rays_d, const uint8_t* grid_in, float bound, float dt_gamma,
diff --git a/torch-ngp_amd/fused.py b/torch-ngp_amd/fused.py
--- a/torch-ngp_amd/fused.py
+++ b/torch-ngp_amd/fused.py
@@ -188,7 +188,7 @@
     return _fused_ngp.apply(x, d, *params, encoder.offsets, cfg, _operands(params, deposit=training), density_scale)
 
 
-def _render_train_march(rays_o, rays_d, bitfield, aabb, counter, cfg, rcfg, noise_seed=None, into=None):
+def _render_train_march(rays_o, rays_d, bitfield, aabb, counter, cfg, rcfg, noise_seed=None, into=None, ahead=None):
     N = rays_o.shape[0]
     M = rcfg.capacity
     dev = rays_o.device
@@ -205,6 +205,21 @@
         rays = torch.empty(N, 3, device=dev, dtype=torch.int32)
         ws = torch.empty(capi.lib.ngp_march_rays_train_workspace_bytes(N), dtype=torch.uint8, device=dev)
     march_flags = capi.NGP_MARCH_RESET_COUNTER | capi.NGP_MARCH_ZERO_TAIL | (0 if USE_FUSED_SCAN else capi.NGP_MARCH_SCAN_LAUNCH)
+    if ahead is not None:
+        src_o, src_d, src_t, keep_t, seed, ring_slot, geometry, waves = ahead
+        noises = None
+        if rcfg.perturb:
+            march_flags |= capi.NGP_MARCH_NOISE_FROM_SEED
+        else:
+            noises = getattr(ws, '_ngp_zero_noise', None)
+            if noises is None:
+                noises = ws._ngp_zero_noise = torch.zeros(N, **f32)
+        capi.check(capi.lib.ngp_march_rays_train_lookahead(
+            src_o.data_ptr(), src_d.data_ptr(), src_t.data_ptr(), bitfield.data_ptr(), float(cfg.bound), float(rcfg.dt_gamma), rcfg.max_steps, N,
+            rcfg.cascade, rcfg.grid_size, M, aabb.data_ptr(), float(rcfg.min_near), rays_o.data_ptr(), rays_d.data_ptr(), keep_t.data_ptr(),
+            int(seed) & 0xffffffff, noise_seed.data_ptr(), ring_slot, nears.data_ptr(), fars.data_ptr(), xyzs.data_ptr(), dirs.data_ptr(),
+            deltas.data_ptr(), rays.data_ptr(), counter.data_ptr(), capi.ptr(noises), ws.data_ptr(), march_flags, geometry, waves, st))
+        return into
     if rcfg.perturb and noise_seed is not None:
         noises, march_flags = noise_seed, march_flags | capi.NGP_MARCH_NOISE_FROM_SEED
     else:
@@ -529,6 +544,11 @@
     def march():
         box_['m'] = _render_train_march(rays_o, rays_d, model.density_bitfield, box, counter, cfg, rcfg, noise_seed, into=box_.get('m'))
 
+    def march_ahead(src_o, src_d, src_target, seed, ring_slot, geometry, waves):
+        _render_train_march(rays_o, rays_d, model.density_bitfield, box, counter, cfg, rcfg, noise_seed, into=box_['m'],
+                            ahead=(src_o, src_d, src_target, target, seed, ring_slot, geometry, waves))
+    march.ahead = march_ahead if noise_seed is not None else None
+
     def rest():
         ta = _table_adam_of(table_adam, model)
         out = _train_iteration_rest(box_['m'], bufs, bg_t, model.encoder.offsets, target, loss_scale, cfg, rcfg, found_inf, overwrite_table, ta,
diff --git a/torch-ngp_amd/graph.py b/torch-ngp_amd/graph.py
--- a/torch-ngp_amd/graph.py
+++ b/torch-ngp_amd/graph.py
@@ -60,6 +60,11 @@
         self.march_at = os.environ.get('NGP_STEP_MARCH_AT', 'boundary')
         if self.march_at not in MARCH_MARKS:
             raise ValueError(f'NGP_STEP_MARCH_AT={self.march_at!r}: one of {sorted(MARCH_MARKS)}')
+        self.march_native = os.environ.get('NGP_STEP_MARCH_NATIVE', '1') != '0'
+        self.march_waves = int(os.environ.get('NGP_STEP_MARCH_WAVES', '0'))
+        if not 0 <= self.march_waves <= 8:
+            raise ValueError(f'NGP_STEP_MARCH_WAVES={self.march_waves}: 0 (one wave per ray) or 1..8 resident waves per CU')
+        self.n_native_marches = 0
         self.n_list_replays = 0
         self.loss = None
         self.image = None
@@ -250,6 +255,17 @@
         if torch.is_tensor(kw.get('bg_color', None)) or (with_march and not kw.get('perturb', False)):
             return False
         return bool(self.use_lists and self.direct and self.scaler is None and self.averager is None and self._checked_ok and self._direct_ok())
+
+    def _march_native_ok(self, q, next_rays):
+        if not (self.march_native and self.scaler is None and self.averager is None and self.la_apply is None and len(next_rays) > 2):
+            return False
+        if getattr(self.la[q][3], 'ahead', None) is None:
+            return False
+        for t, keep in zip(next_rays[:3], (self.la_rays_o[q], self.la_rays_d[q], self.la_target[q])):
+            if not (torch.is_tensor(t) and t.is_cuda and t.device == keep.device and t.dtype == torch.float32 and t.is_contiguous()
+                    and t.numel() == keep.numel() and t.data_ptr() != keep.data_ptr()):
+                return False
+        return True
 
     def _recording(self, lists, with_march=False):
         if not self._cmdlist_ok(with_march):
@@ -600,16 +616,22 @@
                 side.wait_stream(main)
             with torch.cuda.stream(side):
                 no, nd = next_rays[0], next_rays[1]
-                dst, src = [self.la_rays_o[q], self.la_rays_d[q]], [no.view_as(self.la_rays_o[q]), nd.view_as(self.la_rays_d[q])]
                 nt, ntv = None, None
                 if len(next_rays) > 2:
-                    dst.append(self.la_target[q])
-                    src.append(next_rays[2])
                     nt, ntv = next_rays[2], next_rays[2]._version
-                torch._foreach_copy_(dst, src, non_blocking=True)
-                self.la_seed[q:q + 1].fill_(self.global_step + 1)
-                self.la[q][0].replay()
-                m.step_counter[(m.local_step + 1) % 16].copy_(self.counter[q], non_blocking=True)
+                if self._march_native_ok(q, next_rays):
+                    slot_q = m.step_counter[(m.local_step + 1) % 16]
+                    self.la[q][3].ahead(no, nd, nt, self.global_step + 1, slot_q.data_ptr(), 1 if self.march_waves else 0, self.march_waves or 1)
+                    self.n_native_marches += 1
+                else:
+                    dst, src = [self.la_rays_o[q], self.la_rays_d[q]], [no.view_as(self.la_rays_o[q]), nd.view_as(self.la_rays_d[q])]
+                    if nt is not None:
+                        dst.append(self.la_target[q])
+                        src.append(nt)
+                    torch._foreach_copy_(dst, src, non_blocking=True)
+                    self.la_seed[q:q + 1].fill_(self.global_step + 1)
+                    self.la[q][0].replay()
+                    m.step_counter[(m.local_step + 1) % 16].copy_(self.counter[q], non_blocking=True)
                 self.la_event[q].record(side)
             self.la_ready[q] = (no, nd, (no._version, nd._version), self.occupancy_epoch, nt, ntv)
         elif (self.global_step + 1) % self.update_interval == 0 and self.graph_updates and self.update_capture_error is None:
```

New measurement: 649.3 million, median of 2. No clear change (-0.0%).
